# allenai/gpv-1

Measured on AMD Instinct MI355X. Metric: images/sec/node (train step, 480x640, bs32/GPU), higher is better.
Workload: dtype bf16; 1 GPU; GPV-1 (ResNet-50 + 6+6 DETR layers, 100 queries, RoI head, BERT-base, 3 co-attention, 3 text-decoder layers, V=10000) CocoCaptioning-only train step, dropout 0.1, AdamW; global_batch=32, image=480x640, parallelism=dp1

## Files before the change

gpv-1_amd/csrc/common.h:

```cpp
#pragma once
#include <hip/hip_runtime.h>
#include <stdint.h>
#include <type_traits>

typedef __bf16 bf16;
typedef bf16 __attribute__((ext_vector_type(8))) bf16x8;
typedef bf16 __attribute__((ext_vector_type(4))) bf16x4;
typedef bf16 __attribute__((ext_vector_type(2))) bf16x2;
typedef float __attribute__((ext_vector_type(4))) f32x4;

#include <stdlib.h>
#ifdef GPV_TUNING
static inline int tune_env(const char* name, int dflt) { const char* e = getenv(name); return e ? atoi(e) : dflt; }
#else
static inline int tune_env(const char*, int dflt) { return dflt; }
#endif

#define GPV_CHECK_LAUNCH() \
  do {                     \
    hipError_t e_ = hipGetLastError(); \
    if (e_ != hipSuccess) return (int)e_; \
  } while (0)

__host__ __device__ __forceinline__ bool al16(const void* p) { return (reinterpret_cast<uintptr_t>(p) & 15) == 0; }
// ... 74 lines not shown
    for (int e = 0; e < N; ++e) m |= (drop_keep(seed, base + e, thresh) ? 1u : 0u) << e;
  }
  return m;
}
namespace gpvk { extern const uint64_t* g_seed_dev; }
__device__ __forceinline__ uint64_t eff_seed(uint64_t seed, const uint64_t* epoch) {
  return epoch ? seed ^ (*epoch * 0x9E3779B97F4A7C15ull) : seed;
}
__host__ __device__ __forceinline__ uint32_t drop_thresh(float p) {
  double t = (double)p * 4294967296.0;
  if (t < 0) t = 0;
  if (t > 4294967295.0) t = 4294967295.0;
  return (uint32_t)t;
}

template <int NTHR, int U, typename SrcF, typename DstF>
__device__ __forceinline__ void stage_chunks16(int total, int tid, SrcF src, DstF dst) {
  for (int base = 0; base < total; base += NTHR * U) {
    bf16x8 tmp[U];
#pragma unroll
    for (int u = 0; u < U; ++u) {
      const int idx = base + u * NTHR + tid;
      tmp[u] = *reinterpret_cast<const bf16x8*>(src(idx < total ? idx : total - 1));
    }
#pragma unroll
    for (int u = 0; u < U; ++u) {
      const int idx = base + u * NTHR + tid;
      if (idx < total) *reinterpret_cast<bf16x8*>(dst(idx)) = tmp[u];
    }
  }
}

__device__ __forceinline__ float gelu_erf(float x) { return 0.5f * x * (1.0f + erff(x * 0.70710678118654752f)); }

template <typename T> struct Ld8;
template <> struct Ld8<bf16> {
  static __device__ __forceinline__ void ld(const bf16* p, float* o) {
    bf16x8 v = *reinterpret_cast<const bf16x8*>(p);
#pragma unroll
    for (int i = 0; i < 8; ++i) o[i] = (float)v[i];
  }
  static __device__ __forceinline__ void st(bf16* p, const float* o) {
    bf16x8 v;
#pragma unroll
    for (int i = 0; i < 8; ++i) v[i] = (bf16)o[i];
    *reinterpret_cast<bf16x8*>(p) = v;
  }
  static __device__ __forceinline__ void ld_nt(const bf16* p, float* o) {
    const bf16x8 v = __builtin_bit_cast(bf16x8, __builtin_nontemporal_load(reinterpret_cast<const u32x4*>(p)));
#pragma unroll
    for (int i = 0; i < 8; ++i) o[i] = (float)v[i];
  }
  static __device__ __forceinline__ void st_nt(bf16* p, const float* o) {
    bf16x8 v;
#pragma unroll
    for (int i = 0; i < 8; ++i) v[i] = (bf16)o[i];
    __builtin_nontemporal_store(__builtin_bit_cast(u32x4, v), reinterpret_cast<u32x4*>(p));
  }
};
template <> struct Ld8<float> {
  static __device__ __forceinline__ void ld(const float* p, float* o) {
    float4 a = *reinterpret_cast<const float4*>(p);
    float4 b = *reinterpret_cast<const float4*>(p + 4);
    o[0] = a.x; o[1] = a.y; o[2] = a.z; o[3] = a.w; o[4] = b.x; o[5] = b.y; o[6] = b.z; o[7] = b.w;
  }
  static __device__ __forceinline__ void st(float* p, const float* o) {
// ... 18 lines not shown
```

gpv-1_amd/csrc/conv1x1_stream.hip:

```cpp
#include "gemm_common.h"

namespace gpvk {
namespace {


__device__ __forceinline__ f32x4 mfma16s(bf16x8 a, bf16x8 b, f32x4 c) { return __builtin_amdgcn_mfma_f32_16x16x32_bf16(a, b, c, 0, 0, 0); }


template <int K, int NH, bool RES, bool MASK, bool NT, bool LIN = false, int NP = 1, bool BITS = false>
__global__ __launch_bounds__(512) __attribute__((amdgpu_waves_per_eu((NP == 1 && NH * K * 2 > 72 * 1024) ? 2 : 1, (NP == 1 && NH * K * 2 > 72 * 1024) ? 2 : 8)))
void c1s_kernel(GemmK p, int ncols) {
  constexpr int KC = K / 32, NTL = NH / 16, NG = NH / 32, SL = K / 8, ROWB = K * 2;
  constexpr bool BIG = NP == 1 && NH * K * 2 > 72 * 1024;
  extern __shared__ __attribute__((aligned(16))) unsigned char smem_raw[];
  bf16* Wl = reinterpret_cast<bf16*>(smem_raw);
  float* bias_l = reinterpret_cast<float*>(Wl + (size_t)ncols * K);
  const int tid = threadIdx.x, lane = tid & 63, wave = tid >> 6, g = lane >> 4, pl = lane & 15;
  const int cbase = (int)blockIdx.y * ncols;
  const bf16* A = reinterpret_cast<const bf16*>(p.A);
  const bf16* Wg = reinterpret_cast<const bf16*>(p.B) + (int64_t)cbase * p.ldb;
  bf16* C = reinterpret_cast<bf16*>(p.C) + cbase;
  const bf16* R = reinterpret_cast<const bf16*>(p.res) + cbase;
  const bf16* Mk = reinterpret_cast<const bf16*>(p.mask) + cbase;
  const float* bias_g = p.bias ? p.bias + cbase : nullptr;
// ... 130 lines not shown
          for (int i = 0; i < 4; ++i) { acc[2 * t][i] *= p.alpha; acc[2 * t + 1][i] *= p.alpha; }
        }
        float v[8] = {acc[2 * t][0] + b0.x, acc[2 * t][1] + b0.y, acc[2 * t][2] + b0.z, acc[2 * t][3] + b0.w,
                      acc[2 * t + 1][0] + b1.x, acc[2 * t + 1][1] + b1.y, acc[2 * t + 1][2] + b1.z, acc[2 * t + 1][3] + b1.w};
        bf16x8 o;
        bool masked = false;
        if constexpr (LIN) {
          if (p.dthresh) {
            masked = true;
            uint32_t dropw[4];
            if (hfast) {
#pragma unroll
              for (int q = 0; q < 4; ++q) {
                uint32_t x = hbase + (uint32_t)(h * (NH / 2) + t * 16 + q) * 0x9E3779B9u;
                x ^= x >> 16; x = __umul24(x, 0x85EBCBu);
                x ^= x >> 13; x = __umul24(x, 0xC2B2AFu);
                x ^= x >> 16;
                typedef short s16x2 __attribute__((ext_vector_type(2)));
                const s16x2 d = __builtin_elementwise_sub_sat(__builtin_bit_cast(s16x2, x ^ 0x80008000u), __builtin_bit_cast(s16x2, ts2));
                dropw[q] = __builtin_bit_cast(uint32_t, (s16x2)(d >> (s16x2){15, 15}));
              }
            } else {
              const uint32_t keep8 = drop_mask<8>(p.seed, (uint64_t)pxc * (uint64_t)nfull + (uint64_t)(cbase + c0), p.dthresh);
#pragma unroll
              for (int q = 0; q < 4; ++q)
                dropw[q] = (((keep8 >> (2 * q)) & 1u) ? 0u : 0xffffu) | (((keep8 >> (2 * q + 1)) & 1u) ? 0u : 0xffff0000u);
            }
#pragma unroll
            for (int e = 0; e < 8; ++e) {
              float x = v[e];
              if constexpr (RES) x += (float)rv[t][e];
              if (p.act == GPV_ACT_RELU) x = fmaxf(x, 0.f);
              x *= p.dscale;
              if constexpr (MASK) x = (float)mv[t][e] > 0.f ? x : 0.f;
              o[e] = (bf16)x;
            }
            u32x4 ow = __builtin_bit_cast(u32x4, o);
#pragma unroll
            for (int q = 0; q < 4; ++q) ow[q] &= ~dropw[q];
            o = __builtin_bit_cast(bf16x8, ow);
          }
        }
        if (!masked) {
#pragma unroll
          for (int e = 0; e < 8; ++e) {
            float x = v[e];
            if constexpr (RES) x += (float)rv[t][e];
            if (p.act == GPV_ACT_RELU) x = fmaxf(x, 0.f);
            if constexpr (MASK && BITS) x = ((mw[t >> 2] >> ((t & 3) * 8 + e)) & 1u) ? x : 0.f;
            else if constexpr (MASK) x = (float)mv[t][e] > 0.f ? x : 0.f;
            o[e] = (bf16)x;
          }
        }
        if constexpr (BITS && !MASK) {
          bits_acc[t >> 2] |= positive_bits8(__builtin_bit_cast(u32x4, o)) << ((t & 3) * 8);
        }
        {
          bf16* q = C + (int64_t)pxc * p.ldc + c0;
          const u32x4 ov = __builtin_bit_cast(u32x4, o);
          if constexpr (NT) asm volatile("global_store_dwordx4 %0, %1, off nt\n\ts_nop 1" :: "v"(q), "v"(ov) : "memory");
          else asm volatile("global_store_dwordx4 %0, %1, off\n\ts_nop 1" :: "v"(q), "v"(ov) : "memory");
        }
      }
      if constexpr (BITS && !MASK) {
        static_assert(NG == 8 || !(BITS && !MASK), "mask bits are written by 256-channel passes");
        unsigned char* bq = reinterpret_cast<unsigned char*>(p.out_bits) + boff;
        const uint2 bv = make_uint2(bits_acc[0], bits_acc[1]);
// ... 13 lines not shown
  const int ncols = c1s_cols(k.K, k.N), nsl = k.N / ncols;
  const size_t lds = (size_t)ncols * K * 2 + (size_t)ncols * sizeof(float);
  auto fn = c1s_kernel<K, NH, RES, MASK, NT, LIN, NP, BITS>;
  static size_t attr = 0;
  if (lds > 64 * 1024 && lds > attr) {
    hipError_t e = hipFuncSetAttribute(reinterpret_cast<const void*>(fn), hipFuncAttributeMaxDynamicSharedMemorySize, (int)lds);
    if (e != hipSuccess) { (void)hipGetLastError(); return (int)e; }
    attr = lds;
  }
  const int ntile = (k.M + 15) / 16;
  static const int bpc = tune_env("GPV_C1S_BLOCKS", 0);
  int blocks = bpc > 0 ? bpc : (lds <= 72 * 1024 ? 512 : 256);
  blocks = (blocks + nsl - 1) / nsl;
  if (blocks * 8 > ntile) blocks = (ntile + 7) / 8;
  hipLaunchKernelGGL(fn, dim3(blocks, nsl), dim3(512), lds, st, k, ncols);
  GPV_CHECK_LAUNCH();
  return 0;
}

template <int K, int NH, bool RES, bool MASK, bool NT, bool LIN = false, bool BITS = false>
int c1s_launch(const GemmK& k, hipStream_t st) {
  const int np = c1s_cols(k.K, k.N) / NH;
  if (np == 1) return c1s_launch_np<K, NH, RES, MASK, NT, LIN, 1, BITS>(k, st);
  if constexpr (K <= 128 && NH == 256 && !LIN) { if (np == 2) return c1s_launch_np<K, NH, RES, MASK, NT, LIN, 2, BITS>(k, st); }
  return -1;
}

template <int K, int NH>
int c1s_flags(const GemmK& k, hipStream_t st, bool linear) {
  const bool r = k.res != nullptr, m = k.mask != nullptr, nt = k.nt_io != 0;
  if (linear || k.alpha != 1.0f || k.dthresh) {
    if constexpr (K == 256 && NH == 256) {
      if (nt) return -1;
      if (r && m) return c1s_launch<K, NH, true, true, false, true>(k, st);
      if (r) return c1s_launch<K, NH, true, false, false, true>(k, st);
      if (m) return c1s_launch<K, NH, false, true, false, true>(k, st);
      return c1s_launch<K, NH, false, false, false, true>(k, st);
    } else {
      return -1;
    }
  }
  if (k.mask_bits || k.out_bits) {
    if (nt || !r || (k.mask_bits && k.out_bits)) return -1;
    if constexpr ((K == 128 || K == 256) && NH == 256) {
      if (k.out_bits) return (m || k.act != GPV_ACT_RELU) ? -1 : c1s_launch<K, NH, true, false, false, false, true>(k, st);
      return c1s_launch<K, NH, true, true, false, false, true>(k, st);
    } else if constexpr (K == 512 && NH == 128) {
      if (k.out_bits) return -1;
      return c1s_launch<K, NH, true, true, false, false, true>(k, st);
    } else {
      return -1;
    }
  }
  if (nt) {
    if (m) return -1;
    return r ? c1s_launch<K, NH, true, false, true>(k, st) : c1s_launch<K, NH, false, false, true>(k, st);
  }
  if (r && m) return c1s_launch<K, NH, true, true, false>(k, st);
  if (r) return c1s_launch<K, NH, true, false, false>(k, st);
  if (m) return c1s_launch<K, NH, false, true, false>(k, st);
  return c1s_launch<K, NH, false, false, false>(k, st);
}

template <int K>
int c1s_n(const GemmK& k, hipStream_t st, bool linear) {
  switch (c1s_cols(K, k.N)) {
    case 64: return c1s_flags<K, 64>(k, st, linear);
    case 128: return c1s_flags<K, 128>(k, st, linear);
    case 256: case 512: if constexpr (K <= 256) return c1s_flags<K, 256>(k, st, linear); else return -1;
  }
  return -1;
}

}

int g_c1s_mode = 1;
long g_c1s_launches = 0;

int c1s_try_launch(const GemmK& k, int dtype_in, int dtype_out, hipStream_t st, bool linear, bool dry) {
  static const int env = tune_env("GPV_C1S", -1);
  const int mode = env >= 0 ? env : g_c1s_mode;
  if (mode == 0 || dtype_in != GPV_BF16 || dtype_out != GPV_BF16) return -1;
  if (k.K != 64 && k.K != 128 && k.K != 256 && k.K != 512) return -1;
  if (k.N != 64 && k.N != 128 && k.N != 256 && k.N != 512 && k.N != 1024 && k.N != 2048 && !(linear && k.N % 256 == 0 && k.N <= 2048)) return -1;
  const int ncols = c1s_cols(k.K, k.N), nsl = k.N / ncols;
  if ((size_t)ncols * (k.K + 8) * 2 + (size_t)ncols * 4 > 150 * 1024 || nsl > 8) return -1;
  if (k.rowscale || k.accumulate || k.split_k > 1 || k.a_rowsum) return -1;
  if ((k.alpha != 1.0f || k.dthresh) && !(linear && k.K == 256 && k.N >= 256 && k.N % 256 == 0)) return -1;
  if (linear && (k.cg.SH == 2 || k.cg.cm || k.nt_io)) return -1;
  if (k.act != GPV_ACT_NONE && k.act != GPV_ACT_RELU) return -1;
  if (k.lda % 8 || k.ldb != k.K || k.ldc % 8 || (k.res && k.ldr % 8) || (k.mask && k.ldm % 8)) return -1;
  if (!al16(k.A) || !al16(k.B) || !al16(k.C) || (k.res && !al16(k.res)) || (k.mask && !al16(k.mask))) return -1;
  if (linear) {
    if (mode == 1 && (k.K != 256 || k.N < 1536 || k.M < 2048)) return -1;
  } else if (mode == 1 && ((int64_t)k.M * nsl < 65536 || k.M < 32768)) return -1;
  if (k.mask_bits || k.out_bits) {
    const int nh = ncols >= 256 ? 256 : ncols;
    const bool inst = ((k.K == 128 || k.K == 256) && nh == 256) || (k.K == 512 && nh == 128 && !k.out_bits);
    if (linear || !inst || !k.res || k.nt_io || (k.mask_bits && k.out_bits) || k.N % 256 != 0 || (k.out_bits && (k.mask && !k.mask_bits))) return -1;
    if (k.out_bits && k.act != GPV_ACT_RELU) return -1;
    if (k.K <= 128 && ncols / nh > 2) return -1;
    if (k.K > 128 && ncols / nh != 1) return -1;
  }
  if (dry) return 0;
  int e = -1;
  switch (k.K) {
    case 64: e = c1s_n<64>(k, st, linear); break;
    case 128: e = c1s_n<128>(k, st, linear); break;
    case 256: e = c1s_n<256>(k, st, linear); break;
    case 512: e = c1s_n<512>(k, st, linear); break;
  }
  if (e == 0) ++g_c1s_launches;
  return e;
}

}
```

gpv-1_amd/csrc/gemm.hip:

```cpp
#include "gemm_common.h"
#include <cstdlib>

using namespace gpvk;

#ifndef GPV_PF
#define GPV_PF 2
#endif

namespace {

constexpr int BK = 32;
constexpr int LDK = 40;

template <typename T> struct Raw8;
__device__ __forceinline__ uint32_t bf_bits(float x) { return (uint32_t)__builtin_bit_cast(unsigned short, (bf16)x); }
template <> struct Raw8<bf16> {
  uint32_t w[4];
  __device__ __forceinline__ void zero() { w[0] = w[1] = w[2] = w[3] = 0u; }
  __device__ __forceinline__ void load(const bf16* p) {
    uint4 t = *reinterpret_cast<const uint4*>(p);
    w[0] = t.x; w[1] = t.y; w[2] = t.z; w[3] = t.w;
  }
  __device__ __forceinline__ void load_n(const bf16* p, int n) {
    const unsigned short* q = reinterpret_cast<const unsigned short*>(p);
// ... 259 lines not shown
      }
      raw[it].write(hi + kr * PITCH + ch * 8, lo + kr * PITCH + ch * 8);
    }
  }
  __device__ __forceinline__ void flush_sums(float* out) {
    if constexpr (SUM) {
#pragma unroll
      for (int it = 0; it < NIT; ++it) {
        const int ch = (threadIdx.x + it * 256) % CHK;
#pragma unroll
        for (int e = 0; e < 8; ++e) {
          float v = csum[it][e];
#pragma unroll
          for (int s = CHK; s < 64; s <<= 1) v += __shfl_xor(v, s);
          const int col = col0 + ch * 8 + e;
          if ((threadIdx.x & 63) < CHK && col < ncols) atomicAdd(out + col, v);
        }
      }
    }
  }
  static __device__ __forceinline__ bf16x8 frag(const bf16* tile, int cbase, int lane) {
    typedef short __attribute__((ext_vector_type(4))) s16x4;
    typedef __attribute__((address_space(3))) s16x4 lds_s16x4;
    const int g = lane >> 4, i = lane & 15;
    const bf16* p0 = tile + (8 * g + (i >> 2)) * PITCH + cbase + (i & 3) * 4;
    s16x4 a = __builtin_amdgcn_ds_read_tr16_b64_v4i16((lds_s16x4*)(p0));
    s16x4 b = __builtin_amdgcn_ds_read_tr16_b64_v4i16((lds_s16x4*)(p0 + 4 * PITCH));
    typedef short __attribute__((ext_vector_type(8))) s16x8;
    s16x8 r = {a[0], a[1], a[2], a[3], b[0], b[1], b[2], b[3]};
    return __builtin_bit_cast(bf16x8, r);
  }
};

template <typename TIn, typename TOut, int AMODE, int BMODE, int BM, int BN, bool VEC, bool NTIO = false>
__device__ __forceinline__ void gemm_body(const GemmK& p) {
  constexpr bool PRECISE = sizeof(TIn) == 4;
  constexpr int FM = BM / 32, FN = BN / 32;
  constexpr int A_ELEMS = BM * LDK, B_ELEMS = BN * LDK;
  constexpr int STAGE_ELEMS = (A_ELEMS + B_ELEMS) * (PRECISE ? 2 : 1);
  extern __shared__ __attribute__((aligned(16))) unsigned char smem_raw[];
  bf16* smem = reinterpret_cast<bf16*>(smem_raw);

  const int tid = threadIdx.x, lane = tid & 63, wave = tid >> 6;
  const int wm = wave >> 1, wn = wave & 1;
  int tile, ksplit;
  {
    const bool plane = gridDim.z == 1;
    const int gx = gridDim.x;
    const int nwg = plane ? gx * (int)gridDim.y : gx, bid = plane ? (int)blockIdx.x + gx * (int)blockIdx.y : (int)blockIdx.x;
    const int v = xcd_contiguous(bid, nwg);
    ksplit = plane ? v / gx : (int)blockIdx.y;
    tile = plane ? v - ksplit * gx : v;
  }
  int tm = tile / p.tilesN;
  const int tn = tile - tm * p.tilesN;
  if constexpr (AMODE == OP_CONV) {
    if (p.cg.cm && p.cg.cls_rows % BM == 0 && p.M == 4 * p.cg.cls_rows) {
      const int tpc = p.cg.cls_rows / BM;
      tm = (tm & 3) * tpc + (tm >> 2);
    }
  }
  const int row0 = tm * BM, col0 = tn * BN;
  const int batch = blockIdx.z;

  int kt_total = (p.K + BK - 1) / BK;
  int cm_r0 = 0, cm_s0 = 0, cm_nS = 1, cm_cpt = 1;
  bool cm_on = false, cm_empty = false;
// ... 141 lines not shown
  const TOut* Mp = reinterpret_cast<const TOut*>(p.mask);

  if constexpr (ASUM) {
    if (as.do_sum) as.flush_sums(p.a_rowsum);
  }
  if (p.accumulate) {
    if constexpr (sizeof(TOut) == 4) {
#pragma unroll
      for (int i = 0; i < FM; ++i) {
        const int m = row0 + wm * (BM / 2) + i * 16 + (lane & 15);
        if (m >= p.M) continue;
        const float rs = p.rowscale ? p.rowscale[m] * p.alpha : p.alpha;
#pragma unroll
        for (int j = 0; j < FN; ++j) {
          const int n = col0 + wn * (BN / 2) + j * 16 + (lane >> 4) * 4;
          float* dst = reinterpret_cast<float*>(Cp) + (int64_t)m * ldc + n;
#pragma unroll
          for (int r = 0; r < 4; ++r)
            if (n + r < p.N) atomicAdd(dst + r, acc[i][j][r] * rs);
        }
      }
    }
    return;
  }

  float* ep = reinterpret_cast<float*>(smem_raw);
  constexpr int EPITCH = BN + 4;
  constexpr int HR = BM / 2;
  constexpr int CH = BN / 8;
  constexpr int NCH = (HR * CH) / 256;
  const bool v_st = (ldc % 8 == 0) && ((reinterpret_cast<uintptr_t>(Cp) & 15) == 0);
  const bool v_res = Rp && (p.ldr % 8 == 0) && ((reinterpret_cast<uintptr_t>(Rp) & 15) == 0);
  const bool v_msk = Mp && (p.ldm % 8 == 0) && ((reinterpret_cast<uintptr_t>(Mp) & 15) == 0);
  float bv[8];
  {
    const int nb = col0 + (tid % CH) * 8;
    const bool vb = p.bias && nb + 8 <= p.N && ((reinterpret_cast<uintptr_t>(p.bias) & 15) == 0);
    if (vb) {
      const float4 b0 = *reinterpret_cast<const float4*>(p.bias + nb);
      const float4 b1 = *reinterpret_cast<const float4*>(p.bias + nb + 4);
      bv[0] = b0.x; bv[1] = b0.y; bv[2] = b0.z; bv[3] = b0.w; bv[4] = b1.x; bv[5] = b1.y; bv[6] = b1.z; bv[7] = b1.w;
    } else {
#pragma unroll
      for (int e = 0; e < 8; ++e) bv[e] = (p.bias && nb + e < p.N) ? p.bias[nb + e] : 0.f;
    }
  }
#pragma unroll
  for (int half = 0; half < 2; ++half) {
    if (half == 1) __syncthreads();
    if (wm == half) {
#pragma unroll
      for (int i = 0; i < FM; ++i) {
        const int ml = i * 16 + (lane & 15);
#pragma unroll
        for (int j = 0; j < FN; ++j) {
          const int nl = wn * (BN / 2) + j * 16 + (lane >> 4) * 4;
          *reinterpret_cast<float4*>(ep + ml * EPITCH + nl) = make_float4(acc[i][j][0], acc[i][j][1], acc[i][j][2], acc[i][j][3]);
        }
      }
    }
    __syncthreads();
    constexpr int EPG = NCH >= 2 ? 2 : 1;
#pragma unroll
    for (int c0 = 0; c0 < NCH; c0 += EPG) {
      float rv[EPG][8], mv[EPG][8];
#pragma unroll
// ... 6 lines not shown
        const bool full = n + 8 <= p.N;
        const int64_t mp = (AMODE == OP_CONV && p.cg.cm && inb) ? s_rowpix[m - row0] : m;
        if (Rp) {
          if (inb && v_res && full) { if constexpr (NTIO) Ld8<TOut>::ld_nt(Rp + mp * p.ldr + n, rv[g]); else Ld8<TOut>::ld(Rp + mp * p.ldr + n, rv[g]); }
          else {
#pragma unroll
            for (int e = 0; e < 8; ++e) rv[g][e] = (inb && n + e < p.N) ? (float)Rp[mp * p.ldr + n + e] : 0.f;
          }
        }
        if (Mp) {
          if (inb && v_msk && full) Ld8<TOut>::ld(Mp + mp * p.ldm + n, mv[g]);
          else {
#pragma unroll
            for (int e = 0; e < 8; ++e) mv[g][e] = (inb && n + e < p.N) ? (float)Mp[mp * p.ldm + n + e] : 0.f;
          }
        }
      }
#pragma unroll
      for (int g = 0; g < EPG; ++g) {
        const int idx = tid + (c0 + g) * 256;
        const int r = idx / CH, c8 = idx - r * CH;
        const int m = row0 + half * HR + r;
        const int n = col0 + c8 * 8;
        if (m >= p.M || n >= p.N) continue;
        float v[8];
        {
          const float4 a = *reinterpret_cast<const float4*>(ep + r * EPITCH + c8 * 8);
          const float4 b = *reinterpret_cast<const float4*>(ep + r * EPITCH + c8 * 8 + 4);
          v[0] = a.x; v[1] = a.y; v[2] = a.z; v[3] = a.w; v[4] = b.x; v[5] = b.y; v[6] = b.z; v[7] = b.w;
        }
        const float rs = p.rowscale ? p.rowscale[m] * p.alpha : p.alpha;
        const bool full = n + 8 <= p.N;
        const uint32_t keep8 = p.dthresh ? drop_mask<8>(p.seed, ((uint64_t)batch * p.M + m) * (uint64_t)p.N + n, p.dthresh) : 0xffu;
#pragma unroll
        for (int e = 0; e < 8; ++e) {
          float x = v[e] * rs;
          x += bv[e];
          if (Rp) x += rv[g][e];
          if (p.act == GPV_ACT_RELU) x = fmaxf(x, 0.f);
          else if (p.act == GPV_ACT_GELU) x = gelu_erf(x);
          if (p.dthresh) x = ((keep8 >> e) & 1u) ? x * p.dscale : 0.f;
          if (Mp) x = mv[g][e] > 0.f ? x : 0.f;
          v[e] = x;
        }
        const int64_t mp = (AMODE == OP_CONV && p.cg.cm && m < p.M) ? s_rowpix[m - row0] : m;
        TOut* dst = Cp + mp * ldc + n;
        if (v_st && full) { if constexpr (NTIO) Ld8<TOut>::st_nt(dst, v); else Ld8<TOut>::st(dst, v); }
        else {
#pragma unroll
          for (int e = 0; e < 8; ++e)
            if (n + e < p.N) dst[e] = (TOut)v[e];
        }
      }
    }
  }
}

template <typename TIn, typename TOut, int AMODE, int BMODE, int BM, int BN, bool VEC>
__global__ __launch_bounds__(256) void gemm_kernel(GemmK p) {
  if (p.dthresh) p.seed = eff_seed(p.seed, p.seed_dev);
  gemm_body<TIn, TOut, AMODE, BMODE, BM, BN, VEC>(p);
}
template <typename TIn, typename TOut, int BM, int BN, bool VEC>
__global__ __launch_bounds__(256) void conv1x1_kernel(GemmK p) {
  if (p.dthresh) p.seed = eff_seed(p.seed, p.seed_dev);
  gemm_body<TIn, TOut, OP_PLAIN, OP_PLAIN, BM, BN, VEC>(p);
}
template <int BM, int BN>
__global__ __launch_bounds__(256) void conv1x1_nt_kernel(GemmK p) {
  gemm_body<bf16, bf16, OP_PLAIN, OP_PLAIN, BM, BN, true, true>(p);
}

template <int G>
__global__ __launch_bounds__(256) void splitk_reduce_kernel(const float* __restrict__ ws, int nsplit, int M, int N, float* __restrict__ C,
                                                            int64_t ldc) {
  constexpr int QB = 256 / G;
  __shared__ float4 part[G > 1 ? 256 : 1];
  const int64_t slab = (int64_t)M * N;
  const int nq = N >> 2;
  const int64_t total = (int64_t)M * nq;
  const int ql = threadIdx.x % QB, g = threadIdx.x / QB;
  const int64_t i = (int64_t)blockIdx.x * QB + ql;
  float4 a = make_float4(0.f, 0.f, 0.f, 0.f);
  int m = 0, n = 0;
  if (i < total) {
    m = (int)(i / nq); n = (int)(i - (int64_t)m * nq) * 4;
    const float* src = ws + (int64_t)m * N + n;
    for (int s = g; s < nsplit; s += G) {
      const float4 v = *reinterpret_cast<const float4*>(src + s * slab);
      a.x += v.x; a.y += v.y; a.z += v.z; a.w += v.w;
    }
  }
  if constexpr (G > 1) {
    part[threadIdx.x] = a;
// ... 25 lines not shown
    hipLaunchKernelGGL(splitk_reduce_kernel<4>, dim3((unsigned)((quads + 63) / 64)), dim3(256), 0, st, ws, split, M, N, C, ldc);
  } else {
    hipLaunchKernelGGL(splitk_reduce_kernel<1>, dim3((unsigned)((quads + 255) / 256)), dim3(256), 0, st, ws, split, M, N, C, ldc);
  }
  GPV_CHECK_LAUNCH();
  return 0;
}
}

namespace {

template <typename TIn, typename TOut, int AMODE, int BMODE, int BM, int BN, bool VEC>
int launch_cfg_v(const GemmK& k, int batch, hipStream_t st) {
  constexpr bool PRECISE = sizeof(TIn) == 4;
  constexpr size_t lds = (size_t)2 * (BM + BN) * LDK * 2 * (PRECISE ? 2 : 1);
  GemmK p = k;
  const int tilesM = (p.M + BM - 1) / BM;
  p.tilesN = (p.N + BN - 1) / BN;
  const int kt_total = (p.K + BK - 1) / BK;
  int split = p.split_k < 1 ? 1 : p.split_k;
  if (split > kt_total) split = kt_total;
  p.kt_per_split = (kt_total + split - 1) / split;
  split = (kt_total + p.kt_per_split - 1) / p.kt_per_split;
  p.ws = nullptr;
  bool two_pass = false;
  if (p.accumulate && split > 1 && batch == 1 && k.ws_base != nullptr && sizeof(TOut) == 4 &&
      (int64_t)split * p.M * p.N * 4 <= k.ws_bytes && p.N % 4 == 0 && p.ldc % 4 == 0 &&
      (reinterpret_cast<uintptr_t>(p.C) & 15) == 0) {
    two_pass = true;
    p.ws = reinterpret_cast<float*>(k.ws_base);
    p.accumulate = 0; p.res = nullptr; p.mask = nullptr; p.bias = nullptr; p.act = 0; p.dthresh = 0;
  }
  auto fn = gemm_kernel<TIn, TOut, AMODE, BMODE, BM, BN, VEC>;
  if constexpr (AMODE == OP_PLAIN && BMODE == OP_PLAIN) {
    if (k.conv1x1) fn = conv1x1_kernel<TIn, TOut, BM, BN, VEC>;
    if constexpr (std::is_same<TIn, bf16>::value && std::is_same<TOut, bf16>::value && VEC) {
      if (k.conv1x1 && k.nt_io && !p.dthresh && !two_pass) fn = conv1x1_nt_kernel<BM, BN>;
    }
  }
  static bool attr_done[2] = {false, false};
  if (lds > 64 * 1024 && !attr_done[k.conv1x1 ? 1 : 0]) {
    hipError_t e = hipFuncSetAttribute(reinterpret_cast<const void*>(fn), hipFuncAttributeMaxDynamicSharedMemorySize, (int)lds);
    if (e != hipSuccess) { (void)hipGetLastError(); return (int)e; }
    attr_done[k.conv1x1 ? 1 : 0] = true;
  }
  dim3 grid(tilesM * p.tilesN, split, batch);
  hipLaunchKernelGGL(fn, grid, dim3(256), lds, st, p);
  GPV_CHECK_LAUNCH();
  if (two_pass) {
    const int e = launch_splitk_reduce(p.ws, split, p.M, p.N, reinterpret_cast<float*>(p.C), p.ldc, st);
    if (e) return e;
  }
  return 0;
}

template <typename TIn, typename TOut, int AMODE, int BMODE, int BM, int BN>
int launch_cfg(const GemmK& k, int batch, hipStream_t st) {
  if (k.vecA && k.vecB) return launch_cfg_v<TIn, TOut, AMODE, BMODE, BM, BN, true>(k, batch, st);
  return launch_cfg_v<TIn, TOut, AMODE, BMODE, BM, BN, false>(k, batch, st);
}

__global__ __launch_bounds__(256) void conv_split_epilogue_kernel(const float* __restrict__ ws, int nsplit, int M, int N, const float* __restrict__ bias,
                                                                  const bf16* __restrict__ res, int act, bf16* __restrict__ y) {
  const int nq = N >> 2;
  const int64_t i = (int64_t)blockIdx.x * 256 + threadIdx.x;
  if (i >= (int64_t)M * nq) return;
// ... 85 lines not shown
  const int64_t px = i / C8;
  const int ow = (int)(px % OW), oh = (int)((px / OW) % OH);
  if (((oh | ow) & 1) == 0) return;
  bf16x8 o = bf16x8{0, 0, 0, 0, 0, 0, 0, 0};
  if (res) {
    o = *reinterpret_cast<const bf16x8*>(res + i * 8);
    if (mask) {
      const bf16x8 m = *reinterpret_cast<const bf16x8*>(mask + i * 8);
#pragma unroll
      for (int e = 0; e < 8; ++e) o[e] = (float)m[e] > 0.f ? o[e] : (bf16)0.f;
    }
  }
  *reinterpret_cast<bf16x8*>(dx + i * 8) = o;
}

}

extern "C" int gpv_abi_version(void) { return 1; }

extern "C" int gpv_gemm(const gpv_gemm_args* a, void* stream) {
  if (!a || !a->A || !a->B || !a->C || a->M <= 0 || a->N <= 0 || a->K <= 0 || a->batch <= 0) return (int)hipErrorInvalidValue;
  if ((a->split_k > 1 || a->accumulate) && a->dtype_out != GPV_F32) return (int)hipErrorInvalidValue;
  if (a->split_k > 1 && (!a->accumulate || a->bias || a->res || a->act || a->relu_mask || a->drop_p > 0.f)) return (int)hipErrorInvalidValue;
  GemmK k{};
  k.A = a->A; k.B = a->B; k.C = a->C; k.M = a->M; k.N = a->N; k.K = a->K;
  k.lda = a->lda; k.ldb = a->ldb; k.ldc = a->ldc; k.sA = a->sA; k.sB = a->sB; k.sC = a->sC;
  k.alpha = a->alpha; k.rowscale = a->rowscale; k.bias = a->bias;
  k.res = a->res; k.ldr = a->ldr; k.sR = a->sR; k.mask = a->relu_mask; k.ldm = a->ldm;
  k.act = a->act; k.seed = a->seed; k.seed_dev = gpvk::g_seed_dev;
  k.dthresh = a->drop_p > 0.f ? drop_thresh(a->drop_p) : 0u;
  k.dscale = a->drop_p > 0.f ? 1.0f / (1.0f - a->drop_p) : 1.0f;
  k.accumulate = a->accumulate; k.split_k = a->split_k;
  k.a_rowsum = a->a_rowsum;
  k.no_small = (a->flags & GPV_GEMM_NO_PIPE_SMALL) ? 1 : 0;
  k.ws_base = a->workspace; k.ws_bytes = a->workspace ? a->workspace_bytes : 0;
  if (k.a_rowsum && !(a->layoutA == GPV_TRANS && a->layoutB == GPV_TRANS && a->batch == 1)) return (int)hipErrorInvalidValue;
  if (a->accumulate && a->split_k <= 1 && !a->res) {
    k.accumulate = 0; k.res = a->C; k.ldr = a->ldc; k.sR = a->sC;
  }
  const int esz = a->dtype_in == GPV_F32 ? 4 : 2;
  const int64_t vecel = 16 / esz;
  auto vec_ok = [&](const void* ptr, int64_t ld, int64_t bs, int layout, int extent_contig) {
    bool ok = al16(ptr) && (ld % vecel == 0) && (a->batch == 1 || bs % vecel == 0);
    if (layout == GPV_KMAJOR) ok = ok && (a->K % 8 == 0 || ((a->flags & GPV_GEMM_KPAD_FINITE) && ld >= ((int64_t)a->K + 7) / 8 * 8));
    else ok = ok && (extent_contig % 8 == 0 || ld >= ((int64_t)extent_contig + 7) / 8 * 8);
    return ok ? 1 : 0;
  };
  k.vecA = vec_ok(a->A, a->lda, a->sA, a->layoutA, a->M);
  k.vecB = vec_ok(a->B, a->ldb, a->sB, a->layoutB, a->N);
  {
    const int64_t lim = 0x7ffffff0ll / esz;
    if ((int64_t)(a->layoutA == GPV_KMAJOR ? a->M : a->K) * a->lda >= lim) k.vecA = 0;
    if ((int64_t)(a->layoutB == GPV_KMAJOR ? a->N : a->K) * a->ldb >= lim) k.vecB = 0;
  }
  hipStream_t st = reinterpret_cast<hipStream_t>(stream);
  const int la = a->layoutA, lb = a->layoutB;
  if (la == GPV_KMAJOR && lb == GPV_KMAJOR) {
    const int gv = gemv_try_launch(k, a->dtype_in, a->dtype_out, a->batch, st);
    if (gv >= 0) return gv;
    static const bool c1s_linear = tune_env("GPV_C1S_LINEAR", 1) != 0;
    if (a->batch == 1 && !g_kernel_forced && c1s_linear) {
      const int cs = c1s_try_launch(k, a->dtype_in, a->dtype_out, st, true);
      if (cs >= 0) return cs;
    }
    const int pp = pipe_try_launch(k, OP_PLAIN, a->dtype_in, a->dtype_out, a->batch, st);
    if (pp >= 0) return pp;
    const int sk = skinny_try_launch(k, 0, a->dtype_in, a->dtype_out, a->batch, st);
    if (sk >= 0) return sk;
    const int g = glds_try_launch(k, OP_PLAIN, a->dtype_in, a->dtype_out, a->batch, st);
    if (g >= 0) return g;
    return launch_dtype<OP_PLAIN, OP_PLAIN>(k, a->batch, a->dtype_in, a->dtype_out, st);
  }
  if (la == GPV_KMAJOR && lb == GPV_TRANS) {
    const int sk = skinny_try_launch(k, 1, a->dtype_in, a->dtype_out, a->batch, st);
    if (sk >= 0) return sk;
    return launch_dtype<OP_PLAIN, OP_TRANS>(k, a->batch, a->dtype_in, a->dtype_out, st);
  }
  if (la == GPV_TRANS && lb == GPV_TRANS) {
    if (a->accumulate) {
      GemmK kk = k;
      kk.accumulate = 1; kk.res = nullptr; kk.ldr = 0; kk.sR = 0;
      const int gt = glds_tt_try_launch(kk, a->dtype_in, a->dtype_out, a->batch, st);
      if (gt >= 0) return gt;
      const int sk = skinny_tt_try_launch(kk, a->dtype_in, a->dtype_out, a->batch, st);
      if (sk >= 0) return sk;
    }
    return launch_dtype<OP_TRANS, OP_TRANS>(k, a->batch, a->dtype_in, a->dtype_out, st);
  }
  return (int)hipErrorInvalidValue;
}

static int conv2d_impl(const gpv_conv_args* a, hipStream_t st, bool dry) {
  if (!a || !a->x || !a->w || !a->y) return (int)hipErrorInvalidValue;
  if (a->Cin % 32 != 0) return (int)hipErrorInvalidValue;
  if ((a->SH != 1 && a->SH != 2) || (a->SW != 1 && a->SW != 2)) return (int)hipErrorInvalidValue;
  const bool want_bits = a->y_mask_bits != nullptr || a->relu_mask_bits != nullptr;
  if (want_bits) {
    const bool pw1 = a->KH == 1 && a->KW == 1 && a->SH == 1 && a->SW == 1 && a->PH == 0 && a->PW == 0 && a->IH == a->OH && a->IW == a->OW;
    const bool d3s2 = a->mode == 1 && a->KH == 3 && a->KW == 3 && a->SH == 2 && a->SW == 2 && a->PH == 1 && a->PW == 1 && a->Cout == 128 && !a->y_mask_bits;
    if (!pw1 && !d3s2) return (int)hipErrorInvalidValue;
    if ((pw1 && a->Cout % 256 != 0) || (a->y_mask_bits && (a->mode != 0 || a->act != GPV_ACT_RELU || a->relu_mask)) || (a->relu_mask_bits && a->mode != 1)) return (int)hipErrorInvalidValue;
    if ((reinterpret_cast<uintptr_t>(a->y_mask_bits) | reinterpret_cast<uintptr_t>(a->relu_mask_bits)) & 15) return (int)hipErrorInvalidValue;
  } else if (dry) {
    return (int)hipErrorInvalidValue;
  }
  GemmK k{};
  k.alpha = 1.0f; k.rowscale = a->rowscale; k.bias = a->bias; k.act = a->act;
  k.cg = ConvGeom{a->IH, a->IW, a->Cs, a->Cin, a->OH, a->OW, a->KH, a->KW, a->SH, a->SW, a->PH, a->PW, a->mode == 1, 0, 0};
  if (a->mode == 1 && a->SH == 2 && a->SW == 2 && a->OH % 2 == 0 && a->OW % 2 == 0) {
    k.cg.cm = 1;
    k.cg.cls_rows = a->B * (a->OH / 2) * (a->OW / 2);
  }
  const int T = a->KH * a->KW;
  const int esz = a->dtype_in == GPV_F32 ? 4 : 2;
// ... 143 lines not shown
```

gpv-1_amd/csrc/gemm_common.h:

```cpp
#pragma once
#include "common.h"
#include "../../include/gpv_hip.h"

namespace gpvk {

enum { OP_PLAIN = 0, OP_TRANS = 1, OP_CONV = 2 };

struct ConvGeom {
  int IH, IW, Cs, Cin, OH, OW, KH, KW, SH, SW, PH, PW, dgrad;
  int cm;
  int cls_rows;
};

struct GemmK {
  const void* A; const void* B; void* C;
  int M, N, K;
  int64_t lda, ldb, ldc, sA, sB, sC;
  float alpha;
  const float* rowscale; const float* bias;
  const void* res; int64_t ldr, sR;
  const void* mask; int64_t ldm;
  int act; uint32_t dthresh; float dscale; uint64_t seed; const uint64_t* seed_dev;
  int accumulate, split_k, kt_per_split, tilesN;
  int vecA, vecB;
  int conv1x1;
  int depi;
  int no_small;
  int nt_io;
  void* ws_base; int64_t ws_bytes;
  float* ws;
  const uint32_t* mask_bits;
  uint32_t* out_bits;
  float* a_rowsum;
  ConvGeom cg;
};

__device__ __forceinline__ int conv_row_to_pixel(int m, const ConvGeom& g) {
  if (!g.cm) return m;
  const int cls = m / g.cls_rows, rem = m - cls * g.cls_rows;
  const int hw2 = (g.OH >> 1) * (g.OW >> 1), w2 = g.OW >> 1;
  const int b = rem / hw2, r2 = rem - b * hw2;
  const int y2 = r2 / w2, x2 = r2 - y2 * w2;
  return (b * g.OH + 2 * y2 + (cls >> 1)) * g.OW + 2 * x2 + (cls & 1);
}


__device__ __forceinline__ int depi_col_perm(int r) { return (r & ~31) + ((r & 15) >> 2) * 8 + ((r >> 4) & 1) * 4 + (r & 3); }

int glds_try_launch(const GemmK& k, int amode, int dtype_in, int dtype_out, int batch, hipStream_t st);

int pipe_try_launch(const GemmK& k, int amode, int dtype_in, int dtype_out, int batch, hipStream_t st);
int pipe_set_mode(int v);
int pipe_set_small(int v);
long pipe_launches(long set);

int c1s_try_launch(const GemmK& k, int dtype_in, int dtype_out, hipStream_t st, bool linear = false, bool dry = false);
extern int g_c1s_mode;
extern long g_c1s_launches;

int c3s_try_launch(const GemmK& k, int dtype_in, int dtype_out, hipStream_t st, bool dry = false);
extern int g_c3s_mode;
extern long g_c3s_launches;

extern int g_two_per_cu;
extern int g_kernel_forced;
extern int g_bm96_fill;
inline int two_per_cu_bm(const GemmK& k, int batch) {
  if (k.N % 128 != 0 || batch != 1) return 0;
  if (g_bm96_fill && k.M <= 1024) {
    const int64_t t128 = (int64_t)((k.M + 127) / 128) * (k.N / 128), t96 = (int64_t)((k.M + 95) / 96) * (k.N / 128);
    if (t96 <= 256 && t96 * 10 >= t128 * 12) return 96;
  }
  int best = 0;
  double best_u = 0.0;
  for (int bm : {160, 96}) {
    const int64_t t = (int64_t)((k.M + bm - 1) / bm) * (k.N / 128);
    if (t <= 384) continue;
    const double u = (double)t / (512.0 * ((t + 511) / 512));
    if ((t <= 512 || u >= 0.9) && u > best_u) { best = bm; best_u = u; }
  }
  return best;
}
inline bool glds_two_per_cu(const GemmK& k, int batch) {
  return g_two_per_cu && k.K >= 512 && (!k.cg.cm || k.cg.KH == 1) && two_per_cu_bm(k, batch) != 0;
}

int skinny_try_launch(const GemmK& k, int b_trans, int dtype_in, int dtype_out, int batch, hipStream_t st);
extern int g_skinny_mode;

int gemv_try_launch(const GemmK& k, int dtype_in, int dtype_out, int batch, hipStream_t st);
extern int g_gemv_mode;
extern long g_gemv_launches;

int launch_splitk_reduce(const float* ws, int split, int M, int N, float* C, int64_t ldc, hipStream_t st);
int skinny_tt_try_launch(const GemmK& k, int dtype_in, int dtype_out, int batch, hipStream_t st);

int glds_wgrad_try_launch(const GemmK& k, int dtype_in, int dtype_out, hipStream_t st);
int glds_tt_try_launch(const GemmK& k, int dtype_in, int dtype_out, int batch, hipStream_t st);
extern int g_wgrad_mode;
extern int g_wg8_mode;
extern long g_wg8_launches;
extern int g_w8l_mode;
extern int g_wg8h_mode;

}
```

gpv-1_amd/csrc/gemm_glds.hip:

```cpp
#include "gemm_common.h"
#include <cstdlib>
#include <type_traits>

namespace gpvk {
namespace {

constexpr int GBK = 64;
constexpr int ROWB = 128;
constexpr int GBM = 256;
long g_glds_launches = 0;

typedef __attribute__((address_space(3))) void lds_void_t;
typedef const __attribute__((address_space(1))) void glb_void_t;

template <int AMODE, int BM, int BN, typename TOut>
__device__ __forceinline__ void glds_body(const GemmK& p) {
  constexpr int NT = BM == 256 ? 512 : 256, NW = NT / 64;
  constexpr int WN = BN / 64, WM = NW / WN;
  constexpr int WTM = BM / WM;
  constexpr int FM = WTM / 16, FN = 4;
  constexpr int A_BYTES = BM * ROWB, B_BYTES = BN * ROWB, STAGE = A_BYTES + B_BYTES;
  constexpr int AI = BM / (8 * NW), BI = BN / (8 * NW);
  extern __shared__ __attribute__((aligned(128))) unsigned char smem[];
  __shared__ int s_rowpix[AMODE == OP_CONV ? BM : 1];

  const int tid = threadIdx.x, lane = tid & 63;
  const int wave = __builtin_amdgcn_readfirstlane(tid >> 6);
  const int wm = wave / WN, wn = wave - wm * WN;
  int tile = xcd_contiguous(blockIdx.x, gridDim.x);
  if constexpr (AMODE == OP_CONV) {
    if (p.cg.cm && p.cg.cls_rows % BM == 0 && p.M == 4 * p.cg.cls_rows) {
      const int nwg = gridDim.x, bid = blockIdx.x;
      const int xcd = bid & 7, loc = bid >> 3;
      const int s0 = xcd_contiguous(xcd, nwg), cnt = (nwg >> 3) + (xcd < (nwg & 7) ? 1 : 0);
      const int tN = p.tilesN, G = 4 * tN;
      auto below = [&](int x, int c) { const int m = x / G, u = x - m * G - c * tN; return m * tN + (u < 0 ? 0 : (u > tN ? tN : u)); };
      int left = loc, pick = 0, before = 0;
#pragma unroll
      for (int k = 0; k < 4; ++k) {
        const int c = k == 0 ? 3 : k == 1 ? 1 : k == 2 ? 2 : 0;
        const int b = below(s0, c), n = below(s0 + cnt, c) - b;
        if (k == 3 || left < n) { pick = c; before = b; break; }
        left -= n;
      }
      const int ord = before + left;
      tile = (ord / tN) * G + pick * tN + (ord - (ord / tN) * tN);
    }
  }
// ... 29 lines not shown
    }
  }
  constexpr int OOB = 0x7ffffff0;
  const int lrow = lane >> 3;
  const int lchunk = (lane & 7) ^ lrow;
  int a_vo[AI];
  int a_oh[AI], a_ow[AI];
  int b_vo[BI];
  const bf16* Ab = reinterpret_cast<const bf16*>(p.A) + (int64_t)batch * p.sA;
  const bf16* Bb = reinterpret_cast<const bf16*>(p.B) + (int64_t)batch * p.sB;
  const auto rsA = __builtin_amdgcn_make_buffer_rsrc(const_cast<bf16*>(Ab), (short)0, OOB, 0x00020000);
  const auto rsB = __builtin_amdgcn_make_buffer_rsrc(const_cast<bf16*>(Bb), (short)0, OOB, 0x00020000);
#pragma unroll
  for (int j = 0; j < AI; ++j) {
    const int r = wave * (AI * 8) + j * 8 + lrow;
    const int m = min(row0 + r, p.M - 1);
    if constexpr (AMODE == OP_CONV) {
      const int pix = conv_row_to_pixel(m, p.cg);
      const int b = pix / (p.cg.OH * p.cg.OW);
      const int rem = pix - b * (p.cg.OH * p.cg.OW);
      a_oh[j] = rem / p.cg.OW;
      a_ow[j] = rem - a_oh[j] * p.cg.OW;
      a_vo[j] = (b * p.cg.IH * p.cg.IW * p.cg.Cs + lchunk * 8) * 2;
    } else {
      a_oh[j] = a_ow[j] = 0;
      a_vo[j] = (m * (int)p.lda + lchunk * 8) * 2;
    }
  }
  const bool bz = (AMODE == OP_CONV) && cm_empty;
  const bool depi = p.depi && std::is_same<TOut, bf16>::value && p.N % BN == 0 && p.ldc % 8 == 0 &&
                    ((reinterpret_cast<uintptr_t>(p.C) | (uintptr_t)(p.sC * 2)) & 15) == 0 &&
                    (!p.res || (p.ldr % 8 == 0 && ((reinterpret_cast<uintptr_t>(p.res) | (uintptr_t)(p.sR * 2)) & 15) == 0)) &&
                    (!p.mask || (p.ldm % 8 == 0 && (reinterpret_cast<uintptr_t>(p.mask) & 15) == 0)) &&
                    (!p.bias || (reinterpret_cast<uintptr_t>(p.bias) & 15) == 0);
#pragma unroll
  for (int j = 0; j < BI; ++j) {
    const int r = wave * (BI * 8) + j * 8 + lrow;
    const int rp = depi ? (r & ~31) + ((r & 15) >> 2) * 8 + ((r >> 4) & 1) * 4 + (r & 3) : r;
    const int n = min(col0 + rp, p.N - 1);
    b_vo[j] = bz ? OOB : (n * (int)p.ldb + lchunk * 8) * 2;
  }
  auto bload = [&](const decltype(rsA)& rs, int voff, int soff, unsigned char* l) {
    __builtin_amdgcn_raw_ptr_buffer_load_lds(rs, (lds_void_t*)l, 16, voff, soff, 0, 0);
  };

  int it_c0 = 0, it_tr = cm_on ? cm_r0 : 0, it_ts = cm_on ? cm_s0 : 0;
  int tap_off[AI];
#pragma unroll
  for (int j = 0; j < AI; ++j) tap_off[j] = OOB;

  auto issue = [&](int kt, int stage) {
    unsigned char* sa = smem + stage * STAGE + wave * (AI * 1024);
    unsigned char* sb = smem + stage * STAGE + A_BYTES + wave * (BI * 1024);
    int k0;
    if constexpr (AMODE == OP_CONV) {
      const ConvGeom& g = p.cg;
      if (it_c0 == 0) {
#pragma unroll
        for (int j = 0; j < AI; ++j) {
          int ih, iw;
          bool ok = !cm_empty;
          if (g.dgrad) {
            const int th = a_oh[j] + g.PH - it_tr, tw = a_ow[j] + g.PW - it_ts;
            const int sh = g.SH - 1, sw = g.SW - 1;
            ih = th >> sh; iw = tw >> sw;
            ok = ok && th >= 0 && tw >= 0 && ((th & sh) == 0) && ((tw & sw) == 0) && ih < g.IH && iw < g.IW;
          } else {
// ... 33 lines not shown

  issue(0, 0);
  for (int t = 0; t < nk; ++t) {
    asm volatile("s_waitcnt vmcnt(0)" ::: "memory");
    __syncthreads();
    if (t + 1 < nk) issue(t + 1, (t + 1) & 1);
    const unsigned char* st = smem + (t & 1) * STAGE;
#pragma unroll
    for (int kk = 0; kk < 2; ++kk) {
      const int slot = ((kk * 4 + fkg) ^ fsw) << 4;
      bf16x8 af[FM], bfr[FN];
#pragma unroll
      for (int j = 0; j < FN; ++j) bfr[j] = *reinterpret_cast<const bf16x8*>(st + b_off + j * 16 * ROWB + slot);
#pragma unroll
      for (int i = 0; i < FM; ++i) af[i] = *reinterpret_cast<const bf16x8*>(st + a_off + i * 16 * ROWB + slot);
#pragma unroll
      for (int i = 0; i < FM; ++i)
#pragma unroll
        for (int j = 0; j < FN; ++j) acc[i][j] = mfma16(bfr[j], af[i], acc[i][j]);
    }
  }

  TOut* Cp = reinterpret_cast<TOut*>(p.C) + (int64_t)batch * p.sC;
  const TOut* Rp = p.res ? reinterpret_cast<const TOut*>(p.res) + (int64_t)batch * p.sR : nullptr;
  const TOut* Mp = reinterpret_cast<const TOut*>(p.mask);
  float* ep = reinterpret_cast<float*>(smem);
  constexpr int EPITCH = BN + 4;
  constexpr int HR = BM / 2;
  constexpr int CH = BN / 8;
  constexpr int NCH = (HR * CH) / NT;
  const bool v_st = (p.ldc % 8 == 0) && ((reinterpret_cast<uintptr_t>(Cp) & 15) == 0);
  const bool v_res = Rp && (p.ldr % 8 == 0) && ((reinterpret_cast<uintptr_t>(Rp) & 15) == 0);
  const bool v_msk = Mp && (p.ldm % 8 == 0) && ((reinterpret_cast<uintptr_t>(Mp) & 15) == 0);
  if (depi) {
    const int mrow = wm * WTM + frow;
    float bq[2][8];
#pragma unroll
    for (int t = 0; t < 2; ++t) {
      const int n = col0 + wn * 64 + t * 32 + fkg * 8;
      if (p.bias) {
        const float4 b0 = *reinterpret_cast<const float4*>(p.bias + n), b1 = *reinterpret_cast<const float4*>(p.bias + n + 4);
        bq[t][0] = b0.x; bq[t][1] = b0.y; bq[t][2] = b0.z; bq[t][3] = b0.w; bq[t][4] = b1.x; bq[t][5] = b1.y; bq[t][6] = b1.z; bq[t][7] = b1.w;
      } else {
#pragma unroll
        for (int e = 0; e < 8; ++e) bq[t][e] = 0.f;
      }
    }
    if constexpr (std::is_same<TOut, bf16>::value) {
      constexpr int CHK = 2;
#pragma unroll
      for (int i0 = 0; i0 < FM; i0 += CHK) {
        bf16x8 rraw[CHK][2], mraw[CHK][2];
        int64_t mpv[CHK];
        float rsv[CHK];
#pragma unroll
        for (int ii = 0; ii < CHK; ++ii) {
          const int i = i0 + ii;
          if (i < FM) {
            const int ml = mrow + i * 16, m = min(row0 + ml, p.M - 1);
            rsv[ii] = p.rowscale ? p.rowscale[m] : 1.0f;
            int64_t mp = m;
            if constexpr (AMODE == OP_CONV) { if (p.cg.cm) mp = s_rowpix[ml]; }
            mpv[ii] = mp;
#pragma unroll
            for (int t = 0; t < 2; ++t) {
              const int n = col0 + wn * 64 + t * 32 + fkg * 8;
              if (Rp) rraw[ii][t] = *reinterpret_cast<const bf16x8*>(Rp + mp * p.ldr + n);
              if (Mp) mraw[ii][t] = *reinterpret_cast<const bf16x8*>(Mp + mp * p.ldm + n);
            }
          }
        }
#pragma unroll
        for (int ii = 0; ii < CHK; ++ii) {
          const int i = i0 + ii;
          if (i < FM) {
            const int ml = mrow + i * 16, m = row0 + ml;
            const int mc = min(m, p.M - 1);
            const float rs = rsv[ii] * p.alpha;
#pragma unroll
            for (int t = 0; t < 2; ++t) {
              const int n = col0 + wn * 64 + t * 32 + fkg * 8;
              const uint32_t keep8 = p.dthresh ? drop_mask<8>(p.seed, ((uint64_t)batch * p.M + mc) * (uint64_t)p.N + n, p.dthresh) : 0xffu;
              float v[8] = {acc[i][2 * t][0], acc[i][2 * t][1], acc[i][2 * t][2], acc[i][2 * t][3],
                            acc[i][2 * t + 1][0], acc[i][2 * t + 1][1], acc[i][2 * t + 1][2], acc[i][2 * t + 1][3]};
#pragma unroll
              for (int e = 0; e < 8; ++e) {
                float x = v[e] * rs;
                x += bq[t][e];
                if (Rp) x += (float)rraw[ii][t][e];
                if (p.act == GPV_ACT_RELU) x = fmaxf(x, 0.f);
                else if (p.act == GPV_ACT_GELU) x = gelu_erf(x);
                if (p.dthresh) x = ((keep8 >> e) & 1u) ? x * p.dscale : 0.f;
                if (Mp) x = (float)mraw[ii][t][e] > 0.f ? x : 0.f;
                v[e] = x;
              }
              if (m < p.M) Ld8<TOut>::st(Cp + mpv[ii] * p.ldc + n, v);
            }
          }
        }
      }
    }
    return;
  }
  float bv[8];
  {
    const int nb = col0 + (tid % CH) * 8;
    const bool vb = p.bias && nb + 8 <= p.N && ((reinterpret_cast<uintptr_t>(p.bias) & 15) == 0);
    if (vb) {
      const float4 b0 = *reinterpret_cast<const float4*>(p.bias + nb);
      const float4 b1 = *reinterpret_cast<const float4*>(p.bias + nb + 4);
      bv[0] = b0.x; bv[1] = b0.y; bv[2] = b0.z; bv[3] = b0.w; bv[4] = b1.x; bv[5] = b1.y; bv[6] = b1.z; bv[7] = b1.w;
    } else {
#pragma unroll
      for (int e = 0; e < 8; ++e) bv[e] = (p.bias && nb + e < p.N) ? p.bias[nb + e] : 0.f;
    }
  }
#pragma unroll
  for (int half = 0; half < 2; ++half) {
    __syncthreads();
    if ((wm * WTM) / HR == half) {
#pragma unroll
      for (int i = 0; i < FM; ++i) {
        const int r = wm * WTM + i * 16 + frow - half * HR;
#pragma unroll
        for (int j = 0; j < FN; ++j)
          *reinterpret_cast<f32x4*>(ep + r * EPITCH + wn * 64 + j * 16 + fkg * 4) = acc[i][j];
      }
// ... 1 lines not shown
    __syncthreads();
#pragma unroll
    for (int g = 0; g < NCH; ++g) {
      const int idx = tid + g * NT;
      const int r = idx / CH, c8 = idx - r * CH;
      const int m = row0 + half * HR + r;
      const int n = col0 + c8 * 8;
      if (m >= p.M || n >= p.N) continue;
      const bool full = n + 8 <= p.N;
      int64_t mp = m;
      if constexpr (AMODE == OP_CONV) { if (p.cg.cm) mp = s_rowpix[half * HR + r]; }
      float v[8], rv[8], mv[8];
      {
        const float4 a = *reinterpret_cast<const float4*>(ep + r * EPITCH + c8 * 8);
        const float4 b = *reinterpret_cast<const float4*>(ep + r * EPITCH + c8 * 8 + 4);
        v[0] = a.x; v[1] = a.y; v[2] = a.z; v[3] = a.w; v[4] = b.x; v[5] = b.y; v[6] = b.z; v[7] = b.w;
      }
      if (Rp) {
        if (v_res && full) Ld8<TOut>::ld(Rp + mp * p.ldr + n, rv);
        else {
#pragma unroll
          for (int e = 0; e < 8; ++e) rv[e] = (n + e < p.N) ? (float)Rp[mp * p.ldr + n + e] : 0.f;
        }
      }
      if (Mp) {
        if (v_msk && full) Ld8<TOut>::ld(Mp + mp * p.ldm + n, mv);
        else {
#pragma unroll
          for (int e = 0; e < 8; ++e) mv[e] = (n + e < p.N) ? (float)Mp[mp * p.ldm + n + e] : 0.f;
        }
      }
      const float rs = p.rowscale ? p.rowscale[m] * p.alpha : p.alpha;
      const uint32_t keep8 = p.dthresh ? drop_mask<8>(p.seed, ((uint64_t)batch * p.M + m) * (uint64_t)p.N + n, p.dthresh) : 0xffu;
#pragma unroll
      for (int e = 0; e < 8; ++e) {
        float x = v[e] * rs;
        x += bv[e];
        if (Rp) x += rv[e];
        if (p.act == GPV_ACT_RELU) x = fmaxf(x, 0.f);
        else if (p.act == GPV_ACT_GELU) x = gelu_erf(x);
        if (p.dthresh) x = ((keep8 >> e) & 1u) ? x * p.dscale : 0.f;
        if (Mp) x = mv[e] > 0.f ? x : 0.f;
        v[e] = x;
      }
      TOut* dst = Cp + mp * p.ldc + n;
      if (v_st && full) Ld8<TOut>::st(dst, v);
      else {
#pragma unroll
        for (int e = 0; e < 8; ++e)
          if (n + e < p.N) dst[e] = (TOut)v[e];
      }
    }
  }
}

template <int AMODE, int BM, int BN, typename TOut>
__global__ __launch_bounds__(BM == 256 ? 512 : 256) void glds_kernel(GemmK p) {
  if (p.dthresh) p.seed = eff_seed(p.seed, p.seed_dev);
  glds_body<AMODE, BM, BN, TOut>(p);
}

int g_halo_mode = tune_env("GPV_C3_HALO", 1);
long g_halo_launches = 0;

template <int BM>
__global__ __launch_bounds__(256) void glds_halo_kernel(GemmK p) {
  constexpr int BN = 128, NW = 4, WN = 2, WTM = BM / 2, FM = WTM / 16, FN = 4;
  constexpr int HROWS = BM + 96;
  constexpr int A_BYTES = HROWS * ROWB, B_BYTES = BN * ROWB;
  constexpr int AIH = HROWS / (8 * NW), BI = BN / (8 * NW);
  static_assert(HROWS % (8 * NW) == 0 && WTM % 16 == 0, "tile shape");
  extern __shared__ __attribute__((aligned(128))) unsigned char smem[];
  const int tid = threadIdx.x, lane = tid & 63;
  const int wave = __builtin_amdgcn_readfirstlane(tid >> 6);
  const int wm = wave / WN, wn = wave - wm * WN;
  int tile = xcd_contiguous(blockIdx.x, gridDim.x);
// ... 159 lines not shown
int launch_halo(const GemmK& k, hipStream_t st) {
  constexpr size_t lds = (size_t)(BM + 96) * ROWB + (size_t)2 * 128 * ROWB;
  GemmK p = k;
  const int tilesM = (p.M + BM - 1) / BM;
  p.tilesN = p.N / 128;
  auto fn = glds_halo_kernel<BM>;
  static bool attr_done = false;
  if (!attr_done) {
    hipError_t e = hipFuncSetAttribute(reinterpret_cast<const void*>(fn), hipFuncAttributeMaxDynamicSharedMemorySize, (int)lds);
    if (e != hipSuccess) { (void)hipGetLastError(); return (int)e; }
    attr_done = true;
  }
  ++g_halo_launches;
  ++g_glds_launches;
  hipLaunchKernelGGL(fn, dim3(tilesM * p.tilesN), dim3(256), lds, st, p);
  GPV_CHECK_LAUNCH();
  return 0;
}

inline bool halo_ok(const GemmK& k, int dtype_out, int batch) {
  const ConvGeom& g = k.cg;
  return g_halo_mode != 0 && dtype_out == GPV_BF16 && batch == 1 && g.KH == 3 && g.KW == 3 && g.SH == 1 && g.SW == 1 && g.PH == 1 && g.PW == 1 &&
         !g.cm && g.OH == g.IH && g.OW == g.IW && g.IW <= 47 && g.Cin % GBK == 0 && k.N % 128 == 0 && k.K == 9 * g.Cin &&
         k.M % (g.IH * g.IW) == 0 && k.ldc % 8 == 0 && al16(k.C) && (!k.res || (k.ldr % 8 == 0 && al16(k.res))) &&
         (!k.mask || (k.ldm % 8 == 0 && al16(k.mask))) && (!k.bias || al16(k.bias)) && !k.dthresh && k.act != GPV_ACT_GELU;
}

template <int BM, int BN, typename TOut>
__global__ __launch_bounds__(BM == 256 ? 512 : 256) void glds_conv1x1_kernel(GemmK p) {
  if (p.dthresh) p.seed = eff_seed(p.seed, p.seed_dev);
  glds_body<OP_PLAIN, BM, BN, TOut>(p);
}

template <int AMODE, int BM, int BN, typename TOut>
int launch_glds(const GemmK& k, int batch, hipStream_t st) {
  constexpr size_t stage = (size_t)2 * (BM + BN) * ROWB;
  constexpr size_t epi = (size_t)(BM / 2) * (BN + 4) * 4;
  constexpr size_t lds = stage > epi ? stage : epi;
  GemmK p = k;
  const int tilesM = (p.M + BM - 1) / BM;
  p.tilesN = (p.N + BN - 1) / BN;
  const bool c11 = AMODE == OP_PLAIN && p.conv1x1;
  auto fn = c11 ? glds_conv1x1_kernel<BM, BN, TOut> : glds_kernel<AMODE, BM, BN, TOut>;
  static bool attr_done[2] = {false, false};
  if (!attr_done[c11]) {
    hipError_t e = hipFuncSetAttribute(reinterpret_cast<const void*>(fn), hipFuncAttributeMaxDynamicSharedMemorySize, (int)lds);
    if (e != hipSuccess) { (void)hipGetLastError(); return (int)e; }
    attr_done[c11] = true;
  }
  static const int depi = tune_env("GPV_GLDS_DEPI", 1);
  p.depi = depi;
  dim3 grid(tilesM * p.tilesN, 1, batch);
  ++g_glds_launches;
  hipLaunchKernelGGL(fn, grid, dim3(BM == 256 ? 512 : 256), lds, st, p);
  GPV_CHECK_LAUNCH();
  return 0;
}

template <int AMODE, int BM, int BN>
int launch_glds_out(const GemmK& k, int dtype_out, int batch, hipStream_t st) {
  if (dtype_out == GPV_BF16) return launch_glds<AMODE, BM, BN, bf16>(k, batch, st);
  return launch_glds<AMODE, BM, BN, float>(k, batch, st);
}

}
int g_kernel_forced = 0;
int g_two_per_cu = tune_env("GPV_TWO_PER_CU", 1);
int g_bm96_fill = tune_env("GPV_BM96", 1);
namespace {
int g_glds_mode = tune_env("GPV_GLDS", 1);

}

int glds_try_launch(const GemmK& k, int amode, int dtype_in, int dtype_out, int batch, hipStream_t st) {
  const int mode = g_glds_mode;
  if (mode == 0 || dtype_in != GPV_BF16) return -1;
  if (k.accumulate || k.split_k > 1) return -1;
  if (k.K % GBK != 0 || k.K < GBK || k.N <= 64) return -1;
  if (!al16(k.A) || !al16(k.B) || k.ldb % 8 != 0 || (batch > 1 && (k.sA % 8 != 0 || k.sB % 8 != 0))) return -1;
  const int64_t lim = 0x7ffffff0ll / 2;
  if ((int64_t)k.N * k.ldb >= lim) return -1;
  if (amode == OP_CONV) {
    if ((int64_t)k.cg.IH * k.cg.IW * k.cg.Cs * ((int64_t)k.M / ((int64_t)k.cg.OH * k.cg.OW) + 1) >= lim) return -1;
    if (k.cg.Cin % GBK != 0 || k.cg.Cs % 8 != 0) return -1;
  } else if (amode == OP_PLAIN) {
    if (k.lda % 8 != 0 || (int64_t)k.M * k.lda >= lim) return -1;
  } else {
    return -1;
  }
  if (glds_two_per_cu(k, batch) && mode != 2 && mode != 3) {
    const int bm2 = two_per_cu_bm(k, batch);
    if (amode == OP_CONV && halo_ok(k, dtype_out, batch)) {
      if (bm2 == 160) return launch_halo<160>(k, st);
      if (bm2 == 96 && g_halo_mode >= 2) return launch_halo<96>(k, st);
    }
    if (bm2 == 160) return amode == OP_CONV ? launch_glds_out<OP_CONV, 160, 128>(k, dtype_out, batch, st) : launch_glds_out<OP_PLAIN, 160, 128>(k, dtype_out, batch, st);
    if (bm2 == 96) return amode == OP_CONV ? launch_glds_out<OP_CONV, 96, 128>(k, dtype_out, batch, st) : launch_glds_out<OP_PLAIN, 96, 128>(k, dtype_out, batch, st);
  }
  const int bn = k.N > 128 ? 256 : 128;
  bool small_tiles = mode == 3;
  if (mode == 1) {
    const int64_t tiles = (int64_t)((k.M + GBM - 1) / GBM) * ((k.N + bn - 1) / bn) * batch;
    const bool huge = tiles >= 1024 && k.K >= 512 && !(amode == OP_CONV && k.cg.cm);
    small_tiles = !huge && (k.K >= 1024 || (k.K >= 512 && !k.mask));
    if (!huge && !small_tiles) return -1;
  }
  if (small_tiles)
    return amode == OP_CONV ? launch_glds_out<OP_CONV, 128, 128>(k, dtype_out, batch, st) : launch_glds_out<OP_PLAIN, 128, 128>(k, dtype_out, batch, st);
  if (amode == OP_CONV) return bn == 256 ? launch_glds_out<OP_CONV, 256, 256>(k, dtype_out, batch, st) : launch_glds_out<OP_CONV, 256, 128>(k, dtype_out, batch, st);
  return bn == 256 ? launch_glds_out<OP_PLAIN, 256, 256>(k, dtype_out, batch, st) : launch_glds_out<OP_PLAIN, 256, 128>(k, dtype_out, batch, st);
}

}

namespace gpvk { int attn_bwd1_mode(int set); long attn_bwd1_launches(long set); }

extern "C" int gpv_set_option(int option, int value) {
  if (option == GPV_OPT_C1S_LAUNCHES) {
    const long prev = gpvk::g_c1s_launches;
    gpvk::g_c1s_launches = value;
    return (int)prev;
  }
// ... 46 lines not shown
    gpvk::g_wgrad_mode = value;
    return prev;
  }
  if (option == GPV_OPT_C1S) {
    const int prev = gpvk::g_c1s_mode;
    gpvk::g_c1s_mode = value;
    return prev;
  }
  if (option == GPV_OPT_C3S) {
    const int prev = gpvk::g_c3s_mode;
    gpvk::g_c3s_mode = value;
    return prev;
  }
  if (option == GPV_OPT_C3S_LAUNCHES) {
    const long prev = gpvk::g_c3s_launches;
    gpvk::g_c3s_launches = value;
    return (int)prev;
  }
  if (option == GPV_OPT_PIPE) {
    gpvk::g_kernel_forced = (gpvk::g_kernel_forced & ~2) | (value >= 100 ? 2 : 0);
    return gpvk::pipe_set_mode(value);
  }
  if (option == GPV_OPT_PIPE_LAUNCHES) return (int)gpvk::pipe_launches(value);
  if (option == GPV_OPT_C3_HALO) {
    const int prev = gpvk::g_halo_mode;
    gpvk::g_halo_mode = value;
    return prev;
  }
  if (option == GPV_OPT_C3_HALO_LAUNCHES) {
    const long prev = gpvk::g_halo_launches;
    gpvk::g_halo_launches = value;
    return (int)prev;
  }
  if (option == GPV_OPT_GLDS_LAUNCHES) {
    const long prev = gpvk::g_glds_launches;
    gpvk::g_glds_launches = value;
    return (int)prev;
  }
  return -1;
}
```

gpv-1_amd/csrc/gemm_pipe.hip:

```cpp
#include "gemm_common.h"
#include <type_traits>
#include <cstdlib>
#ifndef GPV_PIPE_SWP
#define GPV_PIPE_SWP 1
#endif

namespace gpvk {
namespace {

constexpr int GBK = 64;
constexpr int ROWB = 128;
constexpr int NW = 8, NT = 512;
long g_pipe_launches = 0;

typedef __attribute__((address_space(3))) void lds_void_t;

template <int N> __device__ __forceinline__ void wait_vm_c() { asm volatile("s_waitcnt vmcnt(%0)" ::"n"(N) : "memory"); }
__device__ __forceinline__ void wait_vm(int n) {
  switch (n) {
    case 0: wait_vm_c<0>(); break;
    case 1: wait_vm_c<1>(); break;
    case 2: wait_vm_c<2>(); break;
    case 3: wait_vm_c<3>(); break;
    case 4: wait_vm_c<4>(); break;
    case 5: wait_vm_c<5>(); break;
    case 6: wait_vm_c<6>(); break;
    case 7: wait_vm_c<7>(); break;
    case 8: wait_vm_c<8>(); break;
    case 9: wait_vm_c<9>(); break;
    case 10: wait_vm_c<10>(); break;
    case 11: wait_vm_c<11>(); break;
    case 12: wait_vm_c<12>(); break;
    case 13: wait_vm_c<13>(); break;
    case 14: wait_vm_c<14>(); break;
    case 15: wait_vm_c<15>(); break;
    case 16: wait_vm_c<16>(); break;
    case 17: wait_vm_c<17>(); break;
    case 18: wait_vm_c<18>(); break;
    default: wait_vm_c<0>(); break;
  }
}

template <int AMODE, int BM, int BN, int WM, int NS, typename TOut>
__device__ __forceinline__ void pipe_body(const GemmK& p) {
  constexpr int WN = NW / WM;
  constexpr bool SWP = GPV_PIPE_SWP != 0 && (BM / WM / 16 + BN / (NW / WM) / 16) * 8 + (BM / WM / 16) * (BN / (NW / WM) / 16) * 4 <= 200;
  constexpr int WTM = BM / WM, WTN = BN / WN;
  constexpr int FM = WTM / 16, FN = WTN / 16;
  static_assert(WTM % 16 == 0 && WTN % 16 == 0 && BM % 16 == 0 && BN % 64 == 0, "tile shape");
  constexpr int A_BYTES = BM * ROWB, B_BYTES = BN * ROWB, STAGE = A_BYTES + B_BYTES;
  constexpr int PA = BM / 8, PB = BN / 8;
  constexpr int AI = (PA + NW - 1) / NW, BI = (PB + NW - 1) / NW;
  constexpr bool A_EVEN = PA % NW == 0, B_EVEN = PB % NW == 0;
  extern __shared__ __attribute__((aligned(128))) unsigned char smem[];
  int* s_rowpix = reinterpret_cast<int*>(smem + NS * STAGE);

  const int tid = threadIdx.x, lane = tid & 63;
  const int wave = __builtin_amdgcn_readfirstlane(tid >> 6);
  const int wm = wave / WN, wn = wave - wm * WN;
  int tile = xcd_contiguous(blockIdx.x, gridDim.x);
  int tm = __builtin_amdgcn_readfirstlane(tile / p.tilesN);
  const int tn = tile - tm * p.tilesN;
  if constexpr (AMODE == OP_CONV) {
    if (p.cg.cm && p.cg.cls_rows % BM == 0 && p.M == 4 * p.cg.cls_rows) {
      const int tpc = p.cg.cls_rows / BM;
      tm = (tm & 3) * tpc + (tm >> 2);
    }
  }
  const int row0 = tm * BM, col0 = tn * BN;
  const int batch = blockIdx.z;

  int nk = p.K / GBK;
  int cm_r0 = 0, cm_s0 = 0, cm_nS = 1, cm_cpt = 1;
  bool cm_on = false, cm_empty = false;
  if constexpr (AMODE == OP_CONV) {
    if (p.cg.cm) {
// ... 11 lines not shown
        if (nk == 0) { cm_empty = true; nk = 1; }
      }
    }
  }
  constexpr int OOB = 0x7ffffff0;
  const int lrow = lane >> 3;
  const int lchunk = (lane & 7) ^ lrow;
  int a_vo[AI], a_oh[AI], a_ow[AI], b_vo[BI];
  const bf16* Ab = reinterpret_cast<const bf16*>(p.A) + (int64_t)batch * p.sA;
  const bf16* Bb = reinterpret_cast<const bf16*>(p.B) + (int64_t)batch * p.sB;
  const auto rsA = __builtin_amdgcn_make_buffer_rsrc(const_cast<bf16*>(Ab), (short)0, OOB, 0x00020000);
  const auto rsB = __builtin_amdgcn_make_buffer_rsrc(const_cast<bf16*>(Bb), (short)0, OOB, 0x00020000);
#pragma unroll
  for (int j = 0; j < AI; ++j) {
    const int r = (j * NW + wave) * 8 + lrow;
    const int m = min(row0 + r, p.M - 1);
    if constexpr (AMODE == OP_CONV) {
      const int pix = conv_row_to_pixel(m, p.cg);
      const int b = pix / (p.cg.OH * p.cg.OW);
      const int rem = pix - b * (p.cg.OH * p.cg.OW);
      a_oh[j] = rem / p.cg.OW;
      a_ow[j] = rem - a_oh[j] * p.cg.OW;
      a_vo[j] = (b * p.cg.IH * p.cg.IW * p.cg.Cs + lchunk * 8) * 2;
    } else {
      a_oh[j] = a_ow[j] = 0;
      a_vo[j] = (m * (int)p.lda + lchunk * 8) * 2;
    }
  }
  const bool bz = (AMODE == OP_CONV) && cm_empty;
  const bool depi = (FN % 2 == 0) && p.depi && std::is_same<TOut, bf16>::value && p.N % BN == 0 && p.ldc % 8 == 0 &&
                    ((reinterpret_cast<uintptr_t>(p.C) | (uintptr_t)(p.sC * 2)) & 15) == 0 &&
                    (!p.res || (p.ldr % 8 == 0 && ((reinterpret_cast<uintptr_t>(p.res) | (uintptr_t)(p.sR * 2)) & 15) == 0)) &&
                    (!p.mask || (p.ldm % 8 == 0 && (reinterpret_cast<uintptr_t>(p.mask) & 15) == 0)) &&
                    (!p.bias || (reinterpret_cast<uintptr_t>(p.bias) & 15) == 0);
#pragma unroll
  for (int j = 0; j < BI; ++j) {
    const int r = (j * NW + wave) * 8 + lrow;
    const int rp = depi ? (r & ~31) + ((r & 15) >> 2) * 8 + ((r >> 4) & 1) * 4 + (r & 3) : r;
    const int n = min(col0 + rp, p.N - 1);
    b_vo[j] = bz ? OOB : (n * (int)p.ldb + lchunk * 8) * 2;
  }
  int nl = 0;
#pragma unroll
  for (int j = 0; j < AI; ++j) nl += (A_EVEN || j * NW + wave < PA) ? 1 : 0;
#pragma unroll
  for (int j = 0; j < BI; ++j) nl += (B_EVEN || j * NW + wave < PB) ? 1 : 0;
  nl = __builtin_amdgcn_readfirstlane(nl);

  auto bload = [&](const decltype(rsA)& rs, int voff, int soff, unsigned char* l) {
    __builtin_amdgcn_raw_ptr_buffer_load_lds(rs, (lds_void_t*)l, 16, voff, soff, 0, 0);
  };
  int it_c0 = 0, it_tr = cm_on ? cm_r0 : 0, it_ts = cm_on ? cm_s0 : 0, it_kt = 0;
  int tap_off[AI];
#pragma unroll
  for (int j = 0; j < AI; ++j) tap_off[j] = OOB;

  auto issue = [&](int stage) {
    unsigned char* sa = smem + stage * STAGE + wave * 1024;
    unsigned char* sb = sa + A_BYTES;
    int k0;
    if constexpr (AMODE == OP_CONV) {
      const ConvGeom& g = p.cg;
      if (it_c0 == 0) {
#pragma unroll
        for (int j = 0; j < AI; ++j) {
          int ih, iw;
          bool ok = !cm_empty;
// ... 77 lines not shown
    } else {
#pragma unroll
    for (int kk = 0; kk < 2; ++kk) {
      const int slot = ((kk * 4 + fkg) ^ fsw) << 4;
      bf16x8 af[FM], bfr[FN];
#pragma unroll
      for (int j = 0; j < FN; ++j) bfr[j] = *reinterpret_cast<const bf16x8*>(st + b_off + j * 16 * ROWB + slot);
#pragma unroll
      for (int i = 0; i < FM; ++i) af[i] = *reinterpret_cast<const bf16x8*>(st + a_off + i * 16 * ROWB + slot);
#pragma unroll
      for (int i = 0; i < FM; ++i)
#pragma unroll
        for (int j = 0; j < FN; ++j) acc[i][j] = mfma16(bfr[j], af[i], acc[i][j]);
    }
    }
    sc = sc == NS - 1 ? 0 : sc + 1;
    si = si == NS - 1 ? 0 : si + 1;
  }

  TOut* Cp = reinterpret_cast<TOut*>(p.C) + (int64_t)batch * p.sC;
  const TOut* Rp = p.res ? reinterpret_cast<const TOut*>(p.res) + (int64_t)batch * p.sR : nullptr;
  const TOut* Mp = reinterpret_cast<const TOut*>(p.mask);
  float* ep = reinterpret_cast<float*>(smem);
  constexpr int EPITCH = BN + 4;
  constexpr int NHALF = (BM * BN >= 2 * NT * 8) ? 2 : 1;
  constexpr int HR = BM / NHALF;
  constexpr int CH = BN / 8;
  static_assert(HR % WTM == 0 || WTM % HR == 0, "a wave's rows lie in one half");
  static_assert((size_t)HR * EPITCH * 4 <= (size_t)NS * STAGE, "epilogue image fits the stages");
  constexpr int NCH = (HR * CH + NT - 1) / NT;
  const bool v_st = (p.ldc % 8 == 0) && ((reinterpret_cast<uintptr_t>(Cp) & 15) == 0);
  const bool v_res = Rp && (p.ldr % 8 == 0) && ((reinterpret_cast<uintptr_t>(Rp) & 15) == 0);
  const bool v_msk = Mp && (p.ldm % 8 == 0) && ((reinterpret_cast<uintptr_t>(Mp) & 15) == 0);
  if constexpr (FN % 2 == 0) {
    if (depi) {
      const int mrow = wm * WTM + frow;
#pragma unroll
      for (int i = 0; i < FM; ++i) {
        const int ml = mrow + i * 16, m = row0 + ml;
        if (m >= p.M) continue;
        int64_t mp = m;
        if constexpr (AMODE == OP_CONV) { if (p.cg.cm) mp = s_rowpix[ml]; }
        const float rs = p.rowscale ? p.rowscale[m] * p.alpha : p.alpha;
#pragma unroll
        for (int t = 0; t < FN / 2; ++t) {
          const int n = col0 + wn * WTN + t * 32 + fkg * 8;
          float bq[8] = {0.f, 0.f, 0.f, 0.f, 0.f, 0.f, 0.f, 0.f}, rv[8], mv[8];
          if (p.bias) Ld8<float>::ld(p.bias + n, bq);
          if (Rp) Ld8<TOut>::ld(Rp + mp * p.ldr + n, rv);
          if (Mp) Ld8<TOut>::ld(Mp + mp * p.ldm + n, mv);
          const uint32_t keep8 = p.dthresh ? drop_mask<8>(p.seed, ((uint64_t)batch * p.M + m) * (uint64_t)p.N + n, p.dthresh) : 0xffu;
          float v[8] = {acc[i][2 * t][0], acc[i][2 * t][1], acc[i][2 * t][2], acc[i][2 * t][3],
                        acc[i][2 * t + 1][0], acc[i][2 * t + 1][1], acc[i][2 * t + 1][2], acc[i][2 * t + 1][3]};
#pragma unroll
          for (int e = 0; e < 8; ++e) {
            float x = v[e] * rs;
            x += bq[e];
            if (Rp) x += rv[e];
            if (p.act == GPV_ACT_RELU) x = fmaxf(x, 0.f);
            else if (p.act == GPV_ACT_GELU) x = gelu_erf(x);
            if (p.dthresh) x = ((keep8 >> e) & 1u) ? x * p.dscale : 0.f;
            if (Mp) x = mv[e] > 0.f ? x : 0.f;
            v[e] = x;
          }
          Ld8<TOut>::st(Cp + mp * p.ldc + n, v);
        }
      }
      return;
    }
  }
  float bv[8];
  {
    const int nb = col0 + (tid % CH) * 8;
    const bool vb = p.bias && nb + 8 <= p.N && ((reinterpret_cast<uintptr_t>(p.bias) & 15) == 0);
    if (vb) {
      const float4 b0 = *reinterpret_cast<const float4*>(p.bias + nb);
      const float4 b1 = *reinterpret_cast<const float4*>(p.bias + nb + 4);
      bv[0] = b0.x; bv[1] = b0.y; bv[2] = b0.z; bv[3] = b0.w; bv[4] = b1.x; bv[5] = b1.y; bv[6] = b1.z; bv[7] = b1.w;
    } else {
#pragma unroll
      for (int e = 0; e < 8; ++e) bv[e] = (p.bias && nb + e < p.N) ? p.bias[nb + e] : 0.f;
    }
  }
#pragma unroll
  for (int half = 0; half < NHALF; ++half) {
    __syncthreads();
    if ((wm * WTM) / HR == half) {
#pragma unroll
      for (int i = 0; i < FM; ++i) {
        const int r = wm * WTM + i * 16 + frow - half * HR;
#pragma unroll
        for (int j = 0; j < FN; ++j)
          *reinterpret_cast<f32x4*>(ep + r * EPITCH + wn * WTN + j * 16 + fkg * 4) = acc[i][j];
      }
    }
    __syncthreads();
#pragma unroll
    for (int g = 0; g < NCH; ++g) {
      const int idx = tid + g * NT;
      if ((HR * CH) % NT != 0 && idx >= HR * CH) continue;
      const int r = idx / CH, c8 = idx - r * CH;
      const int m = row0 + half * HR + r;
      const int n = col0 + c8 * 8;
      if (m >= p.M || n >= p.N) continue;
      const bool full = n + 8 <= p.N;
      int64_t mp = m;
      if constexpr (AMODE == OP_CONV) { if (p.cg.cm) mp = s_rowpix[half * HR + r]; }
      float v[8], rv[8], mv[8];
      {
        const float4 a = *reinterpret_cast<const float4*>(ep + r * EPITCH + c8 * 8);
        const float4 b = *reinterpret_cast<const float4*>(ep + r * EPITCH + c8 * 8 + 4);
        v[0] = a.x; v[1] = a.y; v[2] = a.z; v[3] = a.w; v[4] = b.x; v[5] = b.y; v[6] = b.z; v[7] = b.w;
      }
      if (Rp) {
        if (v_res && full) Ld8<TOut>::ld(Rp + mp * p.ldr + n, rv);
        else {
#pragma unroll
          for (int e = 0; e < 8; ++e) rv[e] = (n + e < p.N) ? (float)Rp[mp * p.ldr + n + e] : 0.f;
        }
      }
      if (Mp) {
        if (v_msk && full) Ld8<TOut>::ld(Mp + mp * p.ldm + n, mv);
        else {
#pragma unroll
          for (int e = 0; e < 8; ++e) mv[e] = (n + e < p.N) ? (float)Mp[mp * p.ldm + n + e] : 0.f;
        }
      }
      const float rs = p.rowscale ? p.rowscale[m] * p.alpha : p.alpha;
      const uint32_t keep8 = p.dthresh ? drop_mask<8>(p.seed, ((uint64_t)batch * p.M + m) * (uint64_t)p.N + n, p.dthresh) : 0xffu;
#pragma unroll
      for (int e = 0; e < 8; ++e) {
        float x = v[e] * rs;
        x += bv[e];
        if (Rp) x += rv[e];
        if (p.act == GPV_ACT_RELU) x = fmaxf(x, 0.f);
        else if (p.act == GPV_ACT_GELU) x = gelu_erf(x);
        if (p.dthresh) x = ((keep8 >> e) & 1u) ? x * p.dscale : 0.f;
        if (Mp) x = mv[e] > 0.f ? x : 0.f;
        v[e] = x;
      }
      TOut* dst = Cp + mp * p.ldc + n;
      if (v_st && full) Ld8<TOut>::st(dst, v);
      else {
#pragma unroll
        for (int e = 0; e < 8; ++e)
          if (n + e < p.N) dst[e] = (TOut)v[e];
      }
    }
  }
}

template <int AMODE, int BM, int BN, int WM, int NS, typename TOut>
__global__ __launch_bounds__(NT) void pipe_kernel(GemmK p) {
  if (p.dthresh) p.seed = eff_seed(p.seed, p.seed_dev);
  pipe_body<AMODE, BM, BN, WM, NS, TOut>(p);
}
template <int BM, int BN, int WM, int NS, typename TOut>
__global__ __launch_bounds__(NT) void pipe_conv1x1_kernel(GemmK p) {
  if (p.dthresh) p.seed = eff_seed(p.seed, p.seed_dev);
  pipe_body<OP_PLAIN, BM, BN, WM, NS, TOut>(p);
}

template <int AMODE, int BM, int BN, int WM, int NS>
int launch_pipe(const GemmK& k, int batch, hipStream_t st) {
  constexpr size_t stages = (size_t)NS * (BM + BN) * ROWB;
  constexpr size_t lds = stages + (AMODE == OP_CONV ? (size_t)BM * 4 : 0);
  static_assert(lds <= 160 * 1024, "LDS budget");
  GemmK p = k;
  const int tilesM = (p.M + BM - 1) / BM;
  p.tilesN = (p.N + BN - 1) / BN;
  const bool c11 = AMODE == OP_PLAIN && p.conv1x1;
  void (*fn)(GemmK);
  if constexpr (AMODE == OP_PLAIN) fn = c11 ? pipe_conv1x1_kernel<BM, BN, WM, NS, bf16> : pipe_kernel<AMODE, BM, BN, WM, NS, bf16>;
  else fn = pipe_kernel<AMODE, BM, BN, WM, NS, bf16>;
  static bool attr_done[2] = {false, false};
  if (!attr_done[c11]) {
    hipError_t e = hipFuncSetAttribute(reinterpret_cast<const void*>(fn), hipFuncAttributeMaxDynamicSharedMemorySize, (int)lds);
    if (e != hipSuccess) { (void)hipGetLastError(); return (int)e; }
    attr_done[c11] = true;
  }
  dim3 grid(tilesM * p.tilesN, 1, batch);
  ++g_pipe_launches;
  static const int depi = tune_env("GPV_GLDS_DEPI", 1);
  p.depi = depi;
  hipLaunchKernelGGL(fn, grid, dim3(NT), lds, st, p);
  GPV_CHECK_LAUNCH();
  return 0;
}

struct PipeCfg { int bm, bn; };
constexpr PipeCfg kCfgs[] = {{256, 128}, {192, 128}, {128, 128}, {160, 256}, {128, 256}, {96, 256},
                             {64, 64}, {32, 64}};
constexpr int kNumBig = 6;
constexpr int kNumCfgs = sizeof(kCfgs) / sizeof(kCfgs[0]);

template <int AMODE>
int launch_cfg_idx(int idx, const GemmK& k, int batch, hipStream_t st) {
  switch (idx) {
    case 0: return launch_pipe<AMODE, 256, 128, 4, 3>(k, batch, st);
    case 1: return launch_pipe<AMODE, 192, 128, 4, 3>(k, batch, st);
    case 2: return launch_pipe<AMODE, 128, 128, 2, 3>(k, batch, st);
    case 3: return launch_pipe<AMODE, 160, 256, 2, 3>(k, batch, st);
    case 4: return launch_pipe<AMODE, 128, 256, 2, 3>(k, batch, st);
    case 5: return launch_pipe<AMODE, 96, 256, 2, 3>(k, batch, st);
  }
  if constexpr (AMODE == OP_PLAIN) {
    if (idx == 6) return launch_pipe<OP_PLAIN, 64, 64, 2, 6>(k, batch, st);
    if (idx == 7) return launch_pipe<OP_PLAIN, 32, 64, 2, 8>(k, batch, st);
  }
  return -1;
}

int g_pipe_small = tune_env("GPV_PIPE_SMALL", 1);
int g_pipe_mode = tune_env("GPV_PIPE", 1);

int pick_cfg(const GemmK& k, int batch) {
  double best = 1e300;
  int bi = -1;
  for (int i = 0; i < kNumBig; ++i) {
    const int bm = kCfgs[i].bm, bn = kCfgs[i].bn;
    if (k.N % bn != 0) continue;
    const int64_t tiles = (int64_t)((k.M + bm - 1) / bm) * (k.N / bn) * batch;
    const int64_t rounds = (tiles + 255) / 256;
    const double per_kt = (double)bm * bn / 16384.0 * 4.0 + (double)(bm + bn) * 128.0 / 56.0 / 16.0 * 0.5;
    const double cost = (double)rounds * (per_kt * (k.K / 64) + 40.0);
    if (cost < best - 1e-9) { best = cost; bi = i; }
  }
  return bi;
}

}

int pipe_try_launch(const GemmK& k, int amode, int dtype_in, int dtype_out, int batch, hipStream_t st) {
  const int mode = g_pipe_mode;
  if (mode == 0 || dtype_in != GPV_BF16 || dtype_out != GPV_BF16) return -1;
  if (k.accumulate || k.split_k > 1) return -1;
  if (k.K % GBK != 0 || k.K < 2 * GBK || k.N % 64 != 0) return -1;
  if (!al16(k.A) || !al16(k.B) || k.ldb % 8 != 0 || (batch > 1 && (k.sA % 8 != 0 || k.sB % 8 != 0))) return -1;
  const int64_t lim = 0x7ffffff0ll / 2;
  if ((int64_t)k.N * k.ldb >= lim) return -1;
  if (amode == OP_CONV) {
    if ((int64_t)k.cg.IH * k.cg.IW * k.cg.Cs * ((int64_t)k.M / ((int64_t)k.cg.OH * k.cg.OW) + 1) >= lim) return -1;
    if (k.cg.Cin % GBK != 0 || k.cg.Cs % 8 != 0) return -1;
  } else if (amode == OP_PLAIN) {
    if (k.lda % 8 != 0 || (int64_t)k.M * k.lda >= lim) return -1;
  } else {
    return -1;
  }
  if (mode < 100 && glds_two_per_cu(k, batch)) return -1;
  int idx;
  if (mode >= 100) {
    idx = mode - 100;
    if (idx >= kNumCfgs || k.N % kCfgs[idx].bn != 0 || (idx >= kNumBig && amode != OP_PLAIN)) return -1;
  } else if (g_pipe_small && !k.no_small && amode == OP_PLAIN && !k.conv1x1 && k.K >= 256 &&
             (int64_t)((k.M + 63) / 64) * (k.N / 64) * batch <= 250 &&
             ((int64_t)((k.M + 63) / 64) * (k.N / 64) * batch >= 100 || k.K <= 1024)) {
    const int64_t t64 = (int64_t)((k.M + 63) / 64) * (k.N / 64) * batch;
    idx = t64 < 128 ? 7 : 6;
  } else {
    if (k.K < 512 || k.M < 2048 || k.M > 40000 || k.N < 256) return -1;
    if (amode == OP_CONV && k.cg.cm) return -1;
    if (k.N >= 1024 && k.M >= 9600) return -1;
    if ((int64_t)k.M * k.N * batch > (int64_t)24 << 20) return -1;
    idx = pick_cfg(k, batch);
    if (idx < 0) return -1;
  }
  return amode == OP_CONV ? launch_cfg_idx<OP_CONV>(idx, k, batch, st) : launch_cfg_idx<OP_PLAIN>(idx, k, batch, st);
}

int pipe_set_mode(int v) { const int prev = g_pipe_mode; g_pipe_mode = v; return prev; }
int pipe_set_small(int v) { const int prev = g_pipe_small; g_pipe_small = v; return prev; }
long pipe_launches(long set) { const long prev = g_pipe_launches; if (set >= 0) g_pipe_launches = set; return prev; }

}
```

gpv-1_amd/csrc/gemm_skinny.hip:

```cpp
#include "gemm_common.h"

namespace gpvk {

int g_skinny_mode = 1;

namespace {

constexpr int SBM = 64, SBN = 64, SBK = 128, SPITCH = SBK + 8;
constexpr int TPITCH = SBN + 16;

__device__ __forceinline__ bf16x8 tr_frag(const bf16* tile, int cbase, int lane) {
  typedef short __attribute__((ext_vector_type(4))) s16x4;
  typedef __attribute__((address_space(3))) s16x4 lds_s16x4;
  const int g = lane >> 4, i = lane & 15;
  const bf16* p0 = tile + (8 * g + (i >> 2)) * TPITCH + cbase + (i & 3) * 4;
  s16x4 a = __builtin_amdgcn_ds_read_tr16_b64_v4i16((lds_s16x4*)(p0));
  s16x4 b = __builtin_amdgcn_ds_read_tr16_b64_v4i16((lds_s16x4*)(p0 + 4 * TPITCH));
  typedef short __attribute__((ext_vector_type(8))) s16x8;
  s16x8 r = {a[0], a[1], a[2], a[3], b[0], b[1], b[2], b[3]};
  return __builtin_bit_cast(bf16x8, r);
}

template <typename TOut, bool BT, int PF, int BM, int BN>
__global__ __launch_bounds__(256) void skinny_kernel(GemmK p) {
  static_assert(!BT || BN == 64, "reduction-major B tiles are [128][64]");
  if (p.dthresh) p.seed = eff_seed(p.seed, p.seed_dev);
  extern __shared__ __attribute__((aligned(16))) unsigned char smem[];
  bf16* lds = reinterpret_cast<bf16*>(smem);
  constexpr int FM = BM / 16, FN = BN / 16;
  constexpr int ATILE = BM * SPITCH;
  constexpr int BTILE = BT ? SBK * TPITCH : BN * SPITCH;
  constexpr int STAGE = ATILE + BTILE;
  constexpr int NB = BT ? 4 : FN;
  const int tid = threadIdx.x, lane = tid & 63, wave = tid >> 6;
  const int tn = blockIdx.x % p.tilesN, tm = blockIdx.x / p.tilesN;
  const int row0 = tm * BM, col0 = tn * BN;
// ... 290 lines not shown
      if (lane < 8 && m < p.M) atomicAdd(p.a_rowsum + m, v);
    }
  }
  float* red = reinterpret_cast<float*>(smem);
#pragma unroll
  for (int i = 0; i < 4; ++i)
#pragma unroll
    for (int j = 0; j < 4; ++j)
      *reinterpret_cast<f32x4*>(red + wave * (SBM * SBN) + (i * 4 + j) * 256 + lane * 4) = acc[i][j];
  __syncthreads();
  float* Cp = p.ws ? p.ws + (int64_t)blockIdx.y * p.M * p.N : reinterpret_cast<float*>(p.C);
  const int64_t ldc = p.ws ? p.N : p.ldc;
#pragma unroll
  for (int r = 0; r < 4; ++r) {
    const int q = tid + 256 * r;
    const int ij = q >> 6, l = q & 63;
    f32x4 v = *reinterpret_cast<const f32x4*>(red + ij * 256 + l * 4);
#pragma unroll
    for (int w = 1; w < 4; ++w) {
      const f32x4 u = *reinterpret_cast<const f32x4*>(red + w * (SBM * SBN) + ij * 256 + l * 4);
      v[0] += u[0]; v[1] += u[1]; v[2] += u[2]; v[3] += u[3];
    }
    const int m = row0 + (ij >> 2) * 16 + (l & 15);
    const int n = col0 + (ij & 3) * 16 + (l >> 4) * 4;
    if (m >= p.M || n >= p.N) continue;
    const float rs = p.rowscale ? p.rowscale[m] * p.alpha : p.alpha;
    float4* dst = reinterpret_cast<float4*>(Cp + (int64_t)m * ldc + n);
    float4 o = make_float4(v[0] * rs, v[1] * rs, v[2] * rs, v[3] * rs);
    if (!p.ws) { const float4 c = *dst; o.x += c.x; o.y += c.y; o.z += c.z; o.w += c.w; }
    *dst = o;
  }
}

}

int skinny_try_launch(const GemmK& k, int b_trans, int dtype_in, int dtype_out, int batch, hipStream_t st) {
  if (g_skinny_mode == 0 || dtype_in != GPV_BF16 || batch != 1 || k.accumulate || k.split_k > 1) return -1;
  if (k.K % 8 != 0 || k.lda % 8 != 0 || k.ldb % 8 != 0 || !al16(k.A) || !al16(k.B)) return -1;
  if (b_trans && k.N % 8 != 0) return -1;
  {
    const int64_t lim = 0x7ffffff0ll / 2;
    if ((int64_t)k.M * k.lda >= lim || (int64_t)(b_trans ? k.K : k.N) * k.ldb >= lim) return -1;
  }
  if (g_skinny_mode == 1) {
    const int64_t tiles = (int64_t)((k.M + SBM - 1) / SBM) * ((k.N + SBN - 1) / SBN);
    if (!((tiles <= 360 && k.K >= 128) || (b_trans && tiles <= 640 && k.K >= 2048))) return -1;
  }
  if (b_trans) return dtype_out == GPV_BF16 ? launch_skinny<bf16, true>(k, st) : launch_skinny<float, true>(k, st);
  return dtype_out == GPV_BF16 ? launch_skinny<bf16, false>(k, st) : launch_skinny<float, false>(k, st);
}

int skinny_tt_try_launch(const GemmK& k, int dtype_in, int dtype_out, int batch, hipStream_t st) {
  if (g_skinny_mode == 0 || dtype_in != GPV_BF16 || dtype_out != GPV_F32 || batch != 1 || !k.accumulate) return -1;
  if (k.M % 8 != 0 || k.N % 8 != 0 || k.lda % 8 != 0 || k.ldb % 8 != 0 || k.ldc % 4 != 0) return -1;
  if (!al16(k.A) || !al16(k.B) || !al16(k.C) || k.res || k.mask || k.bias || k.act || k.dthresh) return -1;
  if ((int64_t)k.K * k.lda >= 0x7ffffff0ll / 2 || (int64_t)k.K * k.ldb >= 0x7ffffff0ll / 2) return -1;
  const int64_t tiles = (int64_t)((k.M + SBM - 1) / SBM) * ((k.N + SBN - 1) / SBN);
  const int nk = (k.K + SBK - 1) / SBK;
  if (g_skinny_mode == 1 && (tiles > 256 || nk < 4)) return -1;
  int split = (int)((512 + tiles - 1) / tiles);
  if (split > nk / 3) split = nk / 3;
  if (split < 1) split = 1;
  while (split > 1 && (k.ws_base == nullptr || (int64_t)split * k.M * k.N * 4 > k.ws_bytes)) --split;
  GemmK p = k;
  p.tilesN = (p.N + SBN - 1) / SBN;
  p.kt_per_split = (nk + split - 1) / split;
  split = (nk + p.kt_per_split - 1) / p.kt_per_split;
  p.ws = split > 1 ? reinterpret_cast<float*>(k.ws_base) : nullptr;
  constexpr size_t stage = (size_t)2 * 2 * SBK * TPITCH * 2;
  constexpr size_t redb = (size_t)4 * SBM * SBN * 4;
  constexpr size_t lds = stage > redb ? stage : redb;
  static bool attr_done = false;
  if (!attr_done) {
    hipError_t e = hipFuncSetAttribute(reinterpret_cast<const void*>(skinny_tt_kernel), hipFuncAttributeMaxDynamicSharedMemorySize, (int)lds);
    if (e != hipSuccess) { (void)hipGetLastError(); return (int)e; }
    attr_done = true;
  }
  hipLaunchKernelGGL(skinny_tt_kernel, dim3((unsigned)tiles, split), dim3(256), lds, st, p);
  GPV_CHECK_LAUNCH();
  if (split > 1) return launch_splitk_reduce(p.ws, split, p.M, p.N, reinterpret_cast<float*>(p.C), p.ldc, st);
  return 0;
}
// ... 3 lines not shown
```

gpv-1_amd/csrc/misc.hip:

```cpp
#include "common.h"
#include <cstdlib>
#include "../../include/gpv_hip.h"

namespace {

inline int64_t cdiv(int64_t a, int64_t b) { return (a + b - 1) / b; }
inline int grid1d(int64_t n, int per_block) {
  int64_t g = cdiv(n, per_block);
  return (int)(g > 8192 ? 8192 : (g < 1 ? 1 : g));
}

template <bool HALF> __device__ __forceinline__ float row_sum(float v) {
  if (HALF) {
#pragma unroll
    for (int o = 16; o > 0; o >>= 1) v += __shfl_xor(v, o);
    return v;
  }
  return wave_sum(v);
}

template <typename T, int NV, bool HALF>
__global__ __launch_bounds__(256) void ln_fwd_kernel(const T* __restrict__ x, const T* __restrict__ s,
                                                     const float* __restrict__ gamma, const float* __restrict__ beta,
                                                     T* __restrict__ y, float* __restrict__ mean, float* __restrict__ rstd,
// ... 478 lines not shown
__global__ void relevance_condition_kernel(const T* __restrict__ x, const float* __restrict__ logits, const float* __restrict__ tok,
                                           T* __restrict__ y, int rows, int dim) {
  for (int64_t i = blockIdx.x * (int64_t)blockDim.x + threadIdx.x; i < (int64_t)rows * dim; i += (int64_t)gridDim.x * blockDim.x) {
    int64_t r = i / dim;
    int c = (int)(i - r * dim);
    float l0 = logits[r * 2], l1 = logits[r * 2 + 1];
    float m = fmaxf(l0, l1);
    float e0 = __expf(l0 - m), e1 = __expf(l1 - m);
    float p0 = e0 / (e0 + e1), p1 = e1 / (e0 + e1);
    y[i] = (T)((float)x[i] + p0 * tok[c] + p1 * tok[dim + c]);
  }
}

template <typename T>
__global__ void act_fwd_kernel(const T* __restrict__ x, T* __restrict__ y, int64_t n8, int act) {
  for (int64_t i = blockIdx.x * (int64_t)blockDim.x + threadIdx.x; i < n8; i += (int64_t)gridDim.x * blockDim.x) {
    float v[8];
    Ld8<T>::ld(x + i * 8, v);
#pragma unroll
    for (int e = 0; e < 8; ++e) v[e] = act == GPV_ACT_RELU ? fmaxf(v[e], 0.f) : gelu_erf(v[e]);
    Ld8<T>::st(y + i * 8, v);
  }
}
template <typename T>
__global__ void act_bwd_kernel(const T* __restrict__ dy, const T* __restrict__ ref, T* __restrict__ dx, int64_t n8, int act,
                               float alpha) {
  for (int64_t i = blockIdx.x * (int64_t)blockDim.x + threadIdx.x; i < n8; i += (int64_t)gridDim.x * blockDim.x) {
    float g[8], r[8];
    Ld8<T>::ld(dy + i * 8, g);
    Ld8<T>::ld(ref + i * 8, r);
#pragma unroll
    for (int e = 0; e < 8; ++e) {
      if (act == GPV_ACT_RELU) g[e] = r[e] > 0.f ? g[e] * alpha : 0.f;
      else {
        const float z = r[e];
        const float cdf = 0.5f * (1.0f + erff(z * 0.70710678118654752f));
        const float pdf = 0.3989422804014327f * __expf(-0.5f * z * z);
        g[e] = g[e] * (cdf + z * pdf) * alpha;
      }
    }
    Ld8<T>::st(dx + i * 8, g);
  }
}

__global__ void adamw_kernel(float* __restrict__ p, const float* __restrict__ g, float* __restrict__ m, float* __restrict__ v,
                             bf16* __restrict__ plow, int64_t n, float lr, float b1, float b2, float eps, float wd, float bc1,
                             float bc2, const float* __restrict__ gscale, const uint16_t* __restrict__ seg_id,
                             const int32_t* __restrict__ seg_live) {
  const float gs = gscale ? *gscale : 1.f;
  const float l1 = logf(b1), l2 = logf(b2);
  for (int64_t i = blockIdx.x * (int64_t)blockDim.x + threadIdx.x; i < n; i += (int64_t)gridDim.x * blockDim.x) {
    if (seg_id) {
      const int t = seg_live[seg_id[i >> 3]];
      if (!t) continue;
      bc1 = -expm1f((float)t * l1);
      bc2 = -expm1f((float)t * l2);
    }
    float gi = g[i] * gs;
    float pi = p[i] * (1.f - lr * wd);
    float mi = b1 * m[i] + (1.f - b1) * gi;
    float vi = b2 * v[i] + (1.f - b2) * gi * gi;
    m[i] = mi; v[i] = vi;
    float denom = sqrtf(vi) / sqrtf(bc2) + eps;
    pi -= (lr / bc1) * mi / denom;
    p[i] = pi;
    if (plow) plow[i] = (bf16)pi;
  }
}

template <bool NT>
__global__ __launch_bounds__(256) void adamw_vec4_kernel(float* __restrict__ p, const float* __restrict__ g, float* __restrict__ m,
                                                         float* __restrict__ v, bf16* __restrict__ plow, int64_t nquads, float lr, float b1,
// ... 432 lines not shown
```

gpv-1_amd/hip.py:

```python
import ctypes as C
import os
import threading

import torch

BF16, F32 = 0, 1
ACT_NONE, ACT_RELU, ACT_GELU = 0, 1, 2
KMAJOR, TRANS = 0, 1

_LIB = None
TUNING = os.environ.get('GPV_TUNING_LIB', '0') == '1'
_LIB_PATH = os.environ.get('GPV_HIP_LIB') or os.path.join(os.path.dirname(os.path.abspath(__file__)), 'csrc',
                                                          'libgpv_hip_tuning.so' if TUNING else 'libgpv_hip.so')


class GemmArgs(C.Structure):
    _fields_ = [('A', C.c_void_p), ('B', C.c_void_p), ('C', C.c_void_p),
                ('M', C.c_int), ('N', C.c_int), ('K', C.c_int), ('batch', C.c_int),
                ('lda', C.c_int64), ('ldb', C.c_int64), ('ldc', C.c_int64),
                ('sA', C.c_int64), ('sB', C.c_int64), ('sC', C.c_int64),
                ('layoutA', C.c_int), ('layoutB', C.c_int), ('dtype_in', C.c_int), ('dtype_out', C.c_int),
                ('alpha', C.c_float), ('rowscale', C.c_void_p), ('bias', C.c_void_p),
                ('res', C.c_void_p), ('ldr', C.c_int64), ('sR', C.c_int64),
                ('relu_mask', C.c_void_p), ('ldm', C.c_int64),
                ('act', C.c_int), ('drop_p', C.c_float), ('seed', C.c_uint64),
                ('accumulate', C.c_int), ('split_k', C.c_int), ('workspace', C.c_void_p), ('workspace_bytes', C.c_int64),
                ('a_rowsum', C.c_void_p), ('flags', C.c_int)]


class ConvArgs(C.Structure):
    _fields_ = [('mode', C.c_int), ('x', C.c_void_p), ('w', C.c_void_p), ('y', C.c_void_p),
                ('B', C.c_int), ('IH', C.c_int), ('IW', C.c_int), ('Cs', C.c_int), ('Cin', C.c_int),
                ('OH', C.c_int), ('OW', C.c_int), ('Cout', C.c_int),
                ('KH', C.c_int), ('KW', C.c_int), ('SH', C.c_int), ('SW', C.c_int), ('PH', C.c_int), ('PW', C.c_int),
                ('dtype_in', C.c_int), ('dtype_out', C.c_int),
                ('rowscale', C.c_void_p), ('bias', C.c_void_p), ('res', C.c_void_p), ('relu_mask', C.c_void_p),
                ('act', C.c_int), ('split_k', C.c_int), ('workspace', C.c_void_p), ('workspace_bytes', C.c_int64),
                ('y_mask_bits', C.c_void_p), ('relu_mask_bits', C.c_void_p)]


class AttnArgs(C.Structure):
    _fields_ = [('q', C.c_void_p), ('k', C.c_void_p), ('v', C.c_void_p), ('o', C.c_void_p),
                ('q_bs', C.c_int64), ('q_rs', C.c_int64), ('k_bs', C.c_int64), ('k_rs', C.c_int64),
                ('v_bs', C.c_int64), ('v_rs', C.c_int64), ('o_bs', C.c_int64), ('o_rs', C.c_int64),
                ('B', C.c_int), ('H', C.c_int), ('Sq', C.c_int), ('Sk', C.c_int), ('dh', C.c_int),
                ('scale', C.c_float), ('kpm', C.c_void_p), ('causal', C.c_int),
                ('drop_p', C.c_float), ('seed', C.c_uint64), ('lse', C.c_void_p), ('dtype', C.c_int),
                ('dout', C.c_void_p), ('do_bs', C.c_int64), ('do_rs', C.c_int64),
                ('dq', C.c_void_p), ('dk', C.c_void_p), ('dv', C.c_void_p)]


class TTProblem(C.Structure):
    _fields_ = [('A', C.c_void_p), ('B', C.c_void_p), ('C', C.c_void_p), ('a_rowsum', C.c_void_p),
                ('M', C.c_int), ('N', C.c_int), ('K', C.c_int), ('lda', C.c_int), ('ldb', C.c_int), ('ldc', C.c_int)]


class FoldProblem(C.Structure):
    _fields_ = [('partials', C.c_void_p), ('out0', C.c_void_p), ('out1', C.c_void_p), ('nblk', C.c_int), ('cols', C.c_int)]


# ... 24 lines not shown
def lib():
    global _LIB
    if _LIB is None:
        if not os.path.exists(_LIB_PATH):
            raise RuntimeError(
                f'gpv1_amd: HIP kernel library not found at {_LIB_PATH}. Build it with '
                f'`python -c "import __graft_entry__ as g; g.build()"` (make -C gpv-1_amd/csrc). '
                f'There is no CPU/eager fallback by design.')
        _LIB = C.CDLL(_LIB_PATH)
        _LIB.gpv_abi_version.restype = C.c_int
        if _LIB.gpv_abi_version() != 1:
            raise RuntimeError('gpv1_amd: libgpv_hip.so ABI version mismatch')
    return _LIB


EXPORTS = ['gpv_abi_version', 'gpv_build_id', 'gpv_set_option', 'gpv_gemm', 'gpv_conv2d', 'gpv_conv2d_mask_bits_ok', 'gpv_conv1x1_dual_bits', 'gpv_conv1x1_chain_bits', 'gpv_image_to_nhwc4', 'gpv_maxpool3x3s2',
           'gpv_attention_fwd', 'gpv_attention_bwd', 'gpv_attention_qkv_fwd', 'gpv_layernorm_fwd', 'gpv_layernorm_bwd', 'gpv_layernorm_pos_fwd', 'gpv_layernorm_bwd2', 'gpv_linear_layernorm_fwd',
           'gpv_softmax_ce', 'gpv_roi_weights', 'gpv_add', 'gpv_add_rowbcast', 'gpv_colsum', 'gpv_cast',
           'gpv_cast_rowscale_t', 'gpv_prep_conv_weight', 'gpv_embedding', 'gpv_dropout',
           'gpv_relevance_condition', 'gpv_adamw', 'gpv_sumsq', 'gpv_clip_scale', 'gpv_act_fwd', 'gpv_act_bwd', 'gpv_set_seed_device',
           'gpv_gemm_tt_group', 'gpv_gemm_tt_group_ws', 'gpv_cast_transpose_group', 'gpv_stem_pool', 'gpv_image_pipeline', 'gpv_conv1x1_dual', 'gpv_conv1x1_chain',
           'gpv_conv_wgrad_group', 'gpv_jpeg_parse', 'gpv_jpeg_decode', 'gpv_argmax_rows', 'gpv_ln_linear_rows', 'gpv_attention_row_proj',
           'gpv_layernorm_bwd_blocks', 'gpv_layernorm_bwd3', 'gpv_colsum_fold_group', 'gpv_argmax_rows_embed']


def build_id():
    buf = C.create_string_buffer(64)
    _chk(lib().gpv_build_id(buf, C.c_int(64)), 'gpv_build_id')
    return buf.value.decode()


OPT_GLDS, OPT_GLDS_LAUNCHES, OPT_SKINNY, OPT_GLDS_WGRAD, OPT_PIPE, OPT_PIPE_LAUNCHES, OPT_C1S, OPT_C3S, OPT_C3S_LAUNCHES = 0, 1, 2, 3, 4, 5, 6, 7, 8
OPT_GEMV, OPT_GEMV_LAUNCHES = 9, 10
OPT_ATTN_BWD1, OPT_ATTN_BWD1_LAUNCHES, OPT_C1S_LAUNCHES, OPT_WG8, OPT_WG8_LAUNCHES, OPT_W8L, OPT_PIPE_SMALL, OPT_WG8H, OPT_C3_HALO, OPT_C3_HALO_LAUNCHES = 11, 12, 13, 14, 15, 16, 17, 18, 19, 20


GEMM_NO_PIPE_SMALL = 2
_TL = threading.local()


class gemm_flags:

    def __init__(self, flags):
        self.flags = flags

    def __enter__(self):
        self.prev = getattr(_TL, 'gemm_flags', 0)
        _TL.gemm_flags = self.prev | self.flags
        return self

    def __exit__(self, *exc):
        _TL.gemm_flags = self.prev
        return False


_OPT_SET = {}


def set_option(option, value):
    _OPT_SET[option] = value
    return lib().gpv_set_option(C.c_int(option), C.c_int(value))


def get_option_cached(option):
    return _OPT_SET.get(option)


class option:

    def __init__(self, opt, value):
# ... 44 lines not shown
    return C.c_void_p(torch.cuda.current_stream().cuda_stream)


def _chk(err, what):
    if err != 0:
        raise RuntimeError(f'gpv1_amd: {what} failed with hipError {err}')


def _f32(t):
    if t is not None and t.dtype != torch.float32:
        raise TypeError('expected fp32 tensor')
    return t


_WS = {}
WS_MAX = 256 << 20
_WS_RETIRED = []


def _workspace(device, nbytes):
    need = min(nbytes, WS_MAX)
    key = (device, _raw_stream(torch.cuda.current_device()) if _raw_stream is not None else 0)
    ws = _WS.get(key)
    if ws is None or ws.numel() < need:
        if ws is not None:
            _WS_RETIRED.append(ws)
            need = max(need, min(2 * ws.numel(), WS_MAX))
        ws = _WS[key] = torch.empty(max(need, 64 << 20), device=device, dtype=torch.uint8)
    return ws


def gemm(A, B, Cm, M, N, K, lda, ldb, ldc, layoutA=KMAJOR, layoutB=KMAJOR, batch=1, sA=0, sB=0, sC=0,
         alpha=1.0, rowscale=None, bias=None, res=None, ldr=0, sR=0, relu_mask=None, ldm=0, act=ACT_NONE,
         drop_p=0.0, seed=0, accumulate=False, split_k=1, a_rowsum=None, kpad_finite=False):
    a = GemmArgs()
    a.A, a.B, a.C = _p(A), _p(B), _p(Cm)
    a.M, a.N, a.K, a.batch = M, N, K, batch
    a.lda, a.ldb, a.ldc, a.sA, a.sB, a.sC = lda, ldb, ldc, sA, sB, sC
    a.layoutA, a.layoutB = layoutA, layoutB
    if A.dtype != B.dtype:
        raise TypeError('gemm: A and B dtypes differ')
    a.dtype_in, a.dtype_out = dcode(A), dcode(Cm)
    a.alpha = alpha
    if rowscale is not None or bias is not None:
        check_epilogue_extents('gemm', M, N, rowscale, bias)
    a.rowscale, a.bias = _p(_f32(rowscale)), _p(_f32(bias))
    if res is not None and res.dtype != Cm.dtype:
        raise TypeError('gemm: residual dtype must equal output dtype')
    if relu_mask is not None and relu_mask.dtype != Cm.dtype:
        raise TypeError('gemm: mask dtype must equal output dtype')
    a.res, a.ldr, a.sR = _p(res), ldr, sR
    a.relu_mask, a.ldm = _p(relu_mask), ldm
    a.act, a.drop_p, a.seed = act, drop_p, seed
    a.accumulate, a.split_k = int(accumulate), split_k
    a.a_rowsum = _p(_f32(a_rowsum))
    a.flags = (1 if kpad_finite else 0) | getattr(_TL, 'gemm_flags', 0)
    if accumulate and batch == 1:
        ws = _workspace(A.device, max(max(split_k, 8) * M * N * 4, 512 * 128 * 128 * 4))
        a.workspace, a.workspace_bytes = _p(ws), ws.numel()
    _chk(lib().gpv_gemm(C.byref(a), _stream()), 'gpv_gemm')


def tt_group_ok(dy, x, dw, M, N, K, lda, ldb, ldc):
    return (dy.dtype == torch.bfloat16 and x.dtype == torch.bfloat16 and dw.dtype == torch.float32 and M % 128 == 0 and N % 128 == 0
            and lda % 8 == 0 and ldb % 8 == 0 and ldc % 4 == 0 and dy.data_ptr() % 16 == 0 and x.data_ptr() % 16 == 0
            and dw.data_ptr() % 16 == 0 and K * max(lda, ldb) < (1 << 30))


def gemm_tt_group(problems):
    if not problems:
        return
    problems = sorted(problems, key=lambda q: -q[6])
    arr = (TTProblem * len(problems))()
    for i, (dy, x, dw, bg, M, N, K, lda, ldb, ldc) in enumerate(problems):
        a = arr[i]
        a.A, a.B, a.C, a.a_rowsum = dy.data_ptr(), x.data_ptr(), dw.data_ptr(), (bg.data_ptr() if bg is not None else None)
        a.M, a.N, a.K, a.lda, a.ldb, a.ldc = M, N, K, lda, ldb, ldc
    if _OPT_SET.get(OPT_W8L, 0) or os.environ.get('GPV_W8L', '0') not in ('', '0'):
        ws = _workspace(problems[0][0].device, WS_MAX)
        _chk(lib().gpv_gemm_tt_group_ws(arr, C.c_int(len(problems)), _p(ws), C.c_int64(ws.numel()), _stream()), 'gpv_gemm_tt_group_ws')
    else:
        _chk(lib().gpv_gemm_tt_group_ws(arr, C.c_int(len(problems)), None, C.c_int64(0), _stream()), 'gpv_gemm_tt_group_ws')


def check_epilogue_extents(what, rows, cols, rowscale, bias):
    if rowscale is not None and rowscale.numel() < rows:
        raise ValueError('%s: rowscale has %d elements, the epilogue indexes it by output row: %d needed' % (what, rowscale.numel(), rows))
    if bias is not None and bias.numel() < cols:
        raise ValueError('%s: bias has %d elements, the epilogue indexes it by output column: %d needed' % (what, bias.numel(), cols))
# ... 426 lines not shown
```

gpv-1_amd/ops.py:

```python
import math

import os
import weakref

import torch
from torch.autograd import Function

from . import hip

ACT_NONE, ACT_RELU, ACT_GELU = hip.ACT_NONE, hip.ACT_RELU, hip.ACT_GELU


class Runtime:
    def __init__(self):
        self.dtype = torch.bfloat16
        self.weights_epoch = 0
        self.static_epoch = 0
        self.seed = 0x5EED
        self.seed_explicit = False
        self._ctr = 0
        self.cache = {}
        self.backward_milestone = None
        self.split = None
        self.seed_dev = None
# ... 828 lines not shown
    def backward(ctx, dy, dy2=None):
        nin = 10
        if dy is None and dy2 is None:
            return (None,) * nin
        x2, s2, mean, rstd, a2 = ctx.saved_tensors
        rows, cols = x2.shape
        if dy2 is not None:
            _pos_sink(ctx.pos_param, _c(_as_compute(dy2)).reshape(rows, cols), rows, cols)
        d1, d2 = _two_grads(dy, dy2, rows, cols)
        dx = torch.empty_like(x2)
        ds = torch.empty_like(x2) if ctx.drop_p > 0 else None
        _ln_backward(d1, d2, x2, s2, ctx.gamma, ctx.beta, mean, rstd, dx, ds, rows, cols, ctx.drop_p, ctx.seed)
        dxr = dx.reshape(ctx.shape)
        if ctx.chain is not None and ctx.needs_input_grad[0]:
            ch = ctx.chain
            if ch.acc is not None:
                t = torch.empty_like(dx)
                hip.add(dx, _c(ch.acc).reshape(rows, cols), t, t.numel())
                dxr = t.reshape(ctx.shape)
            elif ds is None:
                dxr = dxr.clone()
            dxr = ch.done(dxr)
        da = _linear_backward(ctx.w, a2, ds if ds is not None else dx, None, ctx.needs_input_grad[1], ctx.ashape)
        return ((dxr if ctx.needs_input_grad[0] else None), da) + (None,) * (nin - 2)


def proj_add_layernorm(x, a, w, gamma, beta, eps, drop_p=0.0, chain=None, pos=None, pos_param=None):
    return ProjAddLayerNormFn.apply(x, a, w, gamma, beta, eps, drop_p, chain, pos, pos_param)


FFN_FUSED = os.environ.get('GPV_FFN_FUSED', '0') == '1'


class FFNBlockFn(Function):

    @staticmethod
    def forward(ctx, x, w1, w2, gamma, beta, eps, drop_p, pos=None, pos_param=None):
        ctx.set_materialize_grads(False)
        K, Fh = w1.K, w1.N
        x2 = _c(_as_compute(x)).reshape(-1, K)
        M = x2.shape[0]
        h = torch.empty(M, Fh, device=x.device, dtype=RT.dtype)
        seed1 = RT.next_seed() if drop_p > 0 else 0
        y = torch.empty(M, K, device=x.device, dtype=RT.dtype)
        out = torch.empty_like(x2)
        mean = torch.empty(M, device=x.device, dtype=torch.float32)
        rstd = torch.empty_like(mean)
        seed2 = RT.next_seed() if drop_p > 0 else 0
        p2 = None if pos is None else _pos_rows(pos, K)
        out2 = None if pos is None else torch.empty_like(x2)
        if not (FFN_FUSED and RT.dtype == torch.bfloat16 and w1.bias is not None and w2.bias is not None and
                hip.ffn_fused_fwd(x2, w1.lp(), w1.bias_f32(), w2.lp(), w2.bias_f32(), gamma.detach(), beta.detach(), h, y, out, mean, rstd,
                                  M, K, Fh, eps, drop_p, seed1, seed2, pos=p2, out2=out2)):
            hip.gemm(x2, w1.lp(), h, M, Fh, K, K, K, Fh, bias=w1.bias_f32(), act=ACT_RELU, drop_p=drop_p, seed=seed1)
            hip.gemm(h, w2.lp(), y, M, K, Fh, Fh, Fh, K, bias=w2.bias_f32())
            hip.layernorm_fwd(x2, y, gamma.detach(), beta.detach(), out, mean, rstd, M, K, eps, drop_p, seed2, pos=p2, y2=out2)
        ctx.w1, ctx.w2, ctx.gamma, ctx.beta, ctx.drop_p, ctx.seed2, ctx.xshape = w1, w2, gamma, beta, drop_p, seed2, x.shape
        ctx.pos_param = pos_param
        ctx.save_for_backward(x2, h, y, mean, rstd)
        if pos is None:
            return out.reshape(x.shape)
        return out.reshape(x.shape), out2.reshape(x.shape)

    @staticmethod
    def backward(ctx, dout, dout2=None):
        nin = 9
        if dout is None and dout2 is None:
            return (None,) * nin
        w1, w2, gamma, beta = ctx.w1, ctx.w2, ctx.gamma, ctx.beta
        x2, h, y, mean, rstd = ctx.saved_tensors
        M, K = x2.shape
        Fh = w1.N
        if dout2 is not None:
            _pos_sink(ctx.pos_param, _c(_as_compute(dout2)).reshape(M, K), M, K)
        d2, d2b = _two_grads(dout, dout2, M, K)
        dx_res = torch.empty_like(x2)
        ds = torch.empty_like(x2) if ctx.drop_p > 0 else None
        _ln_backward(d2, d2b, x2, y, gamma, beta, mean, rstd, dx_res, ds, M, K, ctx.drop_p, ctx.seed2)
        dy2 = ds if ds is not None else dx_res
        nb2 = w2.bias is not None and w2.bias.requires_grad
        if w2.weight.requires_grad:
            wgrad_linear(dy2, h, w2.wgrad(), w2.bgrad() if nb2 else None, K, Fh, M, _split_k(K, Fh, M))
        elif nb2:
            hip.colsum(dy2, w2.bgrad(), M, K, K)
        dz = torch.empty(M, Fh, device=d2.device, dtype=RT.dtype)
        w2.dx_gemm(dy2, dz, M, relu_mask=h, ldm=Fh, alpha=1.0 / (1.0 - ctx.drop_p) if ctx.drop_p > 0 else 1.0)
        nb1 = w1.bias is not None and w1.bias.requires_grad
        if w1.weight.requires_grad:
            wgrad_linear(dz, x2, w1.wgrad(), w1.bgrad() if nb1 else None, Fh, K, M, _split_k(Fh, K, M))
        elif nb1:
            hip.colsum(dz, w1.bgrad(), M, Fh, Fh)
        dx = torch.empty(M, K, device=dz.device, dtype=RT.dtype)
        w1.dx_gemm(dz, dx, M, res=dx_res, ldr=K)
        return (dx.reshape(ctx.xshape),) + (None,) * (nin - 1)


LN_POS = os.environ.get('GPV_LN_POS', '1') != '0'


def _unfused_pos(y, pos, pos_param=None):
    if pos_param is not None and pos_param.requires_grad and torch.is_grad_enabled():
        raise RuntimeError('GPV_LN_POS=0 is a timing switch: it drops the gradient of the learned position term (query_embed); '
                           'not available while that parameter trains')
    cols = y.shape[-1]
    return y, add(y, _pos_rows(pos, cols))


def ffn_block(x, w1, w2, gamma, beta, eps, drop_p=0.0, pos=None, pos_param=None):
    if pos is not None and not LN_POS:
        return _unfused_pos(ffn_block(x, w1, w2, gamma, beta, eps, drop_p), pos, pos_param)
    if not (torch.is_grad_enabled() and x.requires_grad):
        return add_layernorm(x, linear(linear(x, w1, ACT_RELU, drop_p), w2), gamma, beta, eps, drop_p, pos=pos, pos_param=pos_param)
    return FFNBlockFn.apply(x, w1, w2, gamma, beta, eps, drop_p, pos, pos_param)


def add_layernorm(x, s, gamma, beta, eps, drop_p=0.0, chain=None, pos=None, pos_param=None):
    if pos is not None and not LN_POS:
        return _unfused_pos(AddLayerNormFn.apply(x, s, gamma, beta, eps, drop_p, chain, None, None), pos, pos_param)
    return AddLayerNormFn.apply(x, s, gamma, beta, eps, drop_p, chain, pos, pos_param)


class AttentionFn(Function):

    @staticmethod
    def forward(ctx, meta, *bufs):
        roles, B, H, Sq, Sk, dh, kpm, causal, drop_p = meta[:9]
        D = H * dh
        bufs = tuple(_c(_as_compute(b)) for b in bufs)
        (qi, qo), (ki, ko), (vi, vo) = roles
        qb, kb, vb = bufs[qi], bufs[ki], bufs[vi]
        o = torch.empty(B * Sq, D, device=qb.device, dtype=RT.dtype)
        lse = torch.empty(B, H, Sq, device=qb.device, dtype=torch.float32)
        st = ((Sq * qb.shape[1], qb.shape[1]), (Sk * kb.shape[1], kb.shape[1]), (Sk * vb.shape[1], vb.shape[1]), (Sq * D, D))
        seed = RT.next_seed() if drop_p > 0 else 0
        scale = 1.0 / math.sqrt(dh)
        hip.attention_fwd(qb[:, qo:], kb[:, ko:], vb[:, vo:], o, st, B, H, Sq, Sk, dh, scale, kpm=kpm, causal=causal,
                          drop_p=drop_p, seed=seed, lse=lse)
        ctx.meta, ctx.seed, ctx.st, ctx.scale = meta, seed, st, scale
        ctx.save_for_backward(o, lse, *bufs)
        return o

    @staticmethod
    def backward(ctx, do):
        roles, B, H, Sq, Sk, dh, kpm, causal, drop_p = ctx.meta[:9]
        sinks = ctx.meta[9] if len(ctx.meta) > 9 and ctx.meta[9] is not None else (None,) * (len(ctx.saved_tensors) - 2)
        D = H * dh
# ... 117 lines not shown
    @staticmethod
    def backward(ctx, dy):
        return None, None


def embedding(table, ids):
    return EmbeddingFn.apply(table, ids)


class RelevanceConditionFn(Function):

    @staticmethod
    def forward(ctx, x, logits, tokens):
        x2 = _c(_as_compute(x))
        lg = _c(logits.float())
        y = torch.empty_like(x2)
        hip.relevance_condition(x2, lg, tokens.detach(), y, x2.shape[0], x2.shape[1])
        ctx.tokens = tokens
        ctx.save_for_backward(lg)
        return y

    @staticmethod
    def backward(ctx, dy):
        (lg,) = ctx.saved_tensors
        tokens = ctx.tokens
        rows, D = dy.shape
        dyc = _c(_as_compute(dy))
        p = lg.softmax(-1)
        tok_lp = _as_compute(tokens.detach())
        dp = torch.empty(rows, 2, device=dy.device, dtype=torch.float32)
        hip.gemm(dyc, tok_lp, dp, rows, 2, D, D, D, 2)
        if tokens.requires_grad:
            hip.gemm(_as_compute(p), dyc, ensure_grad(tokens), 2, D, rows, 2, D, D, layoutA=hip.TRANS, layoutB=hip.TRANS,
                     accumulate=True, split_k=_split_k(2, D, rows))
        dlg = p * (dp - (p * dp).sum(-1, keepdim=True))
        return (dy if ctx.needs_input_grad[0] else None), (dlg if ctx.needs_input_grad[1] else None), None


def relevance_condition(x, logits, tokens):
    return RelevanceConditionFn.apply(x, logits, tokens)


class SoftmaxCEFn(Function):

    @staticmethod
    def forward(ctx, logits, target):
        lg = _c(logits)
        rows, V = lg.shape
        loss = torch.empty(rows, device=lg.device, dtype=torch.float32)
        hip.softmax_ce(lg, V, _c(target), loss, None, None, rows, V)
        ctx.save_for_backward(lg, target)
        return loss

    @staticmethod
    def backward(ctx, dloss):
        lg, target = ctx.saved_tensors
        rows, V = lg.shape
        dl = torch.empty_like(lg)
        scratch = torch.empty(rows, device=lg.device, dtype=torch.float32)
        hip.softmax_ce(lg, V, _c(target), scratch, dl, _c(dloss.float()), rows, V)
        return dl, None


def softmax_ce(logits, target):
    return SoftmaxCEFn.apply(logits, target)


# ... 31 lines not shown
```

gpv-1_amd/vilbert.py:

```python
import os

import torch
import torch.nn as nn

from . import ops
from .ops import W
from .transformer import LinearP, LayerNormP

FUSE_QKV = os.environ.get('GPV_COATT_QKV', '1') != '0'


class BertBiAttention(nn.Module):
    def __init__(self, cfg):
        super().__init__()
        if cfg.bi_hidden_size % cfg.bi_num_attention_heads != 0:
            raise ValueError('bi_hidden_size must be a multiple of bi_num_attention_heads')
        self.num_attention_heads = cfg.bi_num_attention_heads
        self.attention_head_size = cfg.bi_hidden_size // cfg.bi_num_attention_heads
        self.all_head_size = cfg.bi_hidden_size
        self.query1 = LinearP(cfg.v_hidden_size, self.all_head_size)
        self.key1 = LinearP(cfg.v_hidden_size, self.all_head_size)
        self.value1 = LinearP(cfg.v_hidden_size, self.all_head_size)
        self.query2 = LinearP(cfg.hidden_size, self.all_head_size)
        self.key2 = LinearP(cfg.hidden_size, self.all_head_size)
# ... 49 lines not shown

class _Intermediate(nn.Module):
    def __init__(self, hidden, inter, act):
        super().__init__()
        if act != 'gelu':
            raise NotImplementedError('GPV-1 configs use hidden_act: gelu')
        self.dense = LinearP(hidden, inter)

    def forward(self, x, chain=None):
        return self.dense(x, ops.ACT_GELU, chain=chain)


class _Output(nn.Module):
    def __init__(self, inter, hidden, p):
        super().__init__()
        self.dense = LinearP(inter, hidden)
        self.LayerNorm = LayerNormP(hidden, eps=1e-12)
        self.p = p

    def forward(self, h, inp, chain=None):
        return self.LayerNorm(inp, self.dense(h), self.p if self.training else 0.0, chain=chain)


class BertConnectionLayer(nn.Module):
    def __init__(self, cfg):
        super().__init__()
        self.biattention = BertBiAttention(cfg)
        self.biOutput = BertBiOutput(cfg)
        self.v_intermediate = _Intermediate(cfg.v_hidden_size, cfg.v_intermediate_size, cfg.v_hidden_act)
        self.v_output = _Output(cfg.v_intermediate_size, cfg.v_hidden_size, cfg.v_hidden_dropout_prob)
        self.t_intermediate = _Intermediate(cfg.hidden_size, cfg.intermediate_size, cfg.hidden_act)
        self.t_output = _Output(cfg.intermediate_size, cfg.hidden_size, cfg.hidden_dropout_prob)

    def forward(self, t1, t2, B, T1, T2, kpm1=None):
        c1, c2 = ops.grad_chain(t1), ops.grad_chain(t2)
        br = ops.branch_for(t1) if (FUSE_QKV and t1.shape[-1] == t2.shape[-1]) else None
        bi1, bi2 = self.biattention(t1, t2, B, T1, T2, c1, c2, kpm1, branch=br)
        bo = self.biOutput
        if br is None:
            a1, a2 = bo(bi2, t1, bi1, t2, c1, c2)
            ca1, ca2 = ops.grad_chain(a1), ops.grad_chain(a2)
            o1 = self.v_output(self.v_intermediate(a1, ca1), a1, ca1)
            o2 = self.t_output(self.t_intermediate(a2, ca2), a2, ca2)
            return o1, o2
        br.fork()
        with br.on():
            a1 = bo.LayerNorm1(t1, bo.dense1(bi2), bo.p1 if bo.training else 0.0, chain=c1)
        a2 = bo.LayerNorm2(t2, bo.dense2(bi1), bo.p2 if bo.training else 0.0, chain=c2)
        ca1, ca2 = ops.grad_chain(a1), ops.grad_chain(a2)
        with br.on():
            o1 = self.v_output(self.v_intermediate(a1, ca1), a1, ca1)
        o2 = self.t_output(self.t_intermediate(a2, ca2), a2, ca2)
        br.join()
        return o1, o2
```

include/gpv_hip.h:

```cpp
#ifndef GPV_HIP_H
#define GPV_HIP_H
#include <stdint.h>
#ifdef __cplusplus
extern "C" {
#endif

#define GPV_BF16 0
#define GPV_F32 1

#define GPV_ACT_NONE 0
#define GPV_ACT_RELU 1
#define GPV_ACT_GELU 2

#define GPV_KMAJOR 0
#define GPV_TRANS 1

int gpv_abi_version(void);
int gpv_build_id(char* buf, int cap);

#define GPV_TT_GROUP_MAX 48
typedef struct {
  const void* A; const void* B; float* C; float* a_rowsum;
  int M, N, K;
  int lda, ldb, ldc;
} gpv_tt_problem;
int gpv_gemm_tt_group(const gpv_tt_problem* problems, int n, void* stream);
int gpv_gemm_tt_group_ws(const gpv_tt_problem* problems, int n, void* workspace, int64_t workspace_bytes, void* stream);

#define GPV_OPT_GLDS 0
#define GPV_OPT_SKINNY 2
#define GPV_OPT_GLDS_LAUNCHES 1
#define GPV_OPT_GLDS_WGRAD 3
#define GPV_OPT_PIPE 4
#define GPV_OPT_C1S 6
#define GPV_OPT_C3S 7
#define GPV_OPT_C3S_LAUNCHES 8
#define GPV_OPT_GEMV 9
#define GPV_OPT_GEMV_LAUNCHES 10
#define GPV_OPT_PIPE_LAUNCHES 5
#define GPV_OPT_ATTN_BWD1 11
#define GPV_OPT_ATTN_BWD1_LAUNCHES 12
#define GPV_OPT_WG8 14
#define GPV_OPT_WG8_LAUNCHES 15
#define GPV_OPT_PIPE_SMALL 17
#define GPV_OPT_WG8H 18
#define GPV_OPT_C3_HALO 19
#define GPV_OPT_C3_HALO_LAUNCHES 20
#define GPV_OPT_W8L 16
#define GPV_OPT_C1S_LAUNCHES 13
int gpv_set_option(int option, int value);

typedef struct {
  const void* A; const void* B; void* C;
  int M, N, K, batch;
  int64_t lda, ldb, ldc;
  int64_t sA, sB, sC;
  int layoutA, layoutB;
  int dtype_in, dtype_out;
  float alpha;
  const float* rowscale;
  const float* bias;
  const void* res; int64_t ldr, sR;
  const void* relu_mask; int64_t ldm;
  int act;
  float drop_p; uint64_t seed;
  int accumulate, split_k;
  void* workspace; int64_t workspace_bytes;
  float* a_rowsum;
  int flags;
} gpv_gemm_args;
#define GPV_GEMM_KPAD_FINITE 1
#define GPV_GEMM_NO_PIPE_SMALL 2
int gpv_gemm(const gpv_gemm_args* a, void* stream);

typedef struct {
  int mode;
  const void* x; const void* w; void* y;
  int B, IH, IW, Cs, Cin;
  int OH, OW, Cout;
  int KH, KW, SH, SW, PH, PW;
  int dtype_in, dtype_out;
  const float* rowscale; const float* bias;
  const void* res; const void* relu_mask;
  int act;
  int split_k;
  void* workspace; int64_t workspace_bytes;
  void* y_mask_bits; const void* relu_mask_bits;
} gpv_conv_args;
int gpv_conv2d(const gpv_conv_args* a, void* stream);
int gpv_conv2d_mask_bits_ok(const gpv_conv_args* a);

typedef struct gpv_conv_wgrad_problem {
  const void* x; const void* dy; float* dw; const float* rowscale;
  int B, IH, IW, Cs, Cin, OH, OW, Cout, KH, KW, SH, SW, PH, PW;
} gpv_conv_wgrad_problem;
int gpv_conv_wgrad_group(const gpv_conv_wgrad_problem* problems, int n, void* workspace, int64_t workspace_bytes, void* stream);

int gpv_image_to_nhwc4(const float* img, void* out, int B, int H, int W, int pad, int Hp, int Wp,
                       int dtype_out, void* stream);
int gpv_maxpool3x3s2(const void* x, void* y, int B, int H, int W, int C, int OH, int OW, int dtype,
                     void* stream);
typedef struct gpv_image_desc {
  const unsigned char* src;
  int H, W;
// ... 144 lines not shown
```

Before: 2175 images/sec.

## Fuse GELU FFN with pre-activation output, add bit-packed ReLU masks and tt-rows wgrad

Adds a fused GELU FFN autograd path for the co-attention layers. The first GEMM writes the pre-activation alongside the GELU output, and the backward dx GEMM applies the GELU derivative in its epilogue instead of running separate elementwise kernels. It also routes ReLU FFN masks through bit-packed masks in the streaming 1x1 kernel, adds a new tt-rows accumulate wgrad launcher, and disables split-k for a small token GEMM in bf16. These cut memory traffic and kernel launches, at the cost of extra pre-activation storage and more kernel variants.

```diff
diff --git a/gpv-1_amd/csrc/common.h b/gpv-1_amd/csrc/common.h
--- a/gpv-1_amd/csrc/common.h
+++ b/gpv-1_amd/csrc/common.h
@@ -130,6 +130,11 @@
 }
 
 __device__ __forceinline__ float gelu_erf(float x) { return 0.5f * x * (1.0f + erff(x * 0.70710678118654752f)); }
+__device__ __forceinline__ float gelu_erf_grad(float z) {
+  const float cdf = 0.5f * (1.0f + erff(z * 0.70710678118654752f));
+  const float pdf = 0.3989422804014327f * __expf(-0.5f * z * z);
+  return cdf + z * pdf;
+}
 
 template <typename T> struct Ld8;
 template <> struct Ld8<bf16> {
diff --git a/gpv-1_amd/csrc/conv1x1_stream.hip b/gpv-1_amd/csrc/conv1x1_stream.hip
--- a/gpv-1_amd/csrc/conv1x1_stream.hip
+++ b/gpv-1_amd/csrc/conv1x1_stream.hip
@@ -186,7 +186,8 @@
               if constexpr (RES) x += (float)rv[t][e];
               if (p.act == GPV_ACT_RELU) x = fmaxf(x, 0.f);
               x *= p.dscale;
-              if constexpr (MASK) x = (float)mv[t][e] > 0.f ? x : 0.f;
+              if constexpr (MASK && BITS) x = ((mw[t >> 2] >> ((t & 3) * 8 + e)) & 1u) ? x : 0.f;
+              else if constexpr (MASK) x = (float)mv[t][e] > 0.f ? x : 0.f;
               o[e] = (bf16)x;
             }
             u32x4 ow = __builtin_bit_cast(u32x4, o);
@@ -266,6 +267,8 @@
   if (linear || k.alpha != 1.0f || k.dthresh) {
     if constexpr (K == 256 && NH == 256) {
       if (nt) return -1;
+      if (k.out_bits) return (r || m) ? -1 : c1s_launch<K, NH, false, false, false, true, true>(k, st);
+      if (k.mask_bits) return r ? -1 : c1s_launch<K, NH, false, true, false, true, true>(k, st);
       if (r && m) return c1s_launch<K, NH, true, true, false, true>(k, st);
       if (r) return c1s_launch<K, NH, true, false, false, true>(k, st);
       if (m) return c1s_launch<K, NH, false, true, false, true>(k, st);
@@ -313,7 +316,8 @@
 
 int c1s_try_launch(const GemmK& k, int dtype_in, int dtype_out, hipStream_t st, bool linear, bool dry) {
   static const int env = tune_env("GPV_C1S", -1);
-  const int mode = env >= 0 ? env : g_c1s_mode;
+  const bool lin_bits = linear && (k.mask_bits || k.out_bits);
+  const int mode = lin_bits ? 2 : (env >= 0 ? env : g_c1s_mode);
   if (mode == 0 || dtype_in != GPV_BF16 || dtype_out != GPV_BF16) return -1;
   if (k.K != 64 && k.K != 128 && k.K != 256 && k.K != 512) return -1;
   if (k.N != 64 && k.N != 128 && k.N != 256 && k.N != 512 && k.N != 1024 && k.N != 2048 && !(linear && k.N % 256 == 0 && k.N <= 2048)) return -1;
@@ -328,7 +332,11 @@
   if (linear) {
     if (mode == 1 && (k.K != 256 || k.N < 1536 || k.M < 2048)) return -1;
   } else if (mode == 1 && ((int64_t)k.M * nsl < 65536 || k.M < 32768)) return -1;
-  if (k.mask_bits || k.out_bits) {
+  if (lin_bits) {
+    if (k.K != 256 || k.N % 256 != 0 || k.res || (k.mask_bits && k.out_bits)) return -1;
+    if (k.out_bits && (k.act != GPV_ACT_RELU || k.mask)) return -1;
+    if (k.mask_bits && k.dthresh) return -1;
+  } else if (k.mask_bits || k.out_bits) {
     const int nh = ncols >= 256 ? 256 : ncols;
     const bool inst = ((k.K == 128 || k.K == 256) && nh == 256) || (k.K == 512 && nh == 128 && !k.out_bits);
     if (linear || !inst || !k.res || k.nt_io || (k.mask_bits && k.out_bits) || k.N % 256 != 0 || (k.out_bits && (k.mask && !k.mask_bits))) return -1;
diff --git a/gpv-1_amd/csrc/gemm.hip b/gpv-1_amd/csrc/gemm.hip
--- a/gpv-1_amd/csrc/gemm.hip
+++ b/gpv-1_amd/csrc/gemm.hip
@@ -315,7 +315,7 @@
   }
 };
 
-template <typename TIn, typename TOut, int AMODE, int BMODE, int BM, int BN, bool VEC, bool NTIO = false>
+template <typename TIn, typename TOut, int AMODE, int BMODE, int BM, int BN, bool VEC, bool NTIO = false, bool PA = false>
 __device__ __forceinline__ void gemm_body(const GemmK& p) {
   constexpr bool PRECISE = sizeof(TIn) == 4;
   constexpr int FM = BM / 32, FN = BN / 32;
@@ -523,6 +523,8 @@
   const bool v_st = (ldc % 8 == 0) && ((reinterpret_cast<uintptr_t>(Cp) & 15) == 0);
   const bool v_res = Rp && (p.ldr % 8 == 0) && ((reinterpret_cast<uintptr_t>(Rp) & 15) == 0);
   const bool v_msk = Mp && (p.ldm % 8 == 0) && ((reinterpret_cast<uintptr_t>(Mp) & 15) == 0);
+  TOut* Pp = PA ? reinterpret_cast<TOut*>(p.pre) : nullptr;
+  const bool v_pre = PA && Pp && (p.ldp % 8 == 0) && ((reinterpret_cast<uintptr_t>(Pp) & 15) == 0);
   float bv[8];
   {
     const int nb = col0 + (tid % CH) * 8;
@@ -595,18 +597,34 @@
         const float rs = p.rowscale ? p.rowscale[m] * p.alpha : p.alpha;
         const bool full = n + 8 <= p.N;
         const uint32_t keep8 = p.dthresh ? drop_mask<8>(p.seed, ((uint64_t)batch * p.M + m) * (uint64_t)p.N + n, p.dthresh) : 0xffu;
+        float pv[PA ? 8 : 1];
 #pragma unroll
         for (int e = 0; e < 8; ++e) {
           float x = v[e] * rs;
           x += bv[e];
           if (Rp) x += rv[g][e];
+          if constexpr (PA) {
+            if (Pp) { x = (float)(TOut)x; pv[e] = x; }
+          }
           if (p.act == GPV_ACT_RELU) x = fmaxf(x, 0.f);
           else if (p.act == GPV_ACT_GELU) x = gelu_erf(x);
           if (p.dthresh) x = ((keep8 >> e) & 1u) ? x * p.dscale : 0.f;
-          if (Mp) x = mv[g][e] > 0.f ? x : 0.f;
+          if (PA && p.mask_preact) x = (float)(TOut)x * gelu_erf_grad(mv[g][e]);
+          else if (Mp) x = mv[g][e] > 0.f ? x : 0.f;
           v[e] = x;
         }
         const int64_t mp = (AMODE == OP_CONV && p.cg.cm && m < p.M) ? s_rowpix[m - row0] : m;
+        if constexpr (PA) {
+          if (Pp) {
+            TOut* pdst = Pp + mp * p.ldp + n;
+            if (v_pre && full) Ld8<TOut>::st(pdst, pv);
+            else {
+#pragma unroll
+              for (int e = 0; e < 8; ++e)
+                if (n + e < p.N) pdst[e] = (TOut)pv[e];
+            }
+          }
+        }
         TOut* dst = Cp + mp * ldc + n;
         if (v_st && full) { if constexpr (NTIO) Ld8<TOut>::st_nt(dst, v); else Ld8<TOut>::st(dst, v); }
         else {
@@ -623,6 +641,10 @@
 __global__ __launch_bounds__(256) void gemm_kernel(GemmK p) {
   if (p.dthresh) p.seed = eff_seed(p.seed, p.seed_dev);
   gemm_body<TIn, TOut, AMODE, BMODE, BM, BN, VEC>(p);
+}
+template <typename TIn, typename TOut, int BMODE, int BM, int BN, bool VEC>
+__global__ __launch_bounds__(256) void gemm_pa_kernel(GemmK p) {
+  gemm_body<TIn, TOut, OP_PLAIN, BMODE, BM, BN, VEC, false, true>(p);
 }
 template <typename TIn, typename TOut, int BM, int BN, bool VEC>
 __global__ __launch_bounds__(256) void conv1x1_kernel(GemmK p) {
@@ -714,6 +736,10 @@
     p.accumulate = 0; p.res = nullptr; p.mask = nullptr; p.bias = nullptr; p.act = 0; p.dthresh = 0;
   }
   auto fn = gemm_kernel<TIn, TOut, AMODE, BMODE, BM, BN, VEC>;
+  if (wants_pa(k)) {
+    if constexpr (AMODE == OP_PLAIN && BMODE != OP_CONV) fn = gemm_pa_kernel<TIn, TOut, BMODE, BM, BN, VEC>;
+    else return (int)hipErrorInvalidValue;
+  }
   if constexpr (AMODE == OP_PLAIN && BMODE == OP_PLAIN) {
     if (k.conv1x1) fn = conv1x1_kernel<TIn, TOut, BM, BN, VEC>;
     if constexpr (std::is_same<TIn, bf16>::value && std::is_same<TOut, bf16>::value && VEC) {
@@ -865,6 +891,13 @@
   k.dscale = a->drop_p > 0.f ? 1.0f / (1.0f - a->drop_p) : 1.0f;
   k.accumulate = a->accumulate; k.split_k = a->split_k;
   k.a_rowsum = a->a_rowsum;
+  k.pre = a->pre_act; k.ldp = a->ldp;
+  k.mask_preact = (a->flags & GPV_GEMM_MASK_IS_PREACT) ? 1 : 0;
+  if (wants_pa(k)) {
+    if (a->batch != 1 || a->accumulate || a->split_k > 1 || a->drop_p > 0.f || a->layoutA != GPV_KMAJOR) return (int)hipErrorInvalidValue;
+    if (k.pre && (a->act == GPV_ACT_NONE || a->ldp < a->N)) return (int)hipErrorInvalidValue;
+    if (k.mask_preact && (!a->relu_mask || a->act != GPV_ACT_NONE || k.pre)) return (int)hipErrorInvalidValue;
+  }
   k.no_small = (a->flags & GPV_GEMM_NO_PIPE_SMALL) ? 1 : 0;
   k.ws_base = a->workspace; k.ws_bytes = a->workspace ? a->workspace_bytes : 0;
   if (k.a_rowsum && !(a->layoutA == GPV_TRANS && a->layoutB == GPV_TRANS && a->batch == 1)) return (int)hipErrorInvalidValue;
@@ -888,24 +921,36 @@
   }
   hipStream_t st = reinterpret_cast<hipStream_t>(stream);
   const int la = a->layoutA, lb = a->layoutB;
+  if (a->y_mask_bits || a->relu_mask_bits) {
+    if (la != GPV_KMAJOR || lb != GPV_KMAJOR || a->batch != 1 || wants_pa(k) || a->accumulate || a->split_k > 1 || !k.vecA || !k.vecB) return (int)hipErrorInvalidValue;
+    if (a->y_mask_bits && (a->relu_mask_bits || a->relu_mask || a->act != GPV_ACT_RELU)) return (int)hipErrorInvalidValue;
+    if (a->relu_mask_bits && (a->relu_mask || a->drop_p > 0.f)) return (int)hipErrorInvalidValue;
+    if ((reinterpret_cast<uintptr_t>(a->y_mask_bits) | reinterpret_cast<uintptr_t>(a->relu_mask_bits)) & 15) return (int)hipErrorInvalidValue;
+    k.out_bits = reinterpret_cast<uint32_t*>(a->y_mask_bits);
+    k.mask_bits = reinterpret_cast<const uint32_t*>(a->relu_mask_bits);
+    if (k.mask_bits) { k.mask = a->relu_mask_bits; k.ldm = a->N; }
+    const int cs = c1s_try_launch(k, a->dtype_in, a->dtype_out, st, true);
+    return cs >= 0 ? cs : (int)hipErrorInvalidValue;
+  }
+  const bool pa = wants_pa(k);
   if (la == GPV_KMAJOR && lb == GPV_KMAJOR) {
-    const int gv = gemv_try_launch(k, a->dtype_in, a->dtype_out, a->batch, st);
+    const int gv = pa ? -1 : gemv_try_launch(k, a->dtype_in, a->dtype_out, a->batch, st);
     if (gv >= 0) return gv;
     static const bool c1s_linear = tune_env("GPV_C1S_LINEAR", 1) != 0;
-    if (a->batch == 1 && !g_kernel_forced && c1s_linear) {
+    if (a->batch == 1 && !g_kernel_forced && c1s_linear && !pa) {
       const int cs = c1s_try_launch(k, a->dtype_in, a->dtype_out, st, true);
       if (cs >= 0) return cs;
     }
     const int pp = pipe_try_launch(k, OP_PLAIN, a->dtype_in, a->dtype_out, a->batch, st);
     if (pp >= 0) return pp;
-    const int sk = skinny_try_launch(k, 0, a->dtype_in, a->dtype_out, a->batch, st);
+    const int sk = pa ? -1 : skinny_try_launch(k, 0, a->dtype_in, a->dtype_out, a->batch, st);
     if (sk >= 0) return sk;
     const int g = glds_try_launch(k, OP_PLAIN, a->dtype_in, a->dtype_out, a->batch, st);
     if (g >= 0) return g;
     return launch_dtype<OP_PLAIN, OP_PLAIN>(k, a->batch, a->dtype_in, a->dtype_out, st);
   }
   if (la == GPV_KMAJOR && lb == GPV_TRANS) {
-    const int sk = skinny_try_launch(k, 1, a->dtype_in, a->dtype_out, a->batch, st);
+    const int sk = pa ? -1 : skinny_try_launch(k, 1, a->dtype_in, a->dtype_out, a->batch, st);
     if (sk >= 0) return sk;
     return launch_dtype<OP_PLAIN, OP_TRANS>(k, a->batch, a->dtype_in, a->dtype_out, st);
   }
@@ -913,6 +958,8 @@
     if (a->accumulate) {
       GemmK kk = k;
       kk.accumulate = 1; kk.res = nullptr; kk.ldr = 0; kk.sR = 0;
+      const int tr = tt_rows_try_launch(kk, a->dtype_in, a->dtype_out, a->batch, st);
+      if (tr >= 0) return tr;
       const int gt = glds_tt_try_launch(kk, a->dtype_in, a->dtype_out, a->batch, st);
       if (gt >= 0) return gt;
       const int sk = skinny_tt_try_launch(kk, a->dtype_in, a->dtype_out, a->batch, st);
diff --git a/gpv-1_amd/csrc/gemm_common.h b/gpv-1_amd/csrc/gemm_common.h
--- a/gpv-1_amd/csrc/gemm_common.h
+++ b/gpv-1_amd/csrc/gemm_common.h
@@ -33,7 +33,10 @@
   uint32_t* out_bits;
   float* a_rowsum;
   ConvGeom cg;
+  void* pre; int64_t ldp;
+  int mask_preact;
 };
+inline bool wants_pa(const GemmK& k) { return k.pre != nullptr || k.mask_preact != 0; }
 
 __device__ __forceinline__ int conv_row_to_pixel(int m, const ConvGeom& g) {
   if (!g.cm) return m;
@@ -94,6 +97,8 @@
 
 int launch_splitk_reduce(const float* ws, int split, int M, int N, float* C, int64_t ldc, hipStream_t st);
 int skinny_tt_try_launch(const GemmK& k, int dtype_in, int dtype_out, int batch, hipStream_t st);
+int tt_rows_try_launch(const GemmK& k, int dtype_in, int dtype_out, int batch, hipStream_t st);
+extern long g_tt_rows_launches;
 
 int glds_wgrad_try_launch(const GemmK& k, int dtype_in, int dtype_out, hipStream_t st);
 int glds_tt_try_launch(const GemmK& k, int dtype_in, int dtype_out, int batch, hipStream_t st);
diff --git a/gpv-1_amd/csrc/gemm_glds.hip b/gpv-1_amd/csrc/gemm_glds.hip
--- a/gpv-1_amd/csrc/gemm_glds.hip
+++ b/gpv-1_amd/csrc/gemm_glds.hip
@@ -13,7 +13,7 @@
 typedef __attribute__((address_space(3))) void lds_void_t;
 typedef const __attribute__((address_space(1))) void glb_void_t;
 
-template <int AMODE, int BM, int BN, typename TOut>
+template <int AMODE, int BM, int BN, typename TOut, bool PA = false>
 __device__ __forceinline__ void glds_body(const GemmK& p) {
   constexpr int NT = BM == 256 ? 512 : 256, NW = NT / 64;
   constexpr int WN = BN / 64, WM = NW / WN;
@@ -109,7 +109,8 @@
                     ((reinterpret_cast<uintptr_t>(p.C) | (uintptr_t)(p.sC * 2)) & 15) == 0 &&
                     (!p.res || (p.ldr % 8 == 0 && ((reinterpret_cast<uintptr_t>(p.res) | (uintptr_t)(p.sR * 2)) & 15) == 0)) &&
                     (!p.mask || (p.ldm % 8 == 0 && (reinterpret_cast<uintptr_t>(p.mask) & 15) == 0)) &&
-                    (!p.bias || (reinterpret_cast<uintptr_t>(p.bias) & 15) == 0);
+                    (!p.bias || (reinterpret_cast<uintptr_t>(p.bias) & 15) == 0) &&
+                    (!PA || !p.pre || (p.ldp % 8 == 0 && (reinterpret_cast<uintptr_t>(p.pre) & 15) == 0));
 #pragma unroll
   for (int j = 0; j < BI; ++j) {
     const int r = wave * (BI * 8) + j * 8 + lrow;
@@ -209,6 +210,8 @@
   const bool v_st = (p.ldc % 8 == 0) && ((reinterpret_cast<uintptr_t>(Cp) & 15) == 0);
   const bool v_res = Rp && (p.ldr % 8 == 0) && ((reinterpret_cast<uintptr_t>(Rp) & 15) == 0);
   const bool v_msk = Mp && (p.ldm % 8 == 0) && ((reinterpret_cast<uintptr_t>(Mp) & 15) == 0);
+  TOut* Pp = PA ? reinterpret_cast<TOut*>(p.pre) : nullptr;
+  const bool v_pre = PA && Pp && (p.ldp % 8 == 0) && ((reinterpret_cast<uintptr_t>(Pp) & 15) == 0);
   if (depi) {
     const int mrow = wm * WTM + frow;
     float bq[2][8];
@@ -260,16 +263,24 @@
               const uint32_t keep8 = p.dthresh ? drop_mask<8>(p.seed, ((uint64_t)batch * p.M + mc) * (uint64_t)p.N + n, p.dthresh) : 0xffu;
               float v[8] = {acc[i][2 * t][0], acc[i][2 * t][1], acc[i][2 * t][2], acc[i][2 * t][3],
                             acc[i][2 * t + 1][0], acc[i][2 * t + 1][1], acc[i][2 * t + 1][2], acc[i][2 * t + 1][3]};
+              float pv[PA ? 8 : 1];
 #pragma unroll
               for (int e = 0; e < 8; ++e) {
                 float x = v[e] * rs;
                 x += bq[t][e];
                 if (Rp) x += (float)rraw[ii][t][e];
+                if constexpr (PA) {
+                  if (Pp) { x = (float)(TOut)x; pv[e] = x; }
+                }
                 if (p.act == GPV_ACT_RELU) x = fmaxf(x, 0.f);
                 else if (p.act == GPV_ACT_GELU) x = gelu_erf(x);
                 if (p.dthresh) x = ((keep8 >> e) & 1u) ? x * p.dscale : 0.f;
-                if (Mp) x = (float)mraw[ii][t][e] > 0.f ? x : 0.f;
+                if (PA && p.mask_preact) x = (float)(TOut)x * gelu_erf_grad((float)mraw[ii][t][e]);
+                else if (Mp) x = (float)mraw[ii][t][e] > 0.f ? x : 0.f;
                 v[e] = x;
+              }
+              if constexpr (PA) {
+                if (Pp && m < p.M) Ld8<TOut>::st(Pp + mpv[ii] * p.ldp + n, pv);
               }
               if (m < p.M) Ld8<TOut>::st(Cp + mpv[ii] * p.ldc + n, v);
             }
@@ -337,16 +348,32 @@
       }
       const float rs = p.rowscale ? p.rowscale[m] * p.alpha : p.alpha;
       const uint32_t keep8 = p.dthresh ? drop_mask<8>(p.seed, ((uint64_t)batch * p.M + m) * (uint64_t)p.N + n, p.dthresh) : 0xffu;
+      float pv[PA ? 8 : 1];
 #pragma unroll
       for (int e = 0; e < 8; ++e) {
         float x = v[e] * rs;
         x += bv[e];
         if (Rp) x += rv[e];
+        if constexpr (PA) {
+          if (Pp) { x = (float)(TOut)x; pv[e] = x; }
+        }
         if (p.act == GPV_ACT_RELU) x = fmaxf(x, 0.f);
         else if (p.act == GPV_ACT_GELU) x = gelu_erf(x);
         if (p.dthresh) x = ((keep8 >> e) & 1u) ? x * p.dscale : 0.f;
-        if (Mp) x = mv[e] > 0.f ? x : 0.f;
+        if (PA && p.mask_preact) x = (float)(TOut)x * gelu_erf_grad(mv[e]);
+        else if (Mp) x = mv[e] > 0.f ? x : 0.f;
         v[e] = x;
+      }
+      if constexpr (PA) {
+        if (Pp) {
+          TOut* pdst = Pp + mp * p.ldp + n;
+          if (v_pre && full) Ld8<TOut>::st(pdst, pv);
+          else {
+#pragma unroll
+            for (int e = 0; e < 8; ++e)
+              if (n + e < p.N) pdst[e] = (TOut)pv[e];
+          }
+        }
       }
       TOut* dst = Cp + mp * p.ldc + n;
       if (v_st && full) Ld8<TOut>::st(dst, v);
@@ -572,6 +599,30 @@
   glds_body<OP_PLAIN, BM, BN, TOut>(p);
 }
 
+__global__ __launch_bounds__(256) void glds_pa_kernel(GemmK p) {
+  glds_body<OP_PLAIN, 160, 128, bf16, true>(p);
+}
+int launch_glds_pa(const GemmK& k, hipStream_t st) {
+  constexpr int BM = 160, BN = 128;
+  constexpr size_t lds = (size_t)2 * (BM + BN) * ROWB;
+  static_assert(lds >= (size_t)(BM / 2) * (BN + 4) * 4, "epilogue image fits the stages");
+  GemmK p = k;
+  const int tilesM = (p.M + BM - 1) / BM;
+  p.tilesN = (p.N + BN - 1) / BN;
+  static bool attr_done = false;
+  if (!attr_done) {
+    hipError_t e = hipFuncSetAttribute(reinterpret_cast<const void*>(glds_pa_kernel), hipFuncAttributeMaxDynamicSharedMemorySize, (int)lds);
+    if (e != hipSuccess) { (void)hipGetLastError(); return (int)e; }
+    attr_done = true;
+  }
+  static const int depi = tune_env("GPV_GLDS_DEPI", 1);
+  p.depi = depi;
+  ++g_glds_launches;
+  hipLaunchKernelGGL(glds_pa_kernel, dim3(tilesM * p.tilesN, 1, 1), dim3(256), lds, st, p);
+  GPV_CHECK_LAUNCH();
+  return 0;
+}
+
 template <int AMODE, int BM, int BN, typename TOut>
 int launch_glds(const GemmK& k, int batch, hipStream_t st) {
   constexpr size_t stage = (size_t)2 * (BM + BN) * ROWB;
@@ -628,6 +679,12 @@
   } else {
     return -1;
   }
+  if (wants_pa(k)) {
+    if (amode != OP_PLAIN || dtype_out != GPV_BF16 || batch != 1) return -1;
+    const bool natural = glds_two_per_cu(k, batch) && two_per_cu_bm(k, batch) == 160;
+    if (!natural && mode != 2 && mode != 3) return -1;
+    return launch_glds_pa(k, st);
+  }
   if (glds_two_per_cu(k, batch) && mode != 2 && mode != 3) {
     const int bm2 = two_per_cu_bm(k, batch);
     if (amode == OP_CONV && halo_ok(k, dtype_out, batch)) {
@@ -740,6 +797,11 @@
     gpvk::g_halo_launches = value;
     return (int)prev;
   }
+  if (option == GPV_OPT_TT_ROWS_LAUNCHES) {
+    const long prev = gpvk::g_tt_rows_launches;
+    gpvk::g_tt_rows_launches = value;
+    return (int)prev;
+  }
   if (option == GPV_OPT_GLDS_LAUNCHES) {
     const long prev = gpvk::g_glds_launches;
     gpvk::g_glds_launches = value;
diff --git a/gpv-1_amd/csrc/gemm_pipe.hip b/gpv-1_amd/csrc/gemm_pipe.hip
--- a/gpv-1_amd/csrc/gemm_pipe.hip
+++ b/gpv-1_amd/csrc/gemm_pipe.hip
@@ -41,7 +41,7 @@
   }
 }
 
-template <int AMODE, int BM, int BN, int WM, int NS, typename TOut>
+template <int AMODE, int BM, int BN, int WM, int NS, typename TOut, bool EPA = false>
 __device__ __forceinline__ void pipe_body(const GemmK& p) {
   constexpr int WN = NW / WM;
   constexpr bool SWP = GPV_PIPE_SWP != 0 && (BM / WM / 16 + BN / (NW / WM) / 16) * 8 + (BM / WM / 16) * (BN / (NW / WM) / 16) * 4 <= 200;
@@ -119,7 +119,8 @@
                     ((reinterpret_cast<uintptr_t>(p.C) | (uintptr_t)(p.sC * 2)) & 15) == 0 &&
                     (!p.res || (p.ldr % 8 == 0 && ((reinterpret_cast<uintptr_t>(p.res) | (uintptr_t)(p.sR * 2)) & 15) == 0)) &&
                     (!p.mask || (p.ldm % 8 == 0 && (reinterpret_cast<uintptr_t>(p.mask) & 15) == 0)) &&
-                    (!p.bias || (reinterpret_cast<uintptr_t>(p.bias) & 15) == 0);
+                    (!p.bias || (reinterpret_cast<uintptr_t>(p.bias) & 15) == 0) &&
+                    (!EPA || !p.pre || (p.ldp % 8 == 0 && (reinterpret_cast<uintptr_t>(p.pre) & 15) == 0));
 #pragma unroll
   for (int j = 0; j < BI; ++j) {
     const int r = (j * NW + wave) * 8 + lrow;
@@ -263,6 +264,8 @@
   const bool v_st = (p.ldc % 8 == 0) && ((reinterpret_cast<uintptr_t>(Cp) & 15) == 0);
   const bool v_res = Rp && (p.ldr % 8 == 0) && ((reinterpret_cast<uintptr_t>(Rp) & 15) == 0);
   const bool v_msk = Mp && (p.ldm % 8 == 0) && ((reinterpret_cast<uintptr_t>(Mp) & 15) == 0);
+  TOut* Pp = EPA ? reinterpret_cast<TOut*>(p.pre) : nullptr;
+  const bool v_pre = EPA && Pp && (p.ldp % 8 == 0) && ((reinterpret_cast<uintptr_t>(Pp) & 15) == 0);
   if constexpr (FN % 2 == 0) {
     if (depi) {
       const int mrow = wm * WTM + frow;
@@ -283,16 +286,24 @@
           const uint32_t keep8 = p.dthresh ? drop_mask<8>(p.seed, ((uint64_t)batch * p.M + m) * (uint64_t)p.N + n, p.dthresh) : 0xffu;
           float v[8] = {acc[i][2 * t][0], acc[i][2 * t][1], acc[i][2 * t][2], acc[i][2 * t][3],
                         acc[i][2 * t + 1][0], acc[i][2 * t + 1][1], acc[i][2 * t + 1][2], acc[i][2 * t + 1][3]};
+          float pv[EPA ? 8 : 1];
 #pragma unroll
           for (int e = 0; e < 8; ++e) {
             float x = v[e] * rs;
             x += bq[e];
             if (Rp) x += rv[e];
+            if constexpr (EPA) {
+              if (Pp) { x = (float)(TOut)x; pv[e] = x; }
+            }
             if (p.act == GPV_ACT_RELU) x = fmaxf(x, 0.f);
             else if (p.act == GPV_ACT_GELU) x = gelu_erf(x);
             if (p.dthresh) x = ((keep8 >> e) & 1u) ? x * p.dscale : 0.f;
-            if (Mp) x = mv[e] > 0.f ? x : 0.f;
+            if (EPA && p.mask_preact) x = (float)(TOut)x * gelu_erf_grad(mv[e]);
+            else if (Mp) x = mv[e] > 0.f ? x : 0.f;
             v[e] = x;
+          }
+          if constexpr (EPA) {
+            if (Pp) Ld8<TOut>::st(Pp + mp * p.ldp + n, pv);
           }
           Ld8<TOut>::st(Cp + mp * p.ldc + n, v);
         }
@@ -359,16 +370,32 @@
       }
       const float rs = p.rowscale ? p.rowscale[m] * p.alpha : p.alpha;
       const uint32_t keep8 = p.dthresh ? drop_mask<8>(p.seed, ((uint64_t)batch * p.M + m) * (uint64_t)p.N + n, p.dthresh) : 0xffu;
+      float pv[EPA ? 8 : 1];
 #pragma unroll
       for (int e = 0; e < 8; ++e) {
         float x = v[e] * rs;
         x += bv[e];
         if (Rp) x += rv[e];
+        if constexpr (EPA) {
+          if (Pp) { x = (float)(TOut)x; pv[e] = x; }
+        }
         if (p.act == GPV_ACT_RELU) x = fmaxf(x, 0.f);
         else if (p.act == GPV_ACT_GELU) x = gelu_erf(x);
         if (p.dthresh) x = ((keep8 >> e) & 1u) ? x * p.dscale : 0.f;
-        if (Mp) x = mv[e] > 0.f ? x : 0.f;
+        if (EPA && p.mask_preact) x = (float)(TOut)x * gelu_erf_grad(mv[e]);
+        else if (Mp) x = mv[e] > 0.f ? x : 0.f;
         v[e] = x;
+      }
+      if constexpr (EPA) {
+        if (Pp) {
+          TOut* pdst = Pp + mp * p.ldp + n;
+          if (v_pre && full) Ld8<TOut>::st(pdst, pv);
+          else {
+#pragma unroll
+            for (int e = 0; e < 8; ++e)
+              if (n + e < p.N) pdst[e] = (TOut)pv[e];
+          }
+        }
       }
       TOut* dst = Cp + mp * p.ldc + n;
       if (v_st && full) Ld8<TOut>::st(dst, v);
@@ -392,7 +419,12 @@
   pipe_body<OP_PLAIN, BM, BN, WM, NS, TOut>(p);
 }
 
-template <int AMODE, int BM, int BN, int WM, int NS>
+template <int BM, int BN, int WM, int NS>
+__global__ __launch_bounds__(NT) void pipe_pa_kernel(GemmK p) {
+  pipe_body<OP_PLAIN, BM, BN, WM, NS, bf16, true>(p);
+}
+
+template <int AMODE, int BM, int BN, int WM, int NS, bool EPA = false>
 int launch_pipe(const GemmK& k, int batch, hipStream_t st) {
   constexpr size_t stages = (size_t)NS * (BM + BN) * ROWB;
   constexpr size_t lds = stages + (AMODE == OP_CONV ? (size_t)BM * 4 : 0);
@@ -402,7 +434,8 @@
   p.tilesN = (p.N + BN - 1) / BN;
   const bool c11 = AMODE == OP_PLAIN && p.conv1x1;
   void (*fn)(GemmK);
-  if constexpr (AMODE == OP_PLAIN) fn = c11 ? pipe_conv1x1_kernel<BM, BN, WM, NS, bf16> : pipe_kernel<AMODE, BM, BN, WM, NS, bf16>;
+  if constexpr (EPA) fn = pipe_pa_kernel<BM, BN, WM, NS>;
+  else if constexpr (AMODE == OP_PLAIN) fn = c11 ? pipe_conv1x1_kernel<BM, BN, WM, NS, bf16> : pipe_kernel<AMODE, BM, BN, WM, NS, bf16>;
   else fn = pipe_kernel<AMODE, BM, BN, WM, NS, bf16>;
   static bool attr_done[2] = {false, false};
   if (!attr_done[c11]) {
@@ -424,6 +457,14 @@
                              {64, 64}, {32, 64}};
 constexpr int kNumBig = 6;
 constexpr int kNumCfgs = sizeof(kCfgs) / sizeof(kCfgs[0]);
+
+inline bool pa_cfg(int idx) { return idx == 2 || idx == 6 || idx == 7; }
+int launch_cfg_pa(int idx, const GemmK& k, int batch, hipStream_t st) {
+  if (idx == 2) return launch_pipe<OP_PLAIN, 128, 128, 2, 3, true>(k, batch, st);
+  if (idx == 6) return launch_pipe<OP_PLAIN, 64, 64, 2, 6, true>(k, batch, st);
+  if (idx == 7) return launch_pipe<OP_PLAIN, 32, 64, 2, 8, true>(k, batch, st);
+  return -1;
+}
 
 template <int AMODE>
 int launch_cfg_idx(int idx, const GemmK& k, int batch, hipStream_t st) {
@@ -478,11 +519,14 @@
   } else {
     return -1;
   }
+  const bool pa = wants_pa(k);
+  if (pa && (amode != OP_PLAIN || batch != 1)) return -1;
   if (mode < 100 && glds_two_per_cu(k, batch)) return -1;
   int idx;
   if (mode >= 100) {
     idx = mode - 100;
     if (idx >= kNumCfgs || k.N % kCfgs[idx].bn != 0 || (idx >= kNumBig && amode != OP_PLAIN)) return -1;
+    if (pa && !pa_cfg(idx)) return -1;
   } else if (g_pipe_small && !k.no_small && amode == OP_PLAIN && !k.conv1x1 && k.K >= 256 &&
              (int64_t)((k.M + 63) / 64) * (k.N / 64) * batch <= 250 &&
              ((int64_t)((k.M + 63) / 64) * (k.N / 64) * batch >= 100 || k.K <= 1024)) {
@@ -494,8 +538,10 @@
     if (k.N >= 1024 && k.M >= 9600) return -1;
     if ((int64_t)k.M * k.N * batch > (int64_t)24 << 20) return -1;
     idx = pick_cfg(k, batch);
+    if (pa) idx = k.N % 128 == 0 ? 2 : -1;
     if (idx < 0) return -1;
   }
+  if (pa) return launch_cfg_pa(idx, k, batch, st);
   return amode == OP_CONV ? launch_cfg_idx<OP_CONV>(idx, k, batch, st) : launch_cfg_idx<OP_PLAIN>(idx, k, batch, st);
 }
 
diff --git a/gpv-1_amd/csrc/gemm_skinny.hip b/gpv-1_amd/csrc/gemm_skinny.hip
--- a/gpv-1_amd/csrc/gemm_skinny.hip
+++ b/gpv-1_amd/csrc/gemm_skinny.hip
@@ -2,6 +2,7 @@
 
 namespace gpvk {
 
+long g_tt_rows_launches = 0;
 int g_skinny_mode = 1;
 
 namespace {
@@ -358,6 +359,39 @@
   }
 }
 
+__global__ __launch_bounds__(256) void tt_rows_kernel(const bf16* __restrict__ A, int64_t lda, const bf16* __restrict__ B, int64_t ldb, int M, int N,
+                                                      int K, int rows_per_slab, float alpha, float* __restrict__ ws) {
+  const int c8 = blockIdx.x * 256 + threadIdx.x;
+  if (c8 * 8 >= N) return;
+  const int s = blockIdx.y;
+  const int r0 = s * rows_per_slab, r1 = min(K, r0 + rows_per_slab);
+  float acc[8][8];
+#pragma unroll
+  for (int m = 0; m < 8; ++m)
+#pragma unroll
+    for (int e = 0; e < 8; ++e) acc[m][e] = 0.f;
+  for (int r = r0; r < r1; ++r) {
+    const bf16x8 b = *reinterpret_cast<const bf16x8*>(B + (int64_t)r * ldb + c8 * 8);
+    const bf16* ar = A + (int64_t)r * lda;
+#pragma unroll
+    for (int m = 0; m < 8; ++m) {
+      if (m < M) {
+        const float a = (float)ar[m];
+#pragma unroll
+        for (int e = 0; e < 8; ++e) acc[m][e] = fmaf(a, (float)b[e], acc[m][e]);
+      }
+    }
+  }
+#pragma unroll
+  for (int m = 0; m < 8; ++m) {
+    if (m < M) {
+      float* dst = ws + ((int64_t)s * M + m) * N + c8 * 8;
+      *reinterpret_cast<float4*>(dst) = make_float4(acc[m][0] * alpha, acc[m][1] * alpha, acc[m][2] * alpha, acc[m][3] * alpha);
+      *reinterpret_cast<float4*>(dst + 4) = make_float4(acc[m][4] * alpha, acc[m][5] * alpha, acc[m][6] * alpha, acc[m][7] * alpha);
+    }
+  }
+}
+
 }
 
 int skinny_try_launch(const GemmK& k, int b_trans, int dtype_in, int dtype_out, int batch, hipStream_t st) {
@@ -374,6 +408,22 @@
   }
   if (b_trans) return dtype_out == GPV_BF16 ? launch_skinny<bf16, true>(k, st) : launch_skinny<float, true>(k, st);
   return dtype_out == GPV_BF16 ? launch_skinny<bf16, false>(k, st) : launch_skinny<float, false>(k, st);
+}
+
+int tt_rows_try_launch(const GemmK& k, int dtype_in, int dtype_out, int batch, hipStream_t st) {
+  if (g_skinny_mode == 0 || dtype_in != GPV_BF16 || dtype_out != GPV_F32 || batch != 1 || !k.accumulate || k.M > 8) return -1;
+  if (k.rowscale || k.bias || k.res || k.mask || k.act || k.dthresh || k.a_rowsum) return -1;
+  if (k.N % 8 != 0 || k.ldb % 8 != 0 || k.ldc % 4 != 0 || !al16(k.B) || !al16(k.C) || k.lda < k.M || k.ldb < k.N) return -1;
+  int rps = (k.K + 255) / 256;
+  if (rps < 16) rps = 16;
+  const int slabs = (k.K + rps - 1) / rps;
+  if (k.ws_base == nullptr || !al16(k.ws_base) || (int64_t)slabs * k.M * k.N * 4 > k.ws_bytes) return -1;
+  float* ws = reinterpret_cast<float*>(k.ws_base);
+  ++g_tt_rows_launches;
+  hipLaunchKernelGGL(tt_rows_kernel, dim3((unsigned)((k.N / 8 + 255) / 256), (unsigned)slabs), dim3(256), 0, st, reinterpret_cast<const bf16*>(k.A), k.lda,
+                     reinterpret_cast<const bf16*>(k.B), k.ldb, k.M, k.N, k.K, rps, k.alpha, ws);
+  GPV_CHECK_LAUNCH();
+  return launch_splitk_reduce(ws, slabs, k.M, k.N, reinterpret_cast<float*>(k.C), k.ldc, st);
 }
 
 int skinny_tt_try_launch(const GemmK& k, int dtype_in, int dtype_out, int batch, hipStream_t st) {
diff --git a/gpv-1_amd/csrc/misc.hip b/gpv-1_amd/csrc/misc.hip
--- a/gpv-1_amd/csrc/misc.hip
+++ b/gpv-1_amd/csrc/misc.hip
@@ -534,12 +534,7 @@
 #pragma unroll
     for (int e = 0; e < 8; ++e) {
       if (act == GPV_ACT_RELU) g[e] = r[e] > 0.f ? g[e] * alpha : 0.f;
-      else {
-        const float z = r[e];
-        const float cdf = 0.5f * (1.0f + erff(z * 0.70710678118654752f));
-        const float pdf = 0.3989422804014327f * __expf(-0.5f * z * z);
-        g[e] = g[e] * (cdf + z * pdf) * alpha;
-      }
+      else g[e] = g[e] * gelu_erf_grad(r[e]) * alpha;
     }
     Ld8<T>::st(dx + i * 8, g);
   }
diff --git a/gpv-1_amd/hip.py b/gpv-1_amd/hip.py
--- a/gpv-1_amd/hip.py
+++ b/gpv-1_amd/hip.py
@@ -25,7 +25,8 @@
                 ('relu_mask', C.c_void_p), ('ldm', C.c_int64),
                 ('act', C.c_int), ('drop_p', C.c_float), ('seed', C.c_uint64),
                 ('accumulate', C.c_int), ('split_k', C.c_int), ('workspace', C.c_void_p), ('workspace_bytes', C.c_int64),
-                ('a_rowsum', C.c_void_p), ('flags', C.c_int)]
+                ('a_rowsum', C.c_void_p), ('flags', C.c_int),
+                ('pre_act', C.c_void_p), ('ldp', C.c_int64), ('y_mask_bits', C.c_void_p), ('relu_mask_bits', C.c_void_p)]
 
 
 class ConvArgs(C.Structure):
@@ -116,10 +117,12 @@
 
 OPT_GLDS, OPT_GLDS_LAUNCHES, OPT_SKINNY, OPT_GLDS_WGRAD, OPT_PIPE, OPT_PIPE_LAUNCHES, OPT_C1S, OPT_C3S, OPT_C3S_LAUNCHES = 0, 1, 2, 3, 4, 5, 6, 7, 8
 OPT_GEMV, OPT_GEMV_LAUNCHES = 9, 10
+OPT_TT_ROWS_LAUNCHES = 21
 OPT_ATTN_BWD1, OPT_ATTN_BWD1_LAUNCHES, OPT_C1S_LAUNCHES, OPT_WG8, OPT_WG8_LAUNCHES, OPT_W8L, OPT_PIPE_SMALL, OPT_WG8H, OPT_C3_HALO, OPT_C3_HALO_LAUNCHES = 11, 12, 13, 14, 15, 16, 17, 18, 19, 20
 
 
 GEMM_NO_PIPE_SMALL = 2
+GEMM_MASK_IS_PREACT = 4
 _TL = threading.local()
 
 
@@ -230,7 +233,8 @@
 
 def gemm(A, B, Cm, M, N, K, lda, ldb, ldc, layoutA=KMAJOR, layoutB=KMAJOR, batch=1, sA=0, sB=0, sC=0,
          alpha=1.0, rowscale=None, bias=None, res=None, ldr=0, sR=0, relu_mask=None, ldm=0, act=ACT_NONE,
-         drop_p=0.0, seed=0, accumulate=False, split_k=1, a_rowsum=None, kpad_finite=False):
+         drop_p=0.0, seed=0, accumulate=False, split_k=1, a_rowsum=None, kpad_finite=False, pre_act=None, ldp=0, mask_is_preact=False,
+         y_mask_bits=None, relu_mask_bits=None):
     a = GemmArgs()
     a.A, a.B, a.C = _p(A), _p(B), _p(Cm)
     a.M, a.N, a.K, a.batch = M, N, K, batch
@@ -253,6 +257,16 @@
     a.accumulate, a.split_k = int(accumulate), split_k
     a.a_rowsum = _p(_f32(a_rowsum))
     a.flags = (1 if kpad_finite else 0) | getattr(_TL, 'gemm_flags', 0)
+    if pre_act is not None:
+        if pre_act.dtype != Cm.dtype:
+            raise TypeError('gemm: pre_act dtype must equal output dtype')
+        a.pre_act, a.ldp = _p(pre_act), ldp
+    if mask_is_preact:
+        a.flags |= GEMM_MASK_IS_PREACT
+    for bits in (y_mask_bits, relu_mask_bits):
+        if bits is not None and (bits.dtype != torch.uint8 or bits.numel() < M * (N // 8) or N % 8):
+            raise TypeError('gemm: mask bits are uint8, N / 8 bytes per output row')
+    a.y_mask_bits, a.relu_mask_bits = _p(y_mask_bits), _p(relu_mask_bits)
     if accumulate and batch == 1:
         ws = _workspace(A.device, max(max(split_k, 8) * M * N * 4, 512 * 128 * 128 * 4))
         a.workspace, a.workspace_bytes = _p(ws), ws.numel()
diff --git a/gpv-1_amd/ops.py b/gpv-1_amd/ops.py
--- a/gpv-1_amd/ops.py
+++ b/gpv-1_amd/ops.py
@@ -884,6 +884,15 @@
 FFN_FUSED = os.environ.get('GPV_FFN_FUSED', '0') == '1'
 
 
+FFN_BITS = os.environ.get('GPV_FFN_BITS', '1') != '0'
+
+
+def ffn_bits_ok(x2, w1, w2):
+    return (FFN_BITS and RT.dtype == torch.bfloat16 and w1.K == 256 and w1.N % 256 == 0 and 1536 <= w1.N <= 2048 and x2.shape[0] >= 2048
+            and w1.r0 == 0 and w1.N == w1.Ntot
+            and w2.mirror_ok() and w2.r0 == 0 and w2.N == w2.Ntot and w2.K == w1.N and x2.data_ptr() % 16 == 0 and _gemm_takes('y_mask_bits'))
+
+
 class FFNBlockFn(Function):
 
     @staticmethod
@@ -904,9 +913,14 @@
         if not (FFN_FUSED and RT.dtype == torch.bfloat16 and w1.bias is not None and w2.bias is not None and
                 hip.ffn_fused_fwd(x2, w1.lp(), w1.bias_f32(), w2.lp(), w2.bias_f32(), gamma.detach(), beta.detach(), h, y, out, mean, rstd,
                                   M, K, Fh, eps, drop_p, seed1, seed2, pos=p2, out2=out2)):
-            hip.gemm(x2, w1.lp(), h, M, Fh, K, K, K, Fh, bias=w1.bias_f32(), act=ACT_RELU, drop_p=drop_p, seed=seed1)
+            bits = torch.empty(M, Fh // 8, device=x.device, dtype=torch.uint8) if ffn_bits_ok(x2, w1, w2) else None
+            hip.gemm(x2, w1.lp(), h, M, Fh, K, K, K, Fh, bias=w1.bias_f32(), act=ACT_RELU, drop_p=drop_p, seed=seed1,
+                     **({} if bits is None else {'y_mask_bits': bits}))
             hip.gemm(h, w2.lp(), y, M, K, Fh, Fh, Fh, K, bias=w2.bias_f32())
             hip.layernorm_fwd(x2, y, gamma.detach(), beta.detach(), out, mean, rstd, M, K, eps, drop_p, seed2, pos=p2, y2=out2)
+        else:
+            bits = None
+        ctx.bits = bits
         ctx.w1, ctx.w2, ctx.gamma, ctx.beta, ctx.drop_p, ctx.seed2, ctx.xshape = w1, w2, gamma, beta, drop_p, seed2, x.shape
         ctx.pos_param = pos_param
         ctx.save_for_backward(x2, h, y, mean, rstd)
@@ -936,7 +950,11 @@
         elif nb2:
             hip.colsum(dy2, w2.bgrad(), M, K, K)
         dz = torch.empty(M, Fh, device=d2.device, dtype=RT.dtype)
-        w2.dx_gemm(dy2, dz, M, relu_mask=h, ldm=Fh, alpha=1.0 / (1.0 - ctx.drop_p) if ctx.drop_p > 0 else 1.0)
+        alpha = 1.0 / (1.0 - ctx.drop_p) if ctx.drop_p > 0 else 1.0
+        if ctx.bits is not None and w2.mirror_ok():
+            w2.dx_gemm(dy2, dz, M, relu_mask_bits=ctx.bits, alpha=alpha)
+        else:
+            w2.dx_gemm(dy2, dz, M, relu_mask=h, ldm=Fh, alpha=alpha)
         nb1 = w1.bias is not None and w1.bias.requires_grad
         if w1.weight.requires_grad:
             wgrad_linear(dz, x2, w1.wgrad(), w1.bgrad() if nb1 else None, Fh, K, M, _split_k(Fh, K, M))
@@ -964,6 +982,84 @@
     if not (torch.is_grad_enabled() and x.requires_grad):
         return add_layernorm(x, linear(linear(x, w1, ACT_RELU, drop_p), w2), gamma, beta, eps, drop_p, pos=pos, pos_param=pos_param)
     return FFNBlockFn.apply(x, w1, w2, gamma, beta, eps, drop_p, pos, pos_param)
+
+
+GELU_FFN = os.environ.get('GPV_GELU_FFN', '1') != '0'
+
+
+class GeluFFNFn(Function):
+
+    @staticmethod
+    def forward(ctx, x, w1, w2, gamma, beta, eps, drop_p):
+        ctx.set_materialize_grads(False)
+        K, Fh = w1.K, w1.N
+        x2 = _c(_as_compute(x)).reshape(-1, K)
+        M = x2.shape[0]
+        z = torch.empty(M, Fh, device=x.device, dtype=RT.dtype)
+        h = torch.empty_like(z)
+        hip.gemm(x2, w1.lp(), h, M, Fh, K, K, K, Fh, bias=w1.bias_f32(), act=ACT_GELU, pre_act=z, ldp=Fh)
+        y = torch.empty(M, K, device=x.device, dtype=RT.dtype)
+        hip.gemm(h, w2.lp(), y, M, K, Fh, Fh, Fh, K, bias=w2.bias_f32())
+        out = torch.empty_like(x2)
+        mean = torch.empty(M, device=x.device, dtype=torch.float32)
+        rstd = torch.empty_like(mean)
+        seed = RT.next_seed() if drop_p > 0 else 0
+        hip.layernorm_fwd(x2, y, gamma.detach(), beta.detach(), out, mean, rstd, M, K, eps, drop_p, seed)
+        ctx.w1, ctx.w2, ctx.gamma, ctx.beta, ctx.drop_p, ctx.seed, ctx.xshape = w1, w2, gamma, beta, drop_p, seed, x.shape
+        ctx.save_for_backward(x2, z, h, y, mean, rstd)
+        return out.reshape(x.shape)
+
+    @staticmethod
+    def backward(ctx, dout):
+        nin = 7
+        if dout is None:
+            return (None,) * nin
+        w1, w2, gamma, beta = ctx.w1, ctx.w2, ctx.gamma, ctx.beta
+        x2, z, h, y, mean, rstd = ctx.saved_tensors
+        M, K = x2.shape
+        Fh = w1.N
+        d = _c(_as_compute(dout)).reshape(M, K)
+        dx_res = torch.empty_like(x2)
+        ds = torch.empty_like(x2) if ctx.drop_p > 0 else None
+        _ln_backward(d, None, x2, y, gamma, beta, mean, rstd, dx_res, ds, M, K, ctx.drop_p, ctx.seed)
+        dy2 = ds if ds is not None else dx_res
+        nb2 = w2.bias is not None and w2.bias.requires_grad
+        if w2.weight.requires_grad:
+            wgrad_linear(dy2, h, w2.wgrad(), w2.bgrad() if nb2 else None, K, Fh, M, _split_k(K, Fh, M))
+        elif nb2:
+            hip.colsum(dy2, w2.bgrad(), M, K, K)
+        dz = torch.empty(M, Fh, device=d.device, dtype=RT.dtype)
+        w2.dx_gemm(dy2, dz, M, relu_mask=z, ldm=Fh, mask_is_preact=True)
+        nb1 = w1.bias is not None and w1.bias.requires_grad
+        if w1.weight.requires_grad:
+            wgrad_linear(dz, x2, w1.wgrad(), w1.bgrad() if nb1 else None, Fh, K, M, _split_k(Fh, K, M))
+        elif nb1:
+            hip.colsum(dz, w1.bgrad(), M, Fh, Fh)
+        if not ctx.needs_input_grad[0]:
+            return (None,) * nin
+        dx = torch.empty(M, K, device=dz.device, dtype=RT.dtype)
+        w1.dx_gemm(dz, dx, M, res=dx_res, ldr=K)
+        return (dx.reshape(ctx.xshape),) + (None,) * (nin - 1)
+
+
+_GEMM_FIELDS = {}
+
+
+def _gemm_takes(name):
+    fn = hip.gemm
+    got = _GEMM_FIELDS.get(fn)
+    if got is None:
+        import inspect
+        got = _GEMM_FIELDS[fn] = frozenset(inspect.signature(fn).parameters)
+    return name in got
+
+
+def gelu_ffn_ok(x):
+    return GELU_FFN and RT.dtype == torch.bfloat16 and torch.is_grad_enabled() and x.requires_grad and _gemm_takes('pre_act')
+
+
+def gelu_ffn(x, w1, w2, gamma, beta, eps, drop_p=0.0):
+    return GeluFFNFn.apply(x, w1, w2, gamma, beta, eps, drop_p)
 
 
 def add_layernorm(x, s, gamma, beta, eps, drop_p=0.0, chain=None, pos=None, pos_param=None):
@@ -1147,7 +1243,7 @@
         hip.gemm(dyc, tok_lp, dp, rows, 2, D, D, D, 2)
         if tokens.requires_grad:
             hip.gemm(_as_compute(p), dyc, ensure_grad(tokens), 2, D, rows, 2, D, D, layoutA=hip.TRANS, layoutB=hip.TRANS,
-                     accumulate=True, split_k=_split_k(2, D, rows))
+                     accumulate=True, split_k=1 if RT.dtype == torch.bfloat16 else _split_k(2, D, rows))
         dlg = p * (dp - (p * dp).sum(-1, keepdim=True))
         return (dy if ctx.needs_input_grad[0] else None), (dlg if ctx.needs_input_grad[1] else None), None
 
diff --git a/gpv-1_amd/vilbert.py b/gpv-1_amd/vilbert.py
--- a/gpv-1_amd/vilbert.py
+++ b/gpv-1_amd/vilbert.py
@@ -105,6 +105,14 @@
         self.t_intermediate = _Intermediate(cfg.hidden_size, cfg.intermediate_size, cfg.hidden_act)
         self.t_output = _Output(cfg.intermediate_size, cfg.hidden_size, cfg.hidden_dropout_prob)
 
+    @staticmethod
+    def _ffn(inter, out, a):
+        if ops.gelu_ffn_ok(a):
+            d1, d2, ln = inter.dense, out.dense, out.LayerNorm
+            return ops.gelu_ffn(a, W(d1.weight, d1.bias), W(d2.weight, d2.bias), ln.weight, ln.bias, ln.eps, out.p if out.training else 0.0)
+        ca = ops.grad_chain(a)
+        return out(inter(a, ca), a, ca)
+
     def forward(self, t1, t2, B, T1, T2, kpm1=None):
         c1, c2 = ops.grad_chain(t1), ops.grad_chain(t2)
         br = ops.branch_for(t1) if (FUSE_QKV and t1.shape[-1] == t2.shape[-1]) else None
@@ -112,17 +120,13 @@
         bo = self.biOutput
         if br is None:
             a1, a2 = bo(bi2, t1, bi1, t2, c1, c2)
-            ca1, ca2 = ops.grad_chain(a1), ops.grad_chain(a2)
-            o1 = self.v_output(self.v_intermediate(a1, ca1), a1, ca1)
-            o2 = self.t_output(self.t_intermediate(a2, ca2), a2, ca2)
-            return o1, o2
+            return self._ffn(self.v_intermediate, self.v_output, a1), self._ffn(self.t_intermediate, self.t_output, a2)
         br.fork()
         with br.on():
             a1 = bo.LayerNorm1(t1, bo.dense1(bi2), bo.p1 if bo.training else 0.0, chain=c1)
         a2 = bo.LayerNorm2(t2, bo.dense2(bi1), bo.p2 if bo.training else 0.0, chain=c2)
-        ca1, ca2 = ops.grad_chain(a1), ops.grad_chain(a2)
         with br.on():
-            o1 = self.v_output(self.v_intermediate(a1, ca1), a1, ca1)
-        o2 = self.t_output(self.t_intermediate(a2, ca2), a2, ca2)
+            o1 = self._ffn(self.v_intermediate, self.v_output, a1)
+        o2 = self._ffn(self.t_intermediate, self.t_output, a2)
         br.join()
         return o1, o2
diff --git a/include/gpv_hip.h b/include/gpv_hip.h
--- a/include/gpv_hip.h
+++ b/include/gpv_hip.h
@@ -48,6 +48,7 @@
 #define GPV_OPT_C3_HALO_LAUNCHES 20
 #define GPV_OPT_W8L 16
 #define GPV_OPT_C1S_LAUNCHES 13
+#define GPV_OPT_TT_ROWS_LAUNCHES 21
 int gpv_set_option(int option, int value);
 
 typedef struct {
@@ -68,8 +69,12 @@
   void* workspace; int64_t workspace_bytes;
   float* a_rowsum;
   int flags;
+  void* pre_act; int64_t ldp;
+  void* y_mask_bits;
+  const void* relu_mask_bits;
 } gpv_gemm_args;
 #define GPV_GEMM_KPAD_FINITE 1
+#define GPV_GEMM_MASK_IS_PREACT 4
 #define GPV_GEMM_NO_PIPE_SMALL 2
 int gpv_gemm(const gpv_gemm_args* a, void* stream);
 
```

Measured after the change: 2154 images/sec. No clear change (-0.9%).
